# facebookresearch/dmc-net

Hardware: AMD Instinct MI355X
Metric: clips/sec (3-seg 224x224) DMC-gen+ResNet-18 train step (higher is better)
Workload: dtype f32

## Files before the change

### dmc-net_amd/_lib.py

```python
import ctypes
import os

PKG = os.path.dirname(os.path.abspath(__file__))
LIB_PATH = os.environ.get("DMC_HIP_LIB", os.path.join(PKG, "libdmcnet_hip.so"))

_P = ctypes.c_void_p
_I = ctypes.c_int
_F = ctypes.c_float
_Z = ctypes.c_size_t
_L = ctypes.c_long

SIGNATURES = {
    "dmc_version": (_I, []),
    "dmc_last_error": (ctypes.c_char_p, []),
    "dmc_profile_mark": (_I, [_P]),
    "dmc_set_option": (_I, [ctypes.c_char_p, _I]),
    "dmc_get_option": (_I, [ctypes.c_char_p]),
    "dmc_gen_tiny_workspace_bytes": (_Z, []),
    "dmc_gen_tiny_saved_bytes": (_Z, [_I, _I, _I]),
    "dmc_gen_tiny_gbuf_bytes": (_Z, [_I, _I, _I]),
    "dmc_gen_tiny_partials_bytes": (_Z, [_I, _I, _I]),
    "dmc_gen_tiny_fwd": (_I, [_P, _P, _P, _P, _P, _P, _P, _I, _I, _I, _I, _P]),
    "dmc_gen_tiny_mse_partials_bytes": (_Z, []),
    "dmc_gen_tiny_fwd_mse": (_I, [_P] * 10 + [_I, _I, _I, _I, _P]),
    "dmc_gen_tiny_fwd_loss": (_I, [_I] + [_P] * 10 + [_I, _I, _I, _I, _P]),
    "dmc_gen_tiny_bwd": (_I, [_P, _P, _P, _P, _P, _P, _P, _P, _P, _P, _I, _I, _I, _P]),
    "dmc_flow_mse_partials_bytes": (_Z, []),
    "dmc_flow_mse_fwd": (_I, [_P, _P, _P, _P, _Z, _P]),
    "dmc_flow_mse_bwd": (_I, [_P, _P, _P, _P, _Z, _P]),
    "dmc_flow_loss_partials_bytes": (_Z, []),
    "dmc_flow_loss_fwd": (_I, [_I, _P, _P, _P, _P, _P, _Z, _P]),
    "dmc_flow_loss_bwd": (_I, [_I, _P, _P, _P, _P, _P, _P, _Z, _P]),
    "dmc_consensus_ce_fwd_bwd": (_I, [_P, _P, _P, _P, _P, _I, _I, _I, _P]),
    "dmc_disc_tail_stats_bytes": (_Z, [_I]),
    "dmc_disc_tail_fwd": (_I, [_P, _P, _P, _P, _P, _P, _P, _P, _I, _I, _I, _I, _I, _I, _F, _F, _P]),
    "dmc_disc_tail_bwd": (_I, [_P, _P, _P, _P, _P, _P, _P, _P, _I, _I, _I, _I, _I, _P]),
    "dmc_prepare_inputs_workspace_bytes": (_Z, [_I, _I, _I, _I]),
    "dmc_prepare_inputs": (_I, [_P, _P, _P, _P, _P, _P, _I, _I, _I, _I, _P, _P]),
    "dmc_prepare_crop_workspace_bytes": (_Z, [_I, _I, _I, _I]),
    "dmc_prepare_inputs_crop": (_I, [_P, _P, _P, _P, _P, _P, _P, _I, _I, _I, _I, _I, _I, _P, _P]),
    "dmc_prepare_views_workspace_bytes": (_Z, [_I, _I, _I, _I, _I]),
    "dmc_prepare_inputs_views": (_I, [_P, _P, _P, _P, _P, _P, _P, _P, _I, _I, _I, _I, _I, _I, _I, _I, _P, _P]),
    "dmc_prepare_interp_taps": (_I, [_I, _I, _P, _P, _P]),
    "dmc_prepare_clip_workspace_bytes": (_Z, [_I, _I, _I, _I, _I]),
    "dmc_prepare_clip": (_I, [_P, _P, _P, _P] + [_I] * 8 + [_P, _P, _P]),
    "dmc_bn_act_supported": (_I, [_I, _I]),
    "dmc_bn_act_stats_bytes": (_Z, [_I]),
    "dmc_bn_act_scratch_bytes": (_Z, [_I]),
    "dmc_bn_act_fwd": (_I, [_P, _P, _P, _P, _P, _P, _P, _P, _P, _P, _I, _I, _I, _I, _F, _F, _P]),
    "dmc_bn_act_bwd": (_I, [_P, _P, _P, _P, _P, _P, _P, _P, _P, _P, _P, _P, _I, _I, _I, _P]),
    "dmc_bn_apply_nhwc": (_I, [_P, _P, _P, _P, _P, _I, _I, _P]),
    "dmc_bn_apply_act_nhwc": (_I, [_P, _P, _P, _P, _P, _P, _P, _I, _I, _I, _P]),
    "dmc_bn_bwd_act_nhwc": (_I, [_P] * 10 + [_I, _F, _I, _I, _P]),
    "dmc_channel_sum_nhwc": (_I, [_P, _P, _P, _I, _I, _P]),
    "dmc_bn_relu_pool_supported": (_I, [_I, _I, _I, _I]),
    "dmc_bn_relu_pool_fwd": (_I, [_P, _P, _P, _P, _P, _P, _P, _P, _I, _I, _I, _I, _I, _F, _F, _P]),
    "dmc_bn_relu_pool_codes_bytes": (_Z, [_I, _I, _I, _I]),
    "dmc_bn_relu_pool_bwd": (_I, [_P, _P, _P, _P, _P, _P, _P, _P, _P, _P, _I, _I, _I, _I, _P]),
    "dmc_conv_nhwc_supported": (_I, [_I] * 9),
    "dmc_conv_nhwc_stat_blocks": (_I, [_I] * 8),
    "dmc_conv_nhwc_fwd": (_I, [_P] * 7 + [_I] * 11 + [_P]),
    "dmc_conv_nhwc_stats_final": (_I, [_P, _I, _I, ctypes.c_long, _P, _P, _P, _F, _F, _P]),
    "dmc_conv_nhwc_wt_bytes": (_Z, [_I] * 4),
    "dmc_conv_nhwc_presplit_supported": (_I, [_I, _I]),
    "dmc_conv_nhwc_split": (_I, [_P, _P, _P, _I, _I, _I, _I, _P]),
    "dmc_conv_nhwc_dgrad": (_I, [_P] * 4 + [_I] * 9 + [_P]),
    "dmc_conv_nhwc_dgrad_add": (_I, [_P] * 5 + [_I] * 9 + [_P]),
    "dmc_conv_nhwc_wgrad_bytes": (_Z, [_I] * 9),
    "dmc_conv_nhwc_wgrad": (_I, [_P] * 4 + [_I] * 9 + [_P]),
    "dmc_x3s_slices_bytes": (_Z, [_L, _I]),
    "dmc_x3s_split": (_I, [_P, _P, _L, _I, _P]),
    "dmc_x3s_merge": (_I, [_P, _P, _L, _I, _P]),
    "dmc_x3s_wpack_bytes": (_Z, [_I, _I]),
    "dmc_x3s_pack_weights": (_I, [_P, _P, _P, _I, _I, _P]),
    "dmc_x3s_conv_supported": (_I, [_I] * 5),
    "dmc_x3s_conv_stat_blocks": (_I, [_I] * 4),
    "dmc_x3s_conv_fwd": (_I, [_P] * 4 + [_I] * 6 + [_P]),
    "dmc_x3s_conv_bn_eval": (_I, [_P] * 8 + [_I] * 7 + [_P]),
    "dmc_x3s_conv_dgrad": (_I, [_P] * 4 + [_I] * 5 + [_P]),
    "dmc_x3s_conv_wgrad_supported": (_I, [_I] * 5),
    "dmc_x3s_conv_wgrad_bytes": (_Z, [_I] * 5),
    "dmc_x3s_conv_wgrad": (_I, [_P] * 4 + [_I] * 5 + [_P]),
    "dmc_x3s_conv_dgrad_s2_supported": (_I, [_I] * 5),
    "dmc_x3s_pack_weights_s2": (_I, [_P, _P, _I, _I, _P]),
    "dmc_x3s_conv_dgrad_s2": (_I, [_P] * 3 + [_I] * 5 + [_P]),
    "dmc_x3q_wpack_bytes": (_Z, [_I, _I]),
    "dmc_x3q_supported": (_I, [_I] * 5),
    "dmc_x3q_stat_blocks": (_I, [_I] * 4),
    "dmc_x3q_split": (_I, [_P, _P, _I, _I, _I, _I, _P]),
    "dmc_x3q_merge": (_I, [_P, _P, _I, _I, _I, _I, _P]),
    "dmc_x3q_pack_weights": (_I, [_P, _P, _P, _P, _I, _I, _P]),
    "dmc_x3q_conv_fwd": (_I, [_P] * 6 + [_I] * 6 + [_P]),
    "dmc_x3q_conv_bn_eval": (_I, [_P] * 11 + [_I] * 5 + [_P]),
    "dmc_x3q_conv_dgrad": (_I, [_P] * 4 + [_I] * 5 + [_P]),
    "dmc_bn_apply_act_x3q": (_I, [_P] * 8 + [_I] * 5 + [_P]),
    "dmc_x3q_conv_wgrad_supported": (_I, [_I] * 5),
    "dmc_x3q_conv_wgrad_bytes": (_Z, [_I] * 5),
    "dmc_x3q_conv_wgrad": (_I, [_P] * 6 + [_I] * 5 + [_P]),
    "dmc_bn_apply_act_x3s": (_I, [_P] * 8 + [_I, _I, _I, _P]),
    "dmc_bn_act_bwd_x3s": (_I, [_P] * 13 + [_I, _I, _I, _P]),
    "dmc_x3s_conv_dgrad_bnb": (_I, [_P] * 9 + [_I] + [_P] + [_I] + [_P] * 2 + [_I] * 5 + [_P]),
    "dmc_bn_act_bwd_x3s_apply": (_I, [_P] * 12 + [_I, _I, _I, _P]),
    "dmc_bn_relu_pool_fwd_x3s": (_I, [_P] * 9 + [_I, _I, _I, _I, _I, _F, _F, _P]),
    "dmc_bn_relu_pool_fwd_arg": (_I, [_P] * 11 + [_I, _I, _I, _I, _I, _I, _F, _F, _P]),
    "dmc_bn_relu_pool_bwd_arg": (_I, [_P] * 11 + [_I, _I, _I, _I, _P]),
    "dmc_disc_first_supported": (_I, [_I]),
    "dmc_disc_first_fwd": (_I, [_P] * 5 + [_I] * 5 + [_P]),
    "dmc_disc_first_dgrad": (_I, [_P] * 3 + [_I] * 4 + [_P]),
    "dmc_disc_first_wgrad_bytes": (_Z, [_I]),
    "dmc_disc_first_wgrad": (_I, [_P] * 5 + [_I] * 4 + [_P]),
    "dmc_stem_wgrad_supported": (_I, [_I, _I]),
    "dmc_stem_wgrad_partials_bytes": (_Z, [_I, _I, _I]),
    "dmc_stem_wgrad": (_I, [_P, _P, _P, _P, _I, _I, _I, _P]),
    "dmc_stem_fwd": (_I, [_P, _P, _L, _L, _L, _L, _P, _I, _I, _I, _P]),
    "dmc_stem_fwd_x3_workspace_bytes": (_Z, [_I, _I, _I]),
    "dmc_stem_fwd_x3": (_I, [_P, _P, _L, _L, _L, _L, _P, _P, _I, _I, _I, _P]),
    "dmc_stem_fwd_x3_stat_blocks": (_I, [_I, _I, _I]),
    "dmc_stem_dgrad_workspace_bytes": (_Z, []),
    "dmc_stem_dgrad_supported": (_I, [_I, _I]),
    "dmc_stem_dgrad": (_I, [_P, _P, _L, _L, _L, _L, _P, _P, _I, _I, _I, _P]),
    "dmc_stem_fwd_x3_stats": (_I, [_P, _P, _L, _L, _L, _L, _P, _P, _P, _I, _I, _I, _P]),
    "dmc_conv3d_bf16_supported": (_I, [_I] * 9),
    "dmc_conv3d_bf16_wpack_bytes": (_Z, [_I] * 5),
    "dmc_conv3d_bf16_pack": (_I, [_P, _L, _L, _L, _P, _P] + [_I] * 5 + [_P]),
    "dmc_conv3d_bf16_stat_blocks": (_I, [_I] * 5),
    "dmc_conv3d_bf16_stat_blocks_k": (_I, [_I] * 9),
    "dmc_conv3d_bf16_fwd": (_I, [_P, _P, _L, _L, _L, _P, _P, _P] + [_I] * 9 + [_P]),
    "dmc_conv3d_bf16_dgrad": (_I, [_P, _P, _L, _L, _L, _P, _P] + [_I] * 9 + [_P]),
    "dmc_conv3d_bf16_wgrad_bytes": (_Z, [_I] * 9),
    "dmc_conv3d_bf16_wgrad": (_I, [_P] * 4 + [_I] * 9 + [_P]),
    "dmc_stem3d_bf16_workspace_bytes": (_Z, [_I] * 4),
    "dmc_stem3d_bf16_stat_blocks": (_I, [_I] * 4),
    "dmc_stem3d_bf16_fwd": (_I, [_P] * 5 + [_I] * 4 + [_P]),
    "dmc_stem3d_bf16_wgrad_workspace_bytes": (_Z, [_I] * 4),
    "dmc_stem3d_bf16_wgrad": (_I, [_P] * 4 + [_I] * 4 + [_P]),
    "dmc_stem3d_bf16_dgrad_workspace_bytes": (_Z, []),
    "dmc_stem3d_bf16_dgrad": (_I, [_P] * 4 + [_I] * 4 + [_P]),
    "dmc_bn3d_bf16_supported": (_I, [_L, _I]),
    "dmc_bn3d_bf16_scratch_bytes": (_Z, [_I]),
    "dmc_bn3d_bf16_fwd": (_I, [_P, _P, _I, _P, _P, _P, _P, _P, _P, _L, _I, _I, _F, _F, _P]),
    "dmc_add4_bf16": (_I, [_P] * 5 + [_L, _P]),
    "dmc_bn3d_bf16_fwd_ld": (_I, [_P, _P, _I, _P, _P, _P, _P, _P, _P, _L, _L, _I, _I, _F, _F, _P]),
    "dmc_bn3d_bf16_bwd": (_I, [_P, _L] + [_P] * 8 + [_L, _I, _I, _P]),
    "dmc_unit3d_bf16_fwd_workspace_bytes": (_Z, [_I] * 9),
    "dmc_unit3d_bf16_bwd_workspace_bytes": (_Z, [_I] * 9),
    "dmc_unit3d_bf16_fwd": (_I, [_P] * 9 + [_I] * 10 + [_F, _F, _P]),
    "dmc_unit3d_bf16_fwd_into": (_I, [_P] * 9 + [_L] + [_I] * 10 + [_F, _F, _P]),
    "dmc_unit3d_bf16_bwd": (_I, [_P, _L] + [_P] * 11 + [_I] * 10 + [_P]),
    "dmc_unit3d_bf16_eval_workspace_bytes": (_Z, [_I] * 9),
    "dmc_unit3d_bf16_fwd_eval": (_I, [_P] * 6 + [_F, _P, _P, _L] + [_I] * 10 + [_P]),
    "dmc_stem3d_bf16_eval_workspace_bytes": (_Z, [_I] * 4),
    "dmc_stem3d_bf16_fwd_eval": (_I, [_P] * 6 + [_F, _P, _P] + [_I] * 5 + [_P]),
    "dmc_maxpool3d_tf_out_shape": (_I, [_I] * 10 + [_P] * 3),
    "dmc_maxpool3d_tf_bf16_fwd": (_I, [_P] * 3 + [_I] * 11 + [_P]),
    "dmc_maxpool3d_tf_bf16_bwd": (_I, [_P] * 3 + [_I] * 11 + [_P]),
    "dmc_mv_owner_bytes": (_Z, [_I, _I, _I]),
    "dmc_mv_accu_init": (_I, [_P, _I, _I, _P]),
    "dmc_mv_rasterise": (_I, [_P, _I, _I, _P, _P, _P, _I, _I, _P]),
    "dmc_mv_accumulate": (_I, [_P, _I, _I, _P, _P, _P, _P, _I, _I, _P]),
    "dmc_mv_from_accu": (_I, [_P, _P, _I, _I, _P]),
    "dmc_residual": (_I, [_P, _P, _P, _P, _P, _I, _I, _P]),
    "dmc_mv_gop_batch": (_I, [_P, _I, _I, _P, _I, _P, _I, _P, _P, _P, _P, _P, _P, _P, _P, _I, _I, _P]),
}

_lib = None


class DmcHipError(RuntimeError):
    pass


def load():
    global _lib
    if _lib is None:
        if not os.path.exists(LIB_PATH):
            raise DmcHipError(
                "%s is missing: the DMC-Net hot path has no CPU fallback. Build it with "
                "`python -c 'import __graft_entry__ as g; g.build()'`." % LIB_PATH)
        lib = ctypes.CDLL(LIB_PATH)
        for name, (res, args) in SIGNATURES.items():
            fn = getattr(lib, name)
            fn.restype, fn.argtypes = res, args
        _lib = lib
    return _lib


def check(rc, what):
    if rc != 0:
        raise DmcHipError("%s failed (%d): %s" % (what, rc, load().dmc_last_error().decode()))


def ptr(t):
    return _P(t.data_ptr()) if t is not None else _P(0)


def ptr_array(tensors):
    return (_P * len(tensors))(*[t.data_ptr() for t in tensors])
```

### dmc-net_amd/csrc/conv_x3q.hip

```cpp
#include "dmc_common.h"
#include "x3s_common.h"
#include <type_traits>
#include <utility>

using namespace dmc;
using namespace dmc::x3;

namespace {

constexpr int QBM = 256, QBN = 64;
constexpr int QWSLOT = 3 * QBN * 32;
constexpr int QWB = 3 * QWSLOT;
constexpr int QEP = 272, QETILE = 32 * QEP;

template <int NW_, int NPB_, int NT_>
struct QG {
    static constexpr int NW = NW_, NPB = NPB_, NT = NT_;
    static constexpr int NA = NW / 2;
    static constexpr int KP = (NT + NA - 1) / NA;
    static constexpr int PT = 3 * KP;
    static constexpr int KW = (18 + NA - 1) / NA;
    static constexpr int ZROW = 32 * NT;
    static constexpr int PSL = (ZROW + 1) * 32;
    static constexpr int PB = 3 * PSL;
    static constexpr int WOFF = NPB * PB;
    static constexpr int LDS_OP = WOFF + 2 * QWB;
    static constexpr int LDS_EP = NW * QETILE + 8192;
    static constexpr int LDS = LDS_OP > LDS_EP ? LDS_OP : LDS_EP;
    static constexpr bool COUNTED = NPB == 3;
    static_assert(!COUNTED || NT % NA == 0, "counted waits need the same number of transfers from every patch wave");
};
using QGBig = QG<8, 3, 12>;
using QGTwo = QG<4, 2, 7>;

struct QSlot { int sh, acc; };
struct QStep { int unit, nslot; QSlot s[3]; };

struct ProgFwd {
    static constexpr int NUNIT = 4, NSTEP = 5, NACC = 2, NSH = 4, HALO_UP = 1, HALO_DN = 0, NSLOTS = 10;
    static constexpr int SHY[4] = {-1, -1, 0, 0}, SHX[4] = {-1, 0, -1, 0};
    static constexpr int UNIT_T[4] = {0, 0, 0, 0};
    static constexpr int UNIT_G[4] = {3, 1, 2, 0};
    static constexpr QStep STEP[5] = {{0, 2, {{0, 0}, {1, 0}, {0, 0}}}, {0, 2, {{2, 0}, {3, 0}, {0, 0}}}, {1, 2, {{2, 0}, {3, 0}, {0, 0}}},
                                      {2, 2, {{1, 0}, {3, 0}, {0, 0}}}, {3, 2, {{3, 0}, {3, 1}, {0, 0}}}};
};
struct ProgDgrad {
    static constexpr int NUNIT = 2, NSTEP = 4, NACC = 4, NSH = 4, HALO_UP = 0, HALO_DN = 1, NSLOTS = 10;
    static constexpr int SHY[4] = {0, 0, 1, 1}, SHX[4] = {0, 1, 0, 1};
    static constexpr int UNIT_T[2] = {0, 1};
    static constexpr int UNIT_G[2] = {0, 0};
    static constexpr QStep STEP[4] = {{0, 3, {{3, 3}, {2, 2}, {2, 3}}}, {0, 3, {{1, 1}, {0, 0}, {0, 1}}}, {0, 3, {{1, 3}, {0, 2}, {0, 3}}},
                                      {1, 1, {{0, 0}, {0, 0}, {0, 0}}}};
};

template <class P> constexpr int slots_before(int j) { int n = 0; for (int i = 0; i < j; ++i) n += P::STEP[i].nslot; return n; }

struct X3qArgs {
    const void* t0;
    const void* t1;
    const void* wp;
    float* y0;
    float* y1;
    double* part0;
    double* part1;
    int N, H, W;
    int K, R, M;
    unsigned plane_bytes;
    int pps0, pps1;
};

struct X3qEvalArgs : X3qArgs {
    const float *stats0, *gamma0, *beta0;
    const float *stats1, *gamma1, *beta1;
    unsigned short* ys0;
};

template <int N, class F, int... I>
__device__ __forceinline__ void static_for_impl(F&& f, std::integer_sequence<int, I...>) { (f(std::integral_constant<int, I>{}), ...); }
template <int N, class F>
__device__ __forceinline__ void static_for(F&& f) { static_for_impl<N>(f, std::make_integer_sequence<int, N>{}); }

template <class P, int TN, class GEO, bool EVAL = false>
__global__ __launch_bounds__(GEO::NW * 64) void x3q_conv_kernel(std::conditional_t<EVAL, X3qEvalArgs, X3qArgs> a) {
    static_assert(!EVAL || P::NACC == 2, "the eval epilogue belongs to the forward pair");
    constexpr int NSH = P::NSH, NACC = P::NACC, NSTEP = P::NSTEP, NUNIT = P::NUNIT;
    constexpr int QNW = GEO::NW, QNPB = GEO::NPB, QZROW = GEO::ZROW, QPSL = GEO::PSL, QPB = GEO::PB, QWOFF = GEO::WOFF, QPT = GEO::PT;
    constexpr int NA = GEO::NA, KP = GEO::KP, KW = GEO::KW;
    constexpr int WN = 2 / TN, WM = QNW / WN, BM = 32 * WM;
    static_assert(TN == 1 || TN == 2, "a wave owns 32 or 64 of the workgroup's 64 rows");
    constexpr int CHB = P::NSLOTS * QWSLOT;
    static_assert(P::NSLOTS % 2 == 0, "the fragment registers alternate per slot: an even number per chunk keeps the roles fixed");
    extern __shared__ __attribute__((aligned(1024))) char lds_q[];

    const int tid = threadIdx.x, lane = tid & 63;
    const int wave = __builtin_amdgcn_readfirstlane(tid >> 6);
    const int wm = wave % WM, wn = wave / WM;
    const int l31 = lane & 31, khalf = lane >> 5;
    const unsigned lds0 = lds_addr_of(lds_q);

    const int HW = a.H * a.W, PW = a.W;
    const int m0 = blockIdx.x * BM;
    const int mlast = (m0 + BM < a.M ? m0 + BM : a.M) - 1;
    const int r_first = m0 / PW, r_last = mlast / PW;
    const int f0 = (r_first - P::HALO_UP > 0 ? r_first - P::HALO_UP : 0) * PW;
    const int f1 = (r_last + 1 + P::HALO_DN) * PW < a.M ? (r_last + 1 + P::HALO_DN) * PW : a.M;
    const int PP = f1 - f0;

    const bool grp_a = wave < NA;
    const int wq = wave % NA;
    unsigned pvoff[KP];
#pragma unroll
    for (int k = 0; k < KP; ++k) {
        const int pr = 32 * (wq + NA * k) + (lane >> 1), h = lane & 1;
        pvoff[k] = pr < PP ? (unsigned)(f0 + pr) * 32u + (unsigned)((h ^ ((pr >> 3) & 1)) << 4) : OOB;
    }
    const int nchunk = a.K >> 4;
    const int total_units = nchunk * NUNIT, total_steps = nchunk * NSTEP;
    const u32x4 srd0 = make_srd(a.t0), srd1 = make_srd(a.t1 ? a.t1 : a.t0);
    const u32x4 srd_w = make_srd(reinterpret_cast<const char*>(a.wp) + (size_t)blockIdx.y * nchunk * CHB);
    const unsigned lane16 = (unsigned)lane * 16u;

    auto dma_patch = [&](int c, auto uc, int pbuf, int i) {
        constexpr int u = decltype(uc)::value;
        constexpr int ut = P::UNIT_T[u], ug = P::UNIT_G[u];
        const int s = i / KP, k = i - KP * s;
        const unsigned soff = (unsigned)(s * (ut ? a.pps1 : a.pps0) + ug * nchunk + c) * a.plane_bytes;
        if (GEO::COUNTED || wq + NA * k < GEO::NT)
            dma_buf16(ut ? srd1 : srd0, pvoff[k], soff, lds0 + pbuf * QPB + s * QPSL + (wq + NA * k) * 1024);
    };
    auto dma_weight = [&](int c, auto jc, int wbuf, int e) {
        constexpr int j = decltype(jc)::value;
        constexpr int n = P::STEP[j].nslot * 6, off = slots_before<P>(j) * QWSLOT;
        if (e < n) dma_buf16(srd_w, lane16, (unsigned)(c * CHB + off + e * 1024), lds0 + QWOFF + wbuf * QWB + e * 1024);
    };

    int xaddr[NSH];
    {
        int m = m0 + wm * 32 + l31;
        if (m > mlast) m = mlast;
        const int n = m / HW, rem = m - n * HW, yy = rem / a.W, xx = rem - yy * a.W;
        const int pp = m - f0;
        static_for<NSH>([&](auto sc) {
            constexpr int sh = decltype(sc)::value;
            constexpr int dy = P::SHY[sh], dx = P::SHX[sh];
            const int row = (xx + dx >= 0 && xx + dx < a.W && yy + dy >= 0 && yy + dy < a.H) ? pp + dy * PW + dx : QZROW;
            xaddr[sh] = row * 32 + ((khalf ^ ((row >> 3) & 1)) << 4);
        });
    }
    const int waddr = QWOFF + (wn * TN * 32 + l31) * 32 + ((khalf ^ ((l31 >> 3) & 1)) << 4);

    f32x16 acc[NACC][TN];
#pragma unroll
    for (int s = 0; s < NACC; ++s)
#pragma unroll
        for (int j = 0; j < TN; ++j)
#pragma unroll
            for (int e = 0; e < 16; ++e) acc[s][j][e] = 0.f;

    lds_cptr const L = (lds_cptr)lds_q;
    struct Frag { u32x4 X[3], W[TN][3]; };
    auto load_frags = [&](Frag& f, int xa, int wa, auto kc) {
        constexpr int k = decltype(kc)::value;
#pragma unroll
        for (int s = 0; s < 3; ++s) {
#pragma unroll
            for (int j = 0; j < TN; ++j)
                f.W[j][s] = *reinterpret_cast<const __attribute__((address_space(3))) u32x4*>(L + wa + ((k * 3 + s) * QBN + 32 * j) * 32);
            f.X[s] = *reinterpret_cast<const __attribute__((address_space(3))) u32x4*>(L + xa + s * QPSL);
        }
    };
    auto mfma_slot = [&](const Frag& f, auto ac, auto&& between) {
        constexpr int A = decltype(ac)::value;
#pragma unroll
        for (int p = 0; p < 6; ++p) {
            constexpr int WS[6] = {0, 0, 0, 1, 1, 2}, XS[6] = {2, 1, 0, 1, 0, 0};
#pragma unroll
            for (int j = 0; j < TN; ++j) acc[A][j] = mfma_bf16(f.W[j][WS[p]], f.X[XS[p]], acc[A][j]);
            between(p);
        }
    };
    auto nothing = [](int) {};
    constexpr int NRD = 3 + 3 * TN, NMF = 6 * TN;
    auto interleave = [&]() {
#pragma unroll
        for (int k = 0; k < (NRD < NMF ? NRD : NMF); ++k) {
            __builtin_amdgcn_sched_group_barrier(0x008, 1, 0);
            __builtin_amdgcn_sched_group_barrier(0x100, 1, 0);
        }
        if constexpr (NMF > NRD) __builtin_amdgcn_sched_group_barrier(0x008, NMF - NRD, 0);
    };

    if (tid < 2 * 3 * QNPB)
        *reinterpret_cast<float4*>(lds_q + (tid >> 1) / 3 * QPB + ((tid >> 1) % 3) * QPSL + QZROW * 32 + (tid & 1) * 16) = make_float4(0.f, 0.f, 0.f, 0.f);
    if (grp_a) {
        static_for<QNPB>([&](auto uc) {
            constexpr int U = decltype(uc)::value;
            if (U < total_units) {
#pragma unroll
                for (int i = 0; i < QPT; ++i) dma_patch(U / NUNIT, std::integral_constant<int, U % NUNIT>{}, U, i);
            }
        });
    } else {
        static_for<2>([&](auto gc) {
            constexpr int g = decltype(gc)::value;
            if (g < total_steps) {
#pragma unroll
                for (int i = 0; i < KW; ++i) dma_weight(g / NSTEP, std::integral_constant<int, g % NSTEP>{}, g, wq + NA * i);
            }
        });
    }
    asm volatile("s_waitcnt vmcnt(0)" ::: "memory");
    __builtin_amdgcn_s_barrier();

    Frag F0, F1;
    int pb = 0, wb = 0;
    int xcur[NSH];
#pragma unroll
    for (int sh = 0; sh < NSH; ++sh) xcur[sh] = xaddr[sh];
    int wcur = waddr;
    {
        constexpr int sh0 = P::STEP[0].s[0].sh;
        load_frags(F0, xcur[sh0], wcur, std::integral_constant<int, 0>{});
    }

    auto frag_of = [&](auto ic) -> Frag& {
        if constexpr (decltype(ic)::value == 0) return F0; else return F1;
    };
#pragma unroll 1
    for (int c = 0; c < nchunk; ++c) {
        static_for<NSTEP>([&](auto jc) {
            constexpr int J = decltype(jc)::value;
            constexpr int JN = (J + 1) % NSTEP;
            constexpr int unit = P::STEP[J].unit, nslot = P::STEP[J].nslot;
            constexpr bool unit_last = (P::STEP[JN].unit != unit) || (NUNIT == 1 && J == NSTEP - 1);
            constexpr int par = slots_before<P>(J) & 1;
            const int g = c * NSTEP + J, U = c * NUNIT + unit;
            static_for<nslot - 1>([&](auto kc) {
                constexpr int k = decltype(kc)::value;
                constexpr int sh_next = P::STEP[J].s[k + 1].sh, acc_k = P::STEP[J].s[k].acc;
                load_frags(frag_of(std::integral_constant<int, (par + k + 1) & 1>{}), xcur[sh_next], wcur, std::integral_constant<int, k + 1>{});
                mfma_slot(frag_of(std::integral_constant<int, (par + k) & 1>{}), std::integral_constant<int, acc_k>{}, nothing);
                interleave();
            });
            if (GEO::COUNTED && grp_a && U + 2 < total_units) asm volatile("s_waitcnt vmcnt(%0) lgkmcnt(0)" :: "n"(QPT) : "memory");
            else asm volatile("s_waitcnt vmcnt(0) lgkmcnt(0)" ::: "memory");
            __builtin_amdgcn_s_barrier();
            const int pb_old = pb, wb_old = wb;
            if constexpr (unit_last) {
                pb = pb == QNPB - 1 ? 0 : pb + 1;
#pragma unroll
                for (int sh = 0; sh < NSH; ++sh) xcur[sh] = xaddr[sh] + pb * QPB;
            }
            wb ^= 1;
            wcur = waddr + wb * QWB;
            constexpr int kl = nslot - 1;
            constexpr int sh_first = P::STEP[JN].s[0].sh, acc_last = P::STEP[J].s[kl].acc;
            if (g + 1 < total_steps)
                load_frags(frag_of(std::integral_constant<int, (par + kl + 1) & 1>{}), xcur[sh_first], wcur, std::integral_constant<int, 0>{});
            constexpr int J2 = (J + 2) % NSTEP, C2 = (J + 2) / NSTEP;
            constexpr int U3 = (unit + QNPB) % NUNIT, CU3 = (unit + QNPB) / NUNIT;
            const bool wgo = !grp_a && g + 2 < total_steps;
            const bool pgo = grp_a && unit_last && U + QNPB < total_units;
            mfma_slot(frag_of(std::integral_constant<int, (par + kl) & 1>{}), std::integral_constant<int, acc_last>{}, [&](int p) {
                if (wgo) {
#pragma unroll
                    for (int i = p; i < KW; i += 6) dma_weight(c + C2, std::integral_constant<int, J2>{}, wb_old, wq + NA * i);
                }
                if constexpr (unit_last) {
                    if (pgo) {
#pragma unroll
                        for (int i = p; i < QPT; i += 6) dma_patch(c + CU3, std::integral_constant<int, U3>{}, pb_old, i);
                    }
                }
            });
        });
    }

    __syncthreads();
    constexpr int CW = 32 * TN, LPR = CW / 4, RPI = 64 / LPR;
    char* etile = lds_q + wave * QETILE;
    const int mw0 = m0 + wm * 32;
    const int rbase = blockIdx.y * QBN + wn * CW;
    const bool ok = mw0 + l31 <= mlast;
#pragma unroll
    for (int A = 0; A < NACC; ++A) {
#pragma unroll
        for (int j = 0; j < TN; ++j)
#pragma unroll
            for (int g4 = 0; g4 < 4; ++g4) {
                float4 v = make_float4(acc[A][j][4 * g4], acc[A][j][4 * g4 + 1], acc[A][j][4 * g4 + 2], acc[A][j][4 * g4 + 3]);
                if (!ok) v = make_float4(0.f, 0.f, 0.f, 0.f);
                *reinterpret_cast<float4*>(etile + l31 * QEP + (32 * j + 8 * g4 + 4 * khalf) * 4) = v;
            }
        float* const yout = (NACC == 2 && A == 1) ? a.y1 : a.y0;
        if constexpr (EVAL) {
            const int c4 = rbase + (lane % LPR) * 4;
            const float* const st = A == 1 ? a.stats1 : a.stats0;
            const float4 mean = *reinterpret_cast<const float4*>(st + c4), istd = *reinterpret_cast<const float4*>(st + a.R + c4);
            const float4 gm = *reinterpret_cast<const float4*>((A == 1 ? a.gamma1 : a.gamma0) + c4);
            const float4 bt = *reinterpret_cast<const float4*>((A == 1 ? a.beta1 : a.beta0) + c4);
            unsigned short* const ys = A == 1 ? nullptr : a.ys0;
#pragma unroll
            for (int it = 0; it < 32 / RPI; ++it) {
                const int prow = RPI * it + lane / LPR;
                const int m = mw0 + prow;
                const float4 v = *reinterpret_cast<const float4*>(etile + prow * QEP + (lane % LPR) * 16);
                if (m <= mlast) {
                    const float w[4] = {bn_apply_act1(v.x, mean.x, istd.x, gm.x, bt.x, false, 0.f, A == 0),
                                        bn_apply_act1(v.y, mean.y, istd.y, gm.y, bt.y, false, 0.f, A == 0),
                                        bn_apply_act1(v.z, mean.z, istd.z, gm.z, bt.z, false, 0.f, A == 0),
                                        bn_apply_act1(v.w, mean.w, istd.w, gm.w, bt.w, false, 0.f, A == 0)};
                    if (yout) *reinterpret_cast<float4*>(yout + (size_t)m * a.R + c4) = make_float4(w[0], w[1], w[2], w[3]);
                    if (ys) x3s_store4(ys, w, (size_t)a.M, a.R >> 4, (size_t)m, c4 >> 2);
                }
            }
        } else {
#pragma unroll
        for (int it = 0; it < 32 / RPI; ++it) {
            const int prow = RPI * it + lane / LPR;
            const int m = mw0 + prow;
            const float4 v = *reinterpret_cast<const float4*>(etile + prow * QEP + (lane % LPR) * 16);
            if (m <= mlast) {
                size_t opix = (size_t)m;
                if (NACC == 4) {
                    const int n = m / HW, rem = m - n * HW, ya = rem / a.W, xb = rem - ya * a.W;
                    opix = ((size_t)n * (2 * a.H) + 2 * ya + (A >> 1)) * (2 * a.W) + 2 * xb + (A & 1);
                }
                *reinterpret_cast<float4*>(yout + opix * a.R + rbase + (lane % LPR) * 4) = v;
            }
        }
        }
        if (NACC == 2 && !EVAL) {
            double* const part = A == 1 ? a.part1 : a.part0;
            if (part) {
                double* red = reinterpret_cast<double*>(lds_q + QNW * QETILE);
                if (lane < CW) {
                    double d1 = 0.0, d2 = 0.0;
#pragma unroll 8
                    for (int p = 0; p < 32; ++p) {
                        const double v = (double)*reinterpret_cast<const float*>(etile + p * QEP + lane * 4);
                        d1 += v;
                        d2 += v * v;
                    }
                    red[(wm * 64 + wn * CW + lane) * 2 + 0] = d1;
                    red[(wm * 64 + wn * CW + lane) * 2 + 1] = d2;
                }
                __syncthreads();
                for (int cc = tid; cc < QBN; cc += QNW * 64) {
                    double e1 = 0.0, e2 = 0.0;
#pragma unroll
                    for (int w = 0; w < WM; ++w) { e1 += red[(w * 64 + cc) * 2 + 0]; e2 += red[(w * 64 + cc) * 2 + 1]; }
                    double* dst = part + ((size_t)blockIdx.x * a.R + blockIdx.y * QBN + cc) * 2;
                    dst[0] = e1; dst[1] = e2;
                }
                __syncthreads();
            }
        }
    }
}

__global__ __launch_bounds__(256) void x3q_pack_w_kernel(const float* __restrict__ w3, const float* __restrict__ w1,
                                                         unsigned short* __restrict__ wf, unsigned short* __restrict__ wt, int Cout, int Cin) {
    const bool transposed = blockIdx.y == 1;
    unsigned short* dst = transposed ? wt : wf;
    if (!dst) return;
    const int R = transposed ? Cin : Cout, K = transposed ? Cout : Cin;
    const int nchunk = K >> 4;
    const long total = (long)R * 10 * K;
    for (long i = (long)blockIdx.x * 256 + threadIdx.x; i < total; i += (long)gridDim.x * 256) {
        long t = i;
        const int kk = (int)(t & 15); t >>= 4;
        const int rl = (int)(t & 63); t >>= 6;
        const int slot = (int)(t % 10); t /= 10;
        const int ch = (int)(t % nchunk);
        const int rt = (int)(t / nchunk);
        const int r = rt * 64 + rl, k = ch * 16 + kk;
        constexpr int FWD_TAP[10] = {0, 2, 6, 8, 3, 5, 1, 7, 4, 9};
        const int tap = transposed ? slot : FWD_TAP[slot];
        const int co = transposed ? k : r, ci = transposed ? r : k;
        const float v = tap < 9 ? w3[((long)co * 9 + tap) * Cin + ci] : w1[(long)co * Cin + ci];
        unsigned u0, u1, u2;
        split3(v, u0, u1, u2);
        const size_t base = ((((size_t)(rt * nchunk + ch) * 10 + slot) * 3) * 64 + rl) * 16 + (kk ^ (((rl >> 3) & 1) << 3));
        dst[base] = (unsigned short)(u0 >> 16);
        dst[base + 64 * 16] = (unsigned short)(u1 >> 16);
        dst[base + 2 * 64 * 16] = (unsigned short)(u2 >> 16);
    }
}

__global__ __launch_bounds__(256) void x3q_split_kernel(const float* __restrict__ x, unsigned short* __restrict__ xq, int N, int H, int W, int C) {
    const int c8 = C >> 3, nchunk = C >> 4, H2 = H >> 1, W2 = W >> 1;
    const long total = (long)N * H * W * c8;
    const size_t Mq = (size_t)N * H2 * W2;
    for (long o = (long)blockIdx.x * 256 + threadIdx.x; o < total; o += (long)gridDim.x * 256) {
        const long m = o / c8;
        const int g = (int)(o - m * c8);
        const int xx = (int)(m % W), yy = (int)((m / W) % H), n = (int)(m / ((long)W * H));
        const float4 a = reinterpret_cast<const float4*>(x)[2 * o], b = reinterpret_cast<const float4*>(x)[2 * o + 1];
        const float v[8] = {a.x, a.y, a.z, a.w, b.x, b.y, b.z, b.w};
        const int cls = (yy & 1) * 2 + (xx & 1);
        x3s_store8(xq, v, Mq, 4 * nchunk, ((size_t)n * H2 + (yy >> 1)) * W2 + (xx >> 1), g + cls * 2 * nchunk);
    }
}

__global__ __launch_bounds__(256) void x3q_merge_kernel(const unsigned short* __restrict__ xq, float* __restrict__ x, int N, int H, int W, int C) {
    const int nchunk = C >> 4, H2 = H >> 1, W2 = W >> 1;
    const long total = (long)N * H * W * C;
    const size_t Mq = (size_t)N * H2 * W2, plane = Mq * 16;
    for (long o = (long)blockIdx.x * 256 + threadIdx.x; o < total; o += (long)gridDim.x * 256) {
        const long m = o / C;
        const int c = (int)(o - m * C);
        const int xx = (int)(m % W), yy = (int)((m / W) % H), n = (int)(m / ((long)W * H));
        const int cls = (yy & 1) * 2 + (xx & 1);
        const size_t mq = ((size_t)n * H2 + (yy >> 1)) * W2 + (xx >> 1);
        const size_t w = ((size_t)(cls * nchunk + (c >> 4)) * Mq + mq) * 16 + (c & 15);
        const float s0 = __uint_as_float((unsigned)xq[w] << 16);
        const float s1 = __uint_as_float((unsigned)xq[(size_t)4 * nchunk * plane + w] << 16);
        const float s2 = __uint_as_float((unsigned)xq[(size_t)8 * nchunk * plane + w] << 16);
        x[o] = (s0 + s1) + s2;
    }
}

int stream_blocks_q(long total) {
    long b = (total + 255) / 256;
    return (int)(b < 1 ? 1 : (b > 8192 ? 8192 : b));
}

int q_patch_pixels_max(long M, int W) {
    int worst = 0;
    long tiles = (M + QBM - 1) / QBM;
    if (tiles > W) tiles = W;
    for (long t = 0; t < tiles; ++t) {
        const long m0 = t * QBM, ml = (m0 + QBM < M ? m0 + QBM : M) - 1;
        const int pp = (int)((ml / W - m0 / W + 2) * W);
        if (pp > worst) worst = pp;
    }
    return worst;
}

int q_patch_pixels_max128(long M, int W) {
    int worst = 0;
    long tiles = (M + 127) / 128;
    if (tiles > W) tiles = W;
    for (long t = 0; t < tiles; ++t) {
        const long m0 = t * 128, ml = (m0 + 128 < M ? m0 + 128 : M) - 1;
        const int pp = (int)((ml / W - m0 / W + 2) * W);
        if (pp > worst) worst = pp;
    }
    return worst;
}

bool q_shape_ok(int N, int OH, int OW, int Cin, int Cout) {
    if (N <= 0 || OH <= 0 || OW <= 0 || Cin <= 0 || Cout <= 0 || Cin % 64 != 0 || Cout % 64 != 0) return false;
    const long M = (long)N * OH * OW;
    if (M * 4 * Cin * 6 >= (1L << 31) || M * Cout * 6 >= (1L << 31)) return false;
    return q_patch_pixels_max(M, OW) <= QGBig::ZROW;
}

int q_choose_tn(long M, int R) {
    const int forced = option(OPT_CONV_CFG);
    if (forced == 201) return 2;
    if (forced == 202) return 1;
    const long n2 = ((M + 255) / 256) * (R / QBN), n1 = ((M + 127) / 128) * (R / QBN);
    const double t2 = (double)((n2 + 255) / 256), t1 = 0.75 * (double)((n1 + 255) / 256);
    return t1 < t2 ? 1 : 2;
}

template <class P, int TN, class GEO>
int launch_q(const X3qArgs& a, hipStream_t s) {
    static LdsLimit lim;
    const hipError_t attr = lim.raise(reinterpret_cast<const void*>(&x3q_conv_kernel<P, TN, GEO>), GEO::LDS);
    if (attr != hipSuccess) return fail(DMC_E_LAUNCH, "x3q_conv: cannot raise the dynamic LDS limit: %s", hipGetErrorString(attr));
    constexpr int BM = 32 * GEO::NW / (2 / TN);
    dim3 grid((a.M + BM - 1) / BM, a.R / QBN);
    x3q_conv_kernel<P, TN, GEO><<<grid, GEO::NW * 64, GEO::LDS, s>>>(a);
    return check_launch("x3q_conv");
}

template <int TN, class GEO>
int launch_q_eval(const X3qEvalArgs& a, hipStream_t s) {
    static LdsLimit lim;
    const hipError_t attr = lim.raise(reinterpret_cast<const void*>(&x3q_conv_kernel<ProgFwd, TN, GEO, true>), GEO::LDS);
    if (attr != hipSuccess) return fail(DMC_E_LAUNCH, "x3q_conv_bn_eval: cannot raise the dynamic LDS limit: %s", hipGetErrorString(attr));
    constexpr int BM = 32 * GEO::NW / (2 / TN);
    dim3 grid((a.M + BM - 1) / BM, a.R / QBN);
    x3q_conv_kernel<ProgFwd, TN, GEO, true><<<grid, GEO::NW * 64, GEO::LDS, s>>>(a);
    return check_launch("x3q_conv_bn_eval");
}

int q_patch_pixels_max128(long M, int W);
int q_variant(long M, int W, int R) {
    const int forced = option(OPT_CONV_CFG);
    const bool two_ok = q_patch_pixels_max128(M, W) <= QGTwo::ZROW;
    if (forced == 201) return 0;
    if (forced == 202) return 1;
    if (forced == 203 && two_ok) return 2;
    if (forced != 204 && two_ok && ((M + 127) / 128) * (R / QBN) >= 512) return 2;
    return q_choose_tn(M, R) == 2 ? 0 : 1;
}
int q_block_pixels(int variant) { return variant == 0 ? 256 : 128; }


struct X3qWgArgs {
    const void* xq;
    const void* dys;
    float* part;
    int N, OH, Cin, Cout;
    unsigned plane_bytes;
    int steps, per_group, tiles_ci;
};

template <int OW_, int R, int HP_>
struct QWgGeom {
    static constexpr int PW = OW_ + 1;
    static constexpr int D1 = 3, D0 = 2;
    static constexpr int XPL1 = ((D1 * R * PW + 3) / 8) * 8 + 4;
    static constexpr int XPL0 = ((D0 * R * PW + 3) / 8) * 8 + 4;
    static constexpr int NPX = R * OW_;
    static constexpr int NKB = (NPX + 15) / 16;
    static constexpr int DYT = ((NKB * 16 + 31) / 32) * 32;
    static constexpr int DYPL = ((DYT + 3) / 8) * 8 + 4;
    static constexpr int XI = (R * PW + 31) / 32;
    static constexpr int DI = DYT / 32;
    static constexpr int CLS_OFF[4] = {0, 4 * XPL0 * 32, 8 * XPL0 * 32, 8 * XPL0 * 32 + 4 * XPL1 * 32};
    static constexpr int SLB = 8 * XPL0 * 32 + 8 * XPL1 * 32;
    static constexpr int XBYTES = 3 * SLB, DYBYTES = 12 * DYPL * 32;
    static constexpr int LDS = XBYTES + 2 * DYBYTES;
    static_assert(HP_ % R == 0, "steps are whole groups of padded rows");
};

template <int OW_, int R, int HP_>
__global__ __launch_bounds__(768) void x3q_wgrad_kernel(X3qWgArgs a) {
    using G = QWgGeom<OW_, R, HP_>;
    constexpr int PW = G::PW, DYPL = G::DYPL, NKB = G::NKB;
    extern __shared__ __attribute__((aligned(1024))) char lds_qw[];
    const int tid = threadIdx.x, lane = tid & 63;
    const int wave = __builtin_amdgcn_readfirstlane(tid >> 6);
    const int l31 = lane & 31, khalf = lane >> 5, L = lane & 15, grp = (lane >> 4) & 1;
    const int quarter = wave & 3, trow = wave >> 2;
    const int wi = quarter & 1, wj = quarter >> 1;
    const int tci = blockIdx.x % a.tiles_ci, tco = blockIdx.x / a.tiles_ci;
    const unsigned lds0 = lds_addr_of(lds_qw);
    const int s_begin = blockIdx.y * a.per_group;
    const int s_end = s_begin + a.per_group < a.steps ? s_begin + a.per_group : a.steps;
    const u32x4 srd_x = make_srd(a.xq), srd_d = make_srd(a.dys);
    const int nch_in = a.Cin >> 4;
    const int tsl = wave >> 2, tch = wave & 3;
    const unsigned soff_d = (unsigned)(tsl * (a.Cout >> 4) + tco * 4 + tch) * a.plane_bytes;
    const unsigned dplane = lds0 + G::XBYTES + (unsigned)wave * DYPL * 32;
    const int lpx = lane >> 1;
    const unsigned lhalf = (unsigned)(lane & 1) << 4;

    const unsigned img_bytes = (unsigned)(a.OH * OW_) * 32u;
    unsigned xpre[G::XI], dpre[G::DI];
#pragma unroll
    for (int i = 0; i < G::XI; ++i) {
        const int px = 32 * i + lpx;
        const int r = px / PW, col = px - r * PW - 1;
        xpre[i] = (col >= 0 && col < OW_) ? (unsigned)(r * OW_ + col) * 32u + lhalf : NOPIX;
    }
#pragma unroll
    for (int i = 0; i < G::DI; ++i) {
        const int p = 32 * i + lpx;
        dpre[i] = p < G::NPX ? (unsigned)p * 32u + lhalf : NOPIX;
    }
    auto issue_x = [&](int q, const WgGroupPos& g) {
        unsigned tbase, img_off;
        wg_group_base(g, a.N, OW_, img_bytes, tbase, img_off);
        unsigned voff[G::XI];
#pragma unroll
        for (int i = 0; i < G::XI; ++i) voff[i] = wg_lane_off(tbase, xpre[i], img_bytes);
#pragma unroll
        for (int cls = 0; cls < 4; ++cls) {
            const int D = (cls >> 1) ? G::D1 : G::D0, xpl = (cls >> 1) ? G::XPL1 : G::XPL0;
            const int slot0 = (((q % D) + D) % D) * R;
            const unsigned soff_x = (unsigned)(tsl * 4 * nch_in + cls * nch_in + tci * 4 + tch) * a.plane_bytes + img_off;
            const unsigned xplane = lds0 + (unsigned)(tsl * G::SLB + G::CLS_OFF[cls] + tch * xpl * 32);
#pragma unroll
            for (int i = 0; i < G::XI; ++i)
                if (32 * i + lpx < R * PW) dma_buf16(srd_x, voff[i], soff_x, xplane + (unsigned)(slot0 * PW + 32 * i) * 32u);
        }
    };
    auto issue_dy = [&](const WgGroupPos& g, int buf) {
        unsigned tbase, img_off;
        wg_group_base(g, a.N, OW_, img_bytes, tbase, img_off);
#pragma unroll
        for (int i = 0; i < G::DI; ++i)
            dma_buf16(srd_d, wg_lane_off(tbase, dpre[i], img_bytes), soff_d + img_off, dplane + (unsigned)buf * G::DYBYTES + (unsigned)(32 * i) * 32u);
    };

    f32x16 acc[3];
#pragma unroll
    for (int t = 0; t < 3; ++t)
#pragma unroll
        for (int e = 0; e < 16; ++e) acc[t][e] = 0.f;

    WgGroupPos g1 = wg_group_at(s_begin, R, HP_);
    if (s_begin < s_end) {
        issue_x(s_begin - 1, wg_group_prev(g1, R, HP_));
        issue_x(s_begin, g1);
        issue_dy(g1, 0);
    }
    g1 = wg_group_next(g1, R, HP_);
    asm volatile("s_waitcnt vmcnt(0)" ::: "memory");
    __builtin_amdgcn_s_barrier();
    const int py = trow != 1, da = trow == 0 ? -1 : 0;
    const int DR = (py ? G::D1 : G::D0) * R, xpl = py ? G::XPL1 : G::XPL0;
    const int cls_a = py ? G::CLS_OFF[3] : G::CLS_OFF[1];
    const int cls_b = py ? G::CLS_OFF[2] : G::CLS_OFF[0];
    lds_cptr const LB = (lds_cptr)lds_qw;
    int rr[NKB][2], xcol[NKB][2], dyoff[NKB][2];
#pragma unroll
    for (int kb = 0; kb < NKB; ++kb)
#pragma unroll
        for (int u = 0; u < 2; ++u) {
            int P = 16 * kb + 8 * khalf + 4 * u + (L >> 2);
            dyoff[kb][u] = (2 * wi + grp) * DYPL * 32 + G::XBYTES + (L & 3) * 8 + P * 32;
            if (P >= G::NPX) P = G::NPX - 1;
            rr[kb][u] = P / OW_;
            xcol[kb][u] = (2 * wj + grp) * xpl * 32 + (L & 3) * 8 + (P - rr[kb][u] * OW_) * 32;
        }
#pragma unroll 1
    for (int s = s_begin; s < s_end; ++s) {
        const int buf = (s - s_begin) & 1;
        issue_x(s + 1, g1);
        if (s + 1 < s_end) issue_dy(g1, buf ^ 1);
        g1 = wg_group_next(g1, R, HP_);
        const int sb = (((R * s + da) % DR) + DR) % DR;
#pragma unroll
        for (int kb = 0; kb < NKB; ++kb) {
            int dyo[2], xa[2], xb[2];
#pragma unroll
            for (int u = 0; u < 2; ++u) {
                dyo[u] = dyoff[kb][u] + buf * G::DYBYTES;
                int slot = sb + rr[kb][u];
                slot = slot >= DR ? slot - DR : slot;
                const int xo = xcol[kb][u] + slot * PW * 32;
                xa[u] = xo + cls_a;
                xb[u] = xo + cls_b;
            }
            u32x4 A[3], B[3][3];
#pragma unroll
            for (int sl = 0; sl < 3; ++sl) {
                tr_read2(LB + dyo[0] + sl * 4 * DYPL * 32, LB + dyo[1] + sl * 4 * DYPL * 32, A[sl]);
                tr_read2(LB + xa[0] + sl * G::SLB, LB + xa[1] + sl * G::SLB, B[0][sl]);
                tr_read2(LB + xb[0] + sl * G::SLB + 32, LB + xb[1] + sl * G::SLB + 32, B[1][sl]);
                tr_read2(LB + xa[0] + sl * G::SLB + 32, LB + xa[1] + sl * G::SLB + 32, B[2][sl]);
            }
#pragma unroll
            for (int t = 0; t < 3; ++t) {
                acc[t] = mfma_bf16(A[0], B[t][2], acc[t]);
                acc[t] = mfma_bf16(A[2], B[t][0], acc[t]);
                acc[t] = mfma_bf16(A[1], B[t][1], acc[t]);
                acc[t] = mfma_bf16(A[0], B[t][1], acc[t]);
                acc[t] = mfma_bf16(A[1], B[t][0], acc[t]);
                acc[t] = mfma_bf16(A[0], B[t][0], acc[t]);
            }
        }
        asm volatile("s_waitcnt vmcnt(0) lgkmcnt(0)" ::: "memory");
        __builtin_amdgcn_s_barrier();
    }
    float* out = a.part + (size_t)blockIdx.y * a.Cout * 9 * a.Cin;
    const int ci = tci * 64 + 32 * wj + l31;
#pragma unroll
    for (int t = 0; t < 3; ++t)
#pragma unroll
        for (int e = 0; e < 16; ++e) {
            const int co = tco * 64 + 32 * wi + 8 * (e >> 2) + 4 * khalf + (e & 3);
            out[((size_t)co * 9 + 3 * trow + t) * a.Cin + ci] = acc[t][e];
        }
}

struct X3qWg1Args {
    const void* xq; const void* dys; float* part;
    int Cin, Cout; long Mq; unsigned plane_bytes; int steps, per_group, tiles_ci;
};
constexpr int W1PX = 64, W1PL = 68;
constexpr int W1TILE = 12 * W1PL * 32, W1LDS = 4 * W1TILE;

__global__ __launch_bounds__(256) void x3q_wgrad1_kernel(X3qWg1Args a) {
    extern __shared__ __attribute__((aligned(1024))) char lds_w1[];
    const int tid = threadIdx.x, lane = tid & 63;
    const int wave = __builtin_amdgcn_readfirstlane(tid >> 6);
    const int l31 = lane & 31, khalf = lane >> 5, L = lane & 15, grp = (lane >> 4) & 1;
    const int wi = wave & 1, wj = wave >> 1;
    const int tci = blockIdx.x % a.tiles_ci, tco = blockIdx.x / a.tiles_ci;
    const unsigned lds0 = lds_addr_of(lds_w1);
    const int s_begin = blockIdx.y * a.per_group;
    const int s_end = s_begin + a.per_group < a.steps ? s_begin + a.per_group : a.steps;
    const u32x4 srd_x = make_srd(a.xq), srd_d = make_srd(a.dys);
    const int nch_in = a.Cin >> 4, nch_out = a.Cout >> 4;
    const int lpx = lane >> 1;
    const unsigned lhalf = (unsigned)(lane & 1) << 4;
    auto issue = [&](int s, int buf) {
#pragma unroll
        for (int k = 0; k < 3; ++k) {
            const int pl = 3 * wave + k, sl = pl >> 2, ch = pl & 3;
#pragma unroll
            for (int i = 0; i < 2; ++i) {
                const long p = (long)s * W1PX + 32 * i + lpx;
                const unsigned voff = p < a.Mq ? (unsigned)p * 32u + lhalf : OOB;
                dma_buf16(srd_x, voff, (unsigned)(sl * 4 * nch_in + tci * 4 + ch) * a.plane_bytes,
                          lds0 + (unsigned)(buf * 2 * W1TILE + pl * W1PL * 32 + 32 * i * 32));
                dma_buf16(srd_d, voff, (unsigned)(sl * nch_out + tco * 4 + ch) * a.plane_bytes,
                          lds0 + (unsigned)(buf * 2 * W1TILE + W1TILE + pl * W1PL * 32 + 32 * i * 32));
            }
        }
    };
    f32x16 acc;
#pragma unroll
    for (int e = 0; e < 16; ++e) acc[e] = 0.f;
    if (s_begin < s_end) issue(s_begin, 0);
    asm volatile("s_waitcnt vmcnt(0)" ::: "memory");
    __builtin_amdgcn_s_barrier();
    lds_cptr const LB = (lds_cptr)lds_w1;
#pragma unroll 1
    for (int s = s_begin; s < s_end; ++s) {
        const int buf = (s - s_begin) & 1;
        if (s + 1 < s_end) issue(s + 1, buf ^ 1);
        const int xb = buf * 2 * W1TILE + (2 * wj + grp) * W1PL * 32 + (L & 3) * 8;
        const int db = buf * 2 * W1TILE + W1TILE + (2 * wi + grp) * W1PL * 32 + (L & 3) * 8;
#pragma unroll
        for (int kb = 0; kb < W1PX / 16; ++kb) {
            u32x4 A[3], B[3];
            const int P0 = 16 * kb + 8 * khalf + (L >> 2), P1 = P0 + 4;
#pragma unroll
            for (int sl = 0; sl < 3; ++sl) {
                tr_read2(LB + db + sl * 4 * W1PL * 32 + P0 * 32, LB + db + sl * 4 * W1PL * 32 + P1 * 32, A[sl]);
                tr_read2(LB + xb + sl * 4 * W1PL * 32 + P0 * 32, LB + xb + sl * 4 * W1PL * 32 + P1 * 32, B[sl]);
            }
            acc = mfma_bf16(A[0], B[2], acc);
            acc = mfma_bf16(A[2], B[0], acc);
            acc = mfma_bf16(A[1], B[1], acc);
            acc = mfma_bf16(A[0], B[1], acc);
            acc = mfma_bf16(A[1], B[0], acc);
            acc = mfma_bf16(A[0], B[0], acc);
        }
        asm volatile("s_waitcnt vmcnt(0) lgkmcnt(0)" ::: "memory");
        __builtin_amdgcn_s_barrier();
    }
    float* out = a.part + (size_t)blockIdx.y * a.Cout * a.Cin;
    const int ci = tci * 64 + 32 * wj + l31;
#pragma unroll
    for (int e = 0; e < 16; ++e) {
        const int co = tco * 64 + 32 * wi + 8 * (e >> 2) + 4 * khalf + (e & 3);
        out[(size_t)co * a.Cin + ci] = acc[e];
    }
}

__global__ __launch_bounds__(256) void x3q_wgrad_reduce_kernel(const float* __restrict__ part, float* __restrict__ dw, int ngroup, long numel) {
    __shared__ float4 red[16][17];
    const int o = threadIdx.x & 15, sl = threadIdx.x >> 4;
    for (long i0 = (long)blockIdx.x * 64; i0 < numel; i0 += (long)gridDim.x * 64) {
        const long i = i0 + 4 * o;
        float4 s = make_float4(0.f, 0.f, 0.f, 0.f);
        if (i < numel)
            for (int k = sl; k < ngroup; k += 16) {
                const float4 v = *reinterpret_cast<const float4*>(part + (size_t)k * numel + i);
                s.x += v.x; s.y += v.y; s.z += v.z; s.w += v.w;
            }
        red[sl][o] = s;
        __syncthreads();
        if (sl == 0 && i < numel) {
            float4 t = red[0][o];
#pragma unroll
            for (int k = 1; k < 16; ++k) { const float4 v = red[k][o]; t.x += v.x; t.y += v.y; t.z += v.z; t.w += v.w; }
            *reinterpret_cast<float4*>(dw + i) = t;
        }
        __syncthreads();
    }
}

struct QWgPlan { int R, HP, steps, tiles, groups, per_group, steps1, groups1, per_group1; };
bool q_wgrad_plan(int N, int OH, int OW, int Cin, int Cout, QWgPlan& p) {
    if (Cin % 64 != 0 || Cout % 64 != 0 || N <= 0) return false;
    if (OW == 28 && OH == 28) { p.R = 1; p.HP = 29; }
    else if (OW == 14 && OH == 14) { p.R = 2; p.HP = 16; }
    else if (OW == 7 && OH == 7) { p.R = 4; p.HP = 8; }
    else return false;
    p.steps = N * p.HP / p.R;
    p.tiles = (Cout / 64) * (Cin / 64);
    int groups = 256 / p.tiles;
    if (groups < 1) groups = 1;
    if (groups > p.steps) groups = p.steps;
    p.per_group = (p.steps + groups - 1) / groups;
    p.groups = (p.steps + p.per_group - 1) / p.per_group;
    const long Mq = (long)N * OH * OW;
    p.steps1 = (int)((Mq + W1PX - 1) / W1PX);
    int g1 = 512 / p.tiles;
    if (g1 < 1) g1 = 1;
    if (g1 > p.steps1) g1 = p.steps1;
    p.per_group1 = (p.steps1 + g1 - 1) / g1;
    p.groups1 = (p.steps1 + p.per_group1 - 1) / p.per_group1;
    return true;
}

template <int OW_, int R, int HP_>
int launch_q_wgrad(const QWgPlan& p, const X3qWgArgs& a, hipStream_t s) {
    using G = QWgGeom<OW_, R, HP_>;
    static_assert(G::LDS <= 160 * 1024, "weight-gradient tiles exceed the LDS");
    static LdsLimit lim;
    const hipError_t attr = lim.raise(reinterpret_cast<const void*>(&x3q_wgrad_kernel<OW_, R, HP_>), G::LDS);
    if (attr != hipSuccess) return fail(DMC_E_LAUNCH, "x3q_wgrad: cannot raise the dynamic LDS limit: %s", hipGetErrorString(attr));
    x3q_wgrad_kernel<OW_, R, HP_><<<dim3(p.tiles, p.groups), 768, G::LDS, s>>>(a);
    return check_launch("x3q_wgrad");
}

}

extern "C" {

size_t dmc_x3q_wpack_bytes(int Cin, int Cout) { return (size_t)Cin * (size_t)Cout * 10 * 6; }

int dmc_x3q_supported(int N, int OH, int OW, int Cin, int Cout) { return q_shape_ok(N, OH, OW, Cin, Cout) ? 1 : 0; }

int dmc_x3q_stat_blocks(int N, int OH, int OW, int Cout) {
    const long M = (long)N * OH * OW;
    const int bm = q_block_pixels(q_variant(M, OW, Cout));
    return (int)((M + bm - 1) / bm);
}

int dmc_x3q_split(const float* x, void* xq, int N, int H, int W, int C, dmc_stream_t stream) {
    if (!x || !xq || N <= 0 || H <= 0 || W <= 0 || (H & 1) || (W & 1) || C <= 0 || C % 16 != 0)
        return fail(DMC_E_INVALID, "dmc_x3q_split: bad argument");
    x3q_split_kernel<<<stream_blocks_q((long)N * H * W * (C / 8)), 256, 0, (hipStream_t)stream>>>(x, static_cast<unsigned short*>(xq), N, H, W, C);
    return check_launch("x3q_split");
}

int dmc_x3q_merge(const void* xq, float* x, int N, int H, int W, int C, dmc_stream_t stream) {
    if (!x || !xq || N <= 0 || H <= 0 || W <= 0 || (H & 1) || (W & 1) || C <= 0 || C % 16 != 0)
        return fail(DMC_E_INVALID, "dmc_x3q_merge: bad argument");
    x3q_merge_kernel<<<stream_blocks_q((long)N * H * W * C), 256, 0, (hipStream_t)stream>>>(static_cast<const unsigned short*>(xq), x, N, H, W, C);
    return check_launch("x3q_merge");
}

int dmc_x3q_pack_weights(const float* w3, const float* w1, void* wpack_f, void* wpack_t, int Cin, int Cout, dmc_stream_t stream) {
    if (!w3 || !w1 || (!wpack_f && !wpack_t) || Cin % 64 != 0 || Cout % 64 != 0 || Cin <= 0 || Cout <= 0)
        return fail(DMC_E_INVALID, "dmc_x3q_pack_weights: bad argument");
    const long total = (long)Cin * Cout * 10;
    const int blocks = stream_blocks_q(total) > 1024 ? 1024 : stream_blocks_q(total);
    x3q_pack_w_kernel<<<dim3(blocks, 2), 256, 0, (hipStream_t)stream>>>(w3, w1, static_cast<unsigned short*>(wpack_f),
                                                                           static_cast<unsigned short*>(wpack_t), Cout, Cin);
    return check_launch("x3q_pack_w");
}

int dmc_x3q_conv_fwd(const void* xq, const void* wpack_f, float* y3, float* y1, double* stat_partials3, double* stat_partials1,
                     int stat_blocks, int N, int OH, int OW, int Cin, int Cout, dmc_stream_t stream) {
    if (!xq || !wpack_f || !y3 || !y1) return fail(DMC_E_INVALID, "dmc_x3q_conv_fwd: null pointer");
    if (!q_shape_ok(N, OH, OW, Cin, Cout))
        return fail(DMC_E_INVALID, "dmc_x3q_conv_fwd: unsupported shape N=%d OH=%d OW=%d Cin=%d Cout=%d", N, OH, OW, Cin, Cout);
    const int var = q_variant((long)N * OH * OW, OW, Cout);
    const int rows = (int)(((long)N * OH * OW + q_block_pixels(var) - 1) / q_block_pixels(var));
    if ((stat_partials3 || stat_partials1) && stat_blocks != rows)
        return fail(DMC_E_INVALID, "dmc_x3q_conv_fwd: statistics partials have %d rows but this launch writes %d (dmc_x3q_stat_blocks "
                                   "was called under another conv_cfg option?)", stat_blocks, rows);
    X3qArgs a;
    a.t0 = xq; a.t1 = nullptr; a.wp = wpack_f; a.y0 = y3; a.y1 = y1; a.part0 = stat_partials3; a.part1 = stat_partials1;
    a.N = N; a.H = OH; a.W = OW; a.K = Cin; a.R = Cout; a.M = N * OH * OW;
    a.plane_bytes = (unsigned)a.M * 32u;
    a.pps0 = 4 * (Cin / 16); a.pps1 = 0;
    return var == 0 ? launch_q<ProgFwd, 2, QGBig>(a, (hipStream_t)stream) : var == 1 ? launch_q<ProgFwd, 1, QGBig>(a, (hipStream_t)stream)
                                                                                      : launch_q<ProgFwd, 2, QGTwo>(a, (hipStream_t)stream);
}

int dmc_x3q_conv_bn_eval(const void* xq, const void* wpack_f, const float* stats3, const float* gamma3, const float* beta3,
                         const float* stats1, const float* gamma1, const float* beta1, float* y3, void* ys3, float* y1, int N, int OH,
                         int OW, int Cin, int Cout, dmc_stream_t stream) {
    if (!xq || !wpack_f || !stats3 || !gamma3 || !beta3 || !stats1 || !gamma1 || !beta1 || !y1)
        return fail(DMC_E_INVALID, "dmc_x3q_conv_bn_eval: null pointer");
    if (!y3 && !ys3) return fail(DMC_E_INVALID, "dmc_x3q_conv_bn_eval: no main-branch output (y3 and ys3 are both null)");
    if (!q_shape_ok(N, OH, OW, Cin, Cout))
        return fail(DMC_E_INVALID, "dmc_x3q_conv_bn_eval: unsupported shape N=%d OH=%d OW=%d Cin=%d Cout=%d", N, OH, OW, Cin, Cout);
    const int var = q_variant((long)N * OH * OW, OW, Cout);
    X3qEvalArgs a;
    a.t0 = xq; a.t1 = nullptr; a.wp = wpack_f; a.y0 = y3; a.y1 = y1; a.part0 = a.part1 = nullptr;
    a.N = N; a.H = OH; a.W = OW; a.K = Cin; a.R = Cout; a.M = N * OH * OW;
    a.plane_bytes = (unsigned)a.M * 32u;
    a.pps0 = 4 * (Cin / 16); a.pps1 = 0;
    a.stats0 = stats3; a.gamma0 = gamma3; a.beta0 = beta3; a.stats1 = stats1; a.gamma1 = gamma1; a.beta1 = beta1;
    a.ys0 = static_cast<unsigned short*>(ys3);
    return var == 0 ? launch_q_eval<2, QGBig>(a, (hipStream_t)stream) : var == 1 ? launch_q_eval<1, QGBig>(a, (hipStream_t)stream)
                                                                                  : launch_q_eval<2, QGTwo>(a, (hipStream_t)stream);
}

int dmc_x3q_conv_dgrad(const void* dys3, const void* dys1, const void* wpack_t, float* dx, int N, int OH, int OW, int Cin, int Cout,
                       dmc_stream_t stream) {
    if (!dys3 || !dys1 || !wpack_t || !dx) return fail(DMC_E_INVALID, "dmc_x3q_conv_dgrad: null pointer");
    if (!q_shape_ok(N, OH, OW, Cin, Cout))
        return fail(DMC_E_INVALID, "dmc_x3q_conv_dgrad: unsupported shape N=%d OH=%d OW=%d Cin=%d Cout=%d", N, OH, OW, Cin, Cout);
    X3qArgs a;
    a.t0 = dys3; a.t1 = dys1; a.wp = wpack_t; a.y0 = dx; a.y1 = nullptr; a.part0 = a.part1 = nullptr;
    a.N = N; a.H = OH; a.W = OW; a.K = Cout; a.R = Cin; a.M = N * OH * OW;
    a.plane_bytes = (unsigned)a.M * 32u;
    a.pps0 = a.pps1 = Cout / 16;
    const int var = q_variant(a.M, OW, Cin);
    return var == 0 ? launch_q<ProgDgrad, 2, QGBig>(a, (hipStream_t)stream) : var == 1 ? launch_q<ProgDgrad, 1, QGBig>(a, (hipStream_t)stream)
                                                                                        : launch_q<ProgDgrad, 2, QGTwo>(a, (hipStream_t)stream);
}

int dmc_x3q_conv_wgrad_supported(int N, int OH, int OW, int Cin, int Cout) {
    QWgPlan p;
    return q_shape_ok(N, OH, OW, Cin, Cout) && q_wgrad_plan(N, OH, OW, Cin, Cout, p) ? 1 : 0;
}

size_t dmc_x3q_conv_wgrad_bytes(int N, int OH, int OW, int Cin, int Cout) {
    QWgPlan p;
    if (!q_wgrad_plan(N, OH, OW, Cin, Cout, p)) return 0;
    return ((size_t)p.groups * 9 + (size_t)p.groups1) * Cout * Cin * sizeof(float);
}

int dmc_x3q_conv_wgrad(const void* xq, const void* dys3, const void* dys1, float* dw3, float* dw1, float* workspace, int N, int OH,
                       int OW, int Cin, int Cout, dmc_stream_t stream) {
    QWgPlan p;
    if (!xq || !dys3 || !dys1 || !dw3 || !dw1 || !workspace) return fail(DMC_E_INVALID, "dmc_x3q_conv_wgrad: null pointer");
    if (!dmc_x3q_conv_wgrad_supported(N, OH, OW, Cin, Cout) || !q_wgrad_plan(N, OH, OW, Cin, Cout, p))
        return fail(DMC_E_INVALID, "dmc_x3q_conv_wgrad: unsupported shape N=%d OH=%d OW=%d Cin=%d Cout=%d", N, OH, OW, Cin, Cout);
    hipStream_t s = (hipStream_t)stream;
    const long Mq = (long)N * OH * OW;
    X3qWgArgs a;
    a.xq = xq; a.dys = dys3; a.part = workspace;
    a.N = N; a.OH = OH; a.Cin = Cin; a.Cout = Cout;
    a.plane_bytes = (unsigned)Mq * 32u;
    a.steps = p.steps; a.per_group = p.per_group; a.tiles_ci = Cin / 64;
    int rc = OW == 28 ? launch_q_wgrad<28, 1, 29>(p, a, s) : OW == 14 ? launch_q_wgrad<14, 2, 16>(p, a, s) : launch_q_wgrad<7, 4, 8>(p, a, s);
    if (rc) return rc;
    const long numel3 = (long)Cout * 9 * Cin, numel1 = (long)Cout * Cin;
    long blocks = (numel3 + 63) / 64;
    x3q_wgrad_reduce_kernel<<<(int)(blocks > 4096 ? 4096 : blocks), 256, 0, s>>>(workspace, dw3, p.groups, numel3);
    rc = check_launch("x3q_wgrad_reduce");
    if (rc) return rc;
    float* part1 = workspace + (size_t)p.groups * numel3;
    X3qWg1Args b;
    b.xq = xq; b.dys = dys1; b.part = part1; b.Cin = Cin; b.Cout = Cout; b.Mq = Mq; b.plane_bytes = (unsigned)Mq * 32u;
    b.steps = p.steps1; b.per_group = p.per_group1; b.tiles_ci = Cin / 64;
    static LdsLimit lim1;
    const hipError_t attr = lim1.raise(reinterpret_cast<const void*>(&x3q_wgrad1_kernel), W1LDS);
    if (attr != hipSuccess) return fail(DMC_E_LAUNCH, "x3q_wgrad1: cannot raise the dynamic LDS limit: %s", hipGetErrorString(attr));
    x3q_wgrad1_kernel<<<dim3(p.tiles, p.groups1), 256, W1LDS, s>>>(b);
    rc = check_launch("x3q_wgrad1");
    if (rc) return rc;
    blocks = (numel1 + 63) / 64;
    x3q_wgrad_reduce_kernel<<<(int)(blocks > 4096 ? 4096 : blocks), 256, 0, s>>>(part1, dw1, p.groups1, numel1);
    return check_launch("x3q_wgrad_reduce1");
}

}
```

### dmc-net_amd/csrc/conv_x3s.hip

```cpp
#include "dmc_common.h"
#include "x3s_common.h"
#include <type_traits>

using namespace dmc;
using namespace dmc::x3;

namespace {

__global__ __launch_bounds__(256) void x3s_split_kernel(const float* __restrict__ x, unsigned short* __restrict__ xs, long M, int C) {
    const int c8 = C >> 3;
    const long total = M * c8;
    const int nchunk = C >> 4;
    for (long o = (long)blockIdx.x * 256 + threadIdx.x; o < total; o += (long)gridDim.x * 256) {
        const long m = o / c8;
        const int g = (int)(o - m * c8);
        const float4 a = reinterpret_cast<const float4*>(x)[2 * o], b = reinterpret_cast<const float4*>(x)[2 * o + 1];
        const float v[8] = {a.x, a.y, a.z, a.w, b.x, b.y, b.z, b.w};
        x3s_store8(xs, v, (size_t)M, nchunk, (size_t)m, g);
    }
}

__global__ __launch_bounds__(256) void x3s_merge_kernel(const unsigned short* __restrict__ xs, float* __restrict__ x, long M, int C) {
    const long total = M * C;
    const size_t plane = (size_t)M * 16;
    const int nchunk = C >> 4;
    for (long o = (long)blockIdx.x * 256 + threadIdx.x; o < total; o += (long)gridDim.x * 256) {
        const long m = o / C;
        const int c = (int)(o - m * C);
        const size_t w = ((size_t)(c >> 4) * M + m) * 16 + (c & 15);
        const float a = __uint_as_float((unsigned)xs[w] << 16);
        const float b = __uint_as_float((unsigned)xs[(size_t)nchunk * plane + w] << 16);
        const float d = __uint_as_float((unsigned)xs[(size_t)2 * nchunk * plane + w] << 16);
        x[o] = (a + b) + d;
    }
}

__global__ __launch_bounds__(256) void x3s_pack_w_kernel(const float* __restrict__ w, unsigned short* __restrict__ wf,
                                                         unsigned short* __restrict__ wt, int Cout, int Cin, int mirror) {
    const bool transposed = blockIdx.y == 1;
    unsigned short* dst = transposed ? wt : wf;
    if (!dst) return;
    const int R = transposed ? Cin : Cout, K = transposed ? Cout : Cin;
    const int nchunk = K >> 4;
    const long total = (long)R * 9 * K;
    for (long i = (long)blockIdx.x * 256 + threadIdx.x; i < total; i += (long)gridDim.x * 256) {
        long t = i;
        const int kk = (int)(t & 15); t >>= 4;
        const int rl = (int)(t & 63); t >>= 6;
        const int tap = (int)(t % 9); t /= 9;
        const int ch = (int)(t % nchunk);
        const int rt = (int)(t / nchunk);
        const int r = rt * 64 + rl, k = ch * 16 + kk;
        const float v = transposed ? w[((long)k * 9 + (mirror ? 8 - tap : tap)) * Cin + r] : w[((long)r * 9 + tap) * Cin + k];
        unsigned u0, u1, u2;
        split3(v, u0, u1, u2);
        const size_t base = ((((size_t)(rt * nchunk + ch) * 9 + tap) * 3) * 64 + rl) * 16 + (kk ^ (((rl >> 3) & 1) << 3));
        dst[base] = (unsigned short)(u0 >> 16);
        dst[base + 64 * 16] = (unsigned short)(u1 >> 16);
        dst[base + 2 * 64 * 16] = (unsigned short)(u2 >> 16);
    }
}

struct X3Args {
    const void* xs;
    const void* wp;
    float* y;
    const float* addend;
    double* stat_part;
    int N, H, W, K, R;
    int M;
    unsigned plane_bytes;
    const float* bnb_y = nullptr;
    const float* bnb_stats = nullptr;
    const float* bnb_gamma = nullptr;
    const float* bnb_beta = nullptr;
    const unsigned char* bnb_mask = nullptr;
    int bnb_relu = 0;
    double* bnb_part = nullptr;
    int part_blocks = -1;
    int ablate;
};
struct X3EvalArgs : X3Args {
    const float* stats;
    const float* gamma;
    const float* beta;
    const float* res;
    unsigned short* ys;
    int s2d, relu;
};

template <int WM, int WN, int TM, int TN, int PPMAX, bool STAG = false, int CLS = 1, bool EVAL = false>
__global__ __launch_bounds__(WM * WN * 64) void x3s_conv_kernel(std::conditional_t<EVAL, X3EvalArgs, X3Args> a) {
    static_assert(!EVAL || CLS == 1, "the eval epilogue belongs to the forward convolution");
    constexpr int NW = WM * WN, BM = 32 * TM * WM, BN = 32 * TN * WN;
    static_assert(BN == 64, "packed weight image is 64 rows wide");
    static_assert(PPMAX % 32 == 0 || PPMAX % 32 == 1, "patch transfers move 32 pixel rows");
    constexpr int PSL = PPMAX * 32;
    constexpr int PB = 3 * PSL;
    constexpr int WB = 3 * 3 * BN * 32;
    constexpr int WOFF = 2 * PB;
    static_assert(!STAG || NW >= 4, "two transfer groups need four waves");
    constexpr int NA = STAG ? NW / 2 : NW, NB = NW - (STAG ? NA : 0);
    constexpr int NDW = (PPMAX / 32 + NA - 1) / NA;
    constexpr int NEW = WB / 1024;
    constexpr int NEWW = (NEW + NB - 1) / NB;
    extern __shared__ __attribute__((aligned(1024))) char lds_x3[];

    const int tid = threadIdx.x, lane = tid & 63;
    const int wave = __builtin_amdgcn_readfirstlane(tid >> 6);
    const int wm = wave % WM, wn = wave / WM;
    const int l31 = lane & 31, khalf = lane >> 5;
    const unsigned lds0 = lds_addr_of(lds_x3);

    const int HW = a.H * a.W, PW = a.W;
    constexpr int ZROW = PPMAX - 1;
    const int m0 = blockIdx.x * BM;
    const int mlast = (m0 + BM < a.M ? m0 + BM : a.M) - 1;
    const int r_first = m0 / PW, r_last = mlast / PW;
    const int f0 = (r_first > 0 ? r_first - 1 : 0) * PW;
    const int f1 = (r_last + 2) * PW < a.M ? (r_last + 2) * PW : a.M;
    const int PP = f1 - f0;
    const int ND = (PP + 31) >> 5;

    unsigned pvoff[NDW];
#pragma unroll
    for (int k = 0; k < NDW; ++k) {
        const int pr = 32 * (wave + NA * k) + (lane >> 1), h = lane & 1;
        pvoff[k] = pr < PP ? (unsigned)(f0 + pr) * 32u + (unsigned)((h ^ ((pr >> 3) & 1)) << 4) : OOB;
    }
    int xaddr[TM][9];
#pragma unroll
    for (int i = 0; i < TM; ++i) {
        int m = m0 + (wm * TM + i) * 32 + l31;
        if (m > mlast) m = mlast;
        const int n = m / HW, rem = m - n * HW, yy = rem / a.W, xx = rem - yy * a.W;
        const int pp = m - f0;
#pragma unroll
        for (int t = 0; t < 9; ++t) {
            const int dx = CLS == 4 ? (t % 3 == 0 ? 1 : 0) : t % 3 - 1, dy = CLS == 4 ? (t / 3 == 0 ? 1 : 0) : t / 3 - 1;
            const int row = (xx + dx >= 0 && xx + dx < a.W && yy + dy >= 0 && yy + dy < a.H) ? pp + dy * PW + dx : ZROW;
            xaddr[i][t] = row * 32 + ((khalf ^ ((row >> 3) & 1)) << 4);
        }
    }
    const int waddr = (wn * TN * 32 + l31) * 32 + ((khalf ^ ((l31 >> 3) & 1)) << 4);

    const u32x4 srd_x = make_srd(a.xs);
    const int nchunk = a.K >> 4, S = 3 * nchunk;
    const u32x4 srd_w = make_srd(reinterpret_cast<const char*>(a.wp) + (size_t)blockIdx.y * S * WB);
    const unsigned lane16 = (unsigned)lane * 16u;

    const bool grp_a = wave < NA, grp_b = !STAG || wave >= NA;
    const int wb = STAG ? wave - NA : wave;
    auto dma_weight = [&](int step, int wbuf, int k) {
        const int e = wb + NB * k;
        if (e < NEW) dma_buf16(srd_w, lane16, (unsigned)(step * WB + e * 1024), lds0 + WOFF + wbuf * WB + e * 1024);
    };
    auto dma_patch = [&](int chunk, int slice, int pbuf, int k) {
        const int d = wave + NA * k;
        if (d < ND) dma_buf16(srd_x, pvoff[k], (unsigned)(slice * nchunk + chunk) * a.plane_bytes, lds0 + pbuf * PB + slice * PSL + d * 1024);
    };
    auto issue_weights = [&](int step, int wbuf) {
        if (grp_b) {
#pragma unroll
            for (int k = 0; k < NEWW; ++k) dma_weight(step, wbuf, k);
        }
    };
    auto issue_patch = [&](int chunk, int slice, int pbuf) {
        if (grp_a) {
#pragma unroll
            for (int k = 0; k < NDW; ++k) dma_patch(chunk, slice, pbuf, k);
        }
    };

    f32x16 acc[CLS][TM][TN];
#pragma unroll
    for (int cl = 0; cl < CLS; ++cl)
#pragma unroll
        for (int i = 0; i < TM; ++i)
#pragma unroll
            for (int j = 0; j < TN; ++j)
#pragma unroll
                for (int e = 0; e < 16; ++e) acc[cl][i][j][e] = 0.f;

    lds_cptr const L = (lds_cptr)lds_x3;
    struct Frag { u32x4 X[TM][3], W[TN][3]; };
    auto load_frags = [&](auto pbufc, auto wbufc, auto tc, Frag& f) {
        constexpr int pbuf = decltype(pbufc)::value, wbuf = decltype(wbufc)::value, t = decltype(tc)::value;
#pragma unroll
        for (int s = 0; s < 3; ++s) {
#pragma unroll
            for (int j = 0; j < TN; ++j)
                f.W[j][s] = *reinterpret_cast<const __attribute__((address_space(3))) u32x4*>(
                    L + waddr + (WOFF + wbuf * WB + (((t % 3) * 3 + s) * BN + 32 * j) * 32));
#pragma unroll
            for (int i = 0; i < TM; ++i)
                f.X[i][s] = *reinterpret_cast<const __attribute__((address_space(3))) u32x4*>(L + xaddr[i][t] + (pbuf * PB + s * PSL));
        }
    };
    auto mfma_frags = [&](const Frag& f, auto tc, auto&& between) {
        constexpr int t = decltype(tc)::value;
        constexpr int cl = CLS == 4 ? (t / 3 != 1) * 2 + (t % 3 != 1) : 0;
#pragma unroll
        for (int p = 0; p < 6; ++p) {
            constexpr int WS[6] = {0, 0, 0, 1, 1, 2}, XS[6] = {2, 1, 0, 1, 0, 0};
#pragma unroll
            for (int i = 0; i < TM; ++i)
#pragma unroll
                for (int j = 0; j < TN; ++j) acc[cl][i][j] = mfma_bf16(f.W[j][WS[p]], f.X[i][XS[p]], acc[cl][i][j]);
            between(p);
        }
    };
    auto nothing = [](int) {};
    constexpr int NRD = 3 * (TM + TN), NMF = 6 * TM * TN;
    auto interleave = [&]() {
#pragma unroll
        for (int k = 0; k < NRD; ++k) {
            __builtin_amdgcn_sched_group_barrier(0x008, 1, 0);
            __builtin_amdgcn_sched_group_barrier(0x100, 1, 0);
        }
        __builtin_amdgcn_sched_group_barrier(0x008, NMF - NRD, 0);
    };
    const bool dma_on = !(DMC_ABL(a.ablate) & 64);
    auto step = [&](auto pbufc, auto wbufc, auto qc, Frag& FA, Frag& FB, int c) {
        constexpr int pbuf = decltype(pbufc)::value, wbuf = decltype(wbufc)::value, q = decltype(qc)::value;
        using NP = std::integral_constant<int, q == 2 ? (pbuf ^ 1) : pbuf>;
        using NWB = std::integral_constant<int, wbuf ^ 1>;
        using NT = std::integral_constant<int, q == 2 ? 0 : 3 * (q + 1)>;
        using T0 = std::integral_constant<int, 3 * q>;
        using T1 = std::integral_constant<int, 3 * q + 1>;
        using T2 = std::integral_constant<int, 3 * q + 2>;
        const int s = 3 * c + q;
        load_frags(pbufc, wbufc, std::integral_constant<int, 3 * q + 1>{}, FB);
        if constexpr (STAG) {
            const bool go = grp_b && dma_on && s + 1 < S;
            mfma_frags(FA, T0{}, [&](int p) {
                if (go) {
#pragma unroll
                    for (int k = p; k < NEWW; k += 6) dma_weight(s + 1, wbuf ^ 1, k);
                }
            });
        } else {
            mfma_frags(FA, T0{}, nothing);
            interleave();
        }
        load_frags(pbufc, wbufc, std::integral_constant<int, 3 * q + 2>{}, FA);
        mfma_frags(FB, T1{}, nothing);
        interleave();
        if (DMC_ABL(a.ablate) & 16) asm volatile("s_waitcnt lgkmcnt(0)" ::: "memory");
        else asm volatile("s_waitcnt vmcnt(0) lgkmcnt(0)" ::: "memory");
        __builtin_amdgcn_s_barrier();
        const int vc = q == 2 ? c + 2 : c + 1;
        if constexpr (STAG) {
            if (s + 1 < S) load_frags(NP{}, NWB{}, NT{}, FB);
            const bool go = grp_a && dma_on && vc < nchunk;
            mfma_frags(FA, T2{}, [&](int p) {
                if (go) {
#pragma unroll
                    for (int k = p; k < NDW; k += 6) dma_patch(vc, q == 2 ? 0 : q + 1, q == 2 ? pbuf : (pbuf ^ 1), k);
                }
            });
        } else {
            if (dma_on) {
                if (s + 2 < S) issue_weights(s + 2, wbuf);
                if (vc < nchunk) issue_patch(vc, q == 2 ? 0 : q + 1, q == 2 ? pbuf : (pbuf ^ 1));
            }
            if (s + 1 < S) load_frags(NP{}, NWB{}, NT{}, FB);
            mfma_frags(FA, T2{}, nothing);
        }
    };
    using I0 = std::integral_constant<int, 0>;
    using I1 = std::integral_constant<int, 1>;
    using Q0 = std::integral_constant<int, 0>;
    using Q1 = std::integral_constant<int, 1>;
    using Q2 = std::integral_constant<int, 2>;

    if (tid < 12)
        *reinterpret_cast<float4*>(lds_x3 + (tid >> 1) * PSL + ZROW * 32 + (tid & 1) * 16) = make_float4(0.f, 0.f, 0.f, 0.f);
    issue_weights(0, 0);
    issue_patch(0, 0, 0); issue_patch(0, 1, 0); issue_patch(0, 2, 0);
    asm volatile("s_waitcnt vmcnt(0)" ::: "memory");
    __builtin_amdgcn_s_barrier();
    if (dma_on) {
        if (!STAG && S > 1) issue_weights(1, 1);
        if (nchunk > 1) issue_patch(1, 0, 1);
    }
    Frag F0, F1;
    load_frags(I0{}, I0{}, Q0{}, F0);
#pragma unroll 1
    for (int c = 0; c < ((DMC_ABL(a.ablate) & 256) ? 0 : nchunk); c += 2) {
        step(I0{}, I0{}, Q0{}, F0, F1, c);
        step(I0{}, I1{}, Q1{}, F1, F0, c);
        step(I0{}, I0{}, Q2{}, F0, F1, c);
        step(I1{}, I1{}, Q0{}, F1, F0, c + 1);
        step(I1{}, I0{}, Q1{}, F0, F1, c + 1);
        step(I1{}, I1{}, Q2{}, F1, F0, c + 1);
    }

    static_assert(WN == 1 && TN == 2, "epilogue: a wave owns all 64 channels of its pixels");
    constexpr int EP = 272, ETILE = 32 * TM * EP;
    char* etile = lds_x3 + wave * ETILE;
    const int mw0 = m0 + wm * TM * 32;
    const int rbase = blockIdx.y * BN;
#pragma unroll
    for (int cl = 0; cl < CLS; ++cl) {
#pragma unroll
        for (int i = 0; i < TM; ++i) {
            const bool ok = mw0 + 32 * i + l31 <= mlast;
#pragma unroll
            for (int j = 0; j < TN; ++j)
#pragma unroll
                for (int g = 0; g < 4; ++g) {
                    float4 v = make_float4(acc[cl][i][j][4 * g], acc[cl][i][j][4 * g + 1], acc[cl][i][j][4 * g + 2], acc[cl][i][j][4 * g + 3]);
                    if (!ok) v = make_float4(0.f, 0.f, 0.f, 0.f);
                    *reinterpret_cast<float4*>(etile + (32 * i + l31) * EP + (32 * j + 8 * g + 4 * khalf) * 4) = v;
                }
        }
        if constexpr (EVAL) {
            const int c4 = rbase + (lane & 15) * 4;
            const float4 mean = *reinterpret_cast<const float4*>(a.stats + c4), istd = *reinterpret_cast<const float4*>(a.stats + a.R + c4);
            const float4 gm = *reinterpret_cast<const float4*>(a.gamma + c4), bt = *reinterpret_cast<const float4*>(a.beta + c4);
            const bool has_res = a.res != nullptr, relu = a.relu != 0;
            const int ochunk = a.R >> 4;
#pragma unroll
            for (int it = 0; it < 8 * TM; ++it) {
                const int prow = 4 * it + (lane >> 4);
                const int m = mw0 + prow;
                const float4 v = *reinterpret_cast<const float4*>(etile + prow * EP + (lane & 15) * 16);
                if (m <= mlast) {
                    const size_t o = (size_t)m * a.R + c4;
                    float4 rv = make_float4(0.f, 0.f, 0.f, 0.f);
                    if (has_res) rv = *reinterpret_cast<const float4*>(a.res + o);
                    const float w[4] = {bn_apply_act1(v.x, mean.x, istd.x, gm.x, bt.x, has_res, rv.x, relu),
                                        bn_apply_act1(v.y, mean.y, istd.y, gm.y, bt.y, has_res, rv.y, relu),
                                        bn_apply_act1(v.z, mean.z, istd.z, gm.z, bt.z, has_res, rv.z, relu),
                                        bn_apply_act1(v.w, mean.w, istd.w, gm.w, bt.w, has_res, rv.w, relu)};
                    if (a.y) *reinterpret_cast<float4*>(a.y + o) = make_float4(w[0], w[1], w[2], w[3]);
                    if (a.ys) {
                        if (a.s2d) {
                            const int n = m / HW, rem = m - n * HW, yy = rem / a.W, xx = rem - yy * a.W;
                            const int cls = (yy & 1) * 2 + (xx & 1);
                            const size_t mq = ((size_t)n * (a.H >> 1) + (yy >> 1)) * (a.W >> 1) + (xx >> 1);
                            x3s_store4(a.ys, w, (size_t)a.M >> 2, 4 * ochunk, mq, (c4 >> 2) + cls * 4 * ochunk);
                        } else {
                            x3s_store4(a.ys, w, (size_t)a.M, ochunk, (size_t)m, c4 >> 2);
                        }
                    }
                }
            }
        } else
        if (!(DMC_ABL(a.ablate) & 128)) {
#pragma unroll
            for (int it = 0; it < 8 * TM; ++it) {
                const int prow = 4 * it + (lane >> 4);
                const int m = mw0 + prow;
                float4 v = *reinterpret_cast<const float4*>(etile + prow * EP + (lane & 15) * 16);
                if (m <= mlast) {
                    size_t opix = (size_t)m;
                    if (CLS == 4) {
                        const int n = m / HW, rem = m - n * HW, ya = rem / a.W, xb = rem - ya * a.W;
                        opix = ((size_t)n * (2 * a.H) + 2 * ya + (cl >> 1)) * (2 * a.W) + 2 * xb + (cl & 1);
                    }
                    const size_t o = opix * a.R + rbase + (lane & 15) * 4;
                    if (a.addend) {
                        const float4 av = *reinterpret_cast<const float4*>(a.addend + o);
                        v.x += av.x; v.y += av.y; v.z += av.z; v.w += av.w;
                    }
                    *reinterpret_cast<float4*>(a.y + o) = v;
                    if (CLS == 1 && a.bnb_part) {
                        const int c4 = rbase + (lane & 15) * 4;
                        const float4 yv = *reinterpret_cast<const float4*>(a.bnb_y + o);
                        const float4 mean = *reinterpret_cast<const float4*>(a.bnb_stats + c4);
                        const float4 istd = *reinterpret_cast<const float4*>(a.bnb_stats + a.R + c4);
                        const float4 xh = make_float4((yv.x - mean.x) * istd.x, (yv.y - mean.y) * istd.y, (yv.z - mean.z) * istd.z, (yv.w - mean.w) * istd.w);
                        if (a.bnb_relu) {
                            unsigned mb;
                            if (a.bnb_mask) {
                                mb = a.bnb_mask[o >> 2];
                            } else {
                                const float4 g = *reinterpret_cast<const float4*>(a.bnb_gamma + c4), b = *reinterpret_cast<const float4*>(a.bnb_beta + c4);
                                mb = (fmaf(xh.x, g.x, b.x) > 0.f ? 1u : 0u) | (fmaf(xh.y, g.y, b.y) > 0.f ? 2u : 0u) |
                                     (fmaf(xh.z, g.z, b.z) > 0.f ? 4u : 0u) | (fmaf(xh.w, g.w, b.w) > 0.f ? 8u : 0u);
                            }
                            v.x = (mb & 1) ? v.x : 0.f; v.y = (mb & 2) ? v.y : 0.f; v.z = (mb & 4) ? v.z : 0.f; v.w = (mb & 8) ? v.w : 0.f;
                        }
                        *reinterpret_cast<float4*>(etile + prow * EP + (lane & 15) * 16) = v;
                        *reinterpret_cast<float4*>(etile + NW * ETILE + 8192 + prow * EP + (lane & 15) * 16) = xh;
                    }
                } else if (CLS == 1 && a.bnb_part) {
                    *reinterpret_cast<float4*>(etile + prow * EP + (lane & 15) * 16) = make_float4(0.f, 0.f, 0.f, 0.f);
                    *reinterpret_cast<float4*>(etile + NW * ETILE + 8192 + prow * EP + (lane & 15) * 16) = make_float4(0.f, 0.f, 0.f, 0.f);
                }
            }
        }
    }
    if constexpr (EVAL) return;
    if (CLS == 1 && a.bnb_part) {
        double* red = reinterpret_cast<double*>(lds_x3 + NW * ETILE);
        const char* xtile = etile + NW * ETILE + 8192;
        double d1 = 0.0, d2 = 0.0;
#pragma unroll 8
        for (int p = 0; p < 32 * TM; ++p) {
            const double d = (double)*reinterpret_cast<const float*>(etile + p * EP + lane * 4);
            const double xh = (double)*reinterpret_cast<const float*>(xtile + p * EP + lane * 4);
            d1 += d;
            d2 += d * xh;
        }
        red[(wm * 64 + lane) * 2 + 0] = d1;
        red[(wm * 64 + lane) * 2 + 1] = d2;
        __syncthreads();
        for (int cc = tid; cc < BN; cc += NW * 64) {
            double e1 = 0.0, e2 = 0.0;
#pragma unroll
            for (int w = 0; w < WM; ++w) { e1 += red[(w * 64 + cc) * 2 + 0]; e2 += red[(w * 64 + cc) * 2 + 1]; }
            double* dst = a.bnb_part + ((size_t)blockIdx.x * a.R + rbase + cc) * 2;
            dst[0] = e1; dst[1] = e2;
        }
    }
    if (CLS == 1 && a.stat_part) {
        double* red = reinterpret_cast<double*>(lds_x3 + NW * ETILE);
        double d1 = 0.0, d2 = 0.0;
#pragma unroll 8
        for (int p = 0; p < 32 * TM; ++p) {
            const double v = (double)*reinterpret_cast<const float*>(etile + p * EP + lane * 4);
            d1 += v;
            d2 += v * v;
        }
        red[(wm * 64 + lane) * 2 + 0] = d1;
        red[(wm * 64 + lane) * 2 + 1] = d2;
        __syncthreads();
        for (int c = tid; c < BN; c += NW * 64) {
            double e1 = 0.0, e2 = 0.0;
#pragma unroll
            for (int w = 0; w < WM; ++w) { e1 += red[(w * 64 + c) * 2 + 0]; e2 += red[(w * 64 + c) * 2 + 1]; }
            double* dst = a.stat_part + ((size_t)blockIdx.x * a.R + rbase + c) * 2;
            dst[0] = e1; dst[1] = e2;
        }
    }
}

int patch_pixels_max(int N, int H, int W, int BM) {
    const long M = (long)N * H * W;
    int worst = 0;
    long tiles = (M + BM - 1) / BM;
    if (tiles > W) tiles = W;
    for (long t = 0; t < tiles; ++t) {
        const long m0 = t * BM, ml = (m0 + BM < M ? m0 + BM : M) - 1;
        const long r0 = m0 / W, r1 = ml / W;
        const long f0 = (r0 > 0 ? r0 - 1 : 0) * W, f1 = (r1 + 2) * W;
        if ((int)(f1 - f0) + 1 > worst) worst = (int)(f1 - f0) + 1;
    }
    return worst;
}

struct X3Cfg { int id, BM, PPMAX, threads; };
constexpr X3Cfg X3CFGS[] = {{0, 256, 608, 512}, {1, 128, 320, 256}, {2, 64, 192, 128}, {3, 256, 608, 256}, {4, 128, 225, 256}};

bool x3s_shape_ok(int N, int H, int W, int K, int R) {
    if (N <= 0 || H <= 0 || W <= 0 || K % 32 != 0 || R % 64 != 0 || K <= 0 || R <= 0) return false;
    const long M = (long)N * H * W;
    return M * (K > R ? K : R) * 6 < (1L << 31);
}

int x3s_choose(int N, int H, int W, int R) {
    const long M = (long)N * H * W;
    const int forced = option(OPT_CONV_CFG);
    if (forced >= 101 && forced <= 105 && patch_pixels_max(N, H, W, X3CFGS[forced - 101].BM) <= X3CFGS[forced - 101].PPMAX) return forced - 101;
    if (forced != 106 && patch_pixels_max(N, H, W, X3CFGS[4].BM) <= X3CFGS[4].PPMAX && ((M + X3CFGS[4].BM - 1) / X3CFGS[4].BM) * (R / 64) >= 512)
        return 4;
    int fallback = -1;
    for (const X3Cfg& c : X3CFGS) {
        if (c.id > 2 || patch_pixels_max(N, H, W, c.BM) > c.PPMAX) continue;
        const long wgs = ((M + c.BM - 1) / c.BM) * (R / 64);
        if (wgs >= 160) return c.id;
        fallback = c.id;
    }
    return fallback;
}

template <int WM, int TM, int PPMAX>
int launch_x3s(const X3Args& a, hipStream_t s) {
    constexpr int BM = 32 * TM * WM;
    constexpr size_t op_bytes = 2 * 3 * PPMAX * 32 + 2 * 3 * 3 * 64 * 32, ep_bytes = 2 * (size_t)BM * 272 + 8192;
    constexpr size_t lds_bytes = op_bytes > ep_bytes ? op_bytes : ep_bytes;
    dim3 grid((a.M + BM - 1) / BM, a.R / 64);
    if ((a.stat_part || a.bnb_part) && a.part_blocks >= 0 && (unsigned)a.part_blocks != grid.x)
        return fail(DMC_E_INVALID, "x3s_conv: statistics partials have %d rows but this launch writes %u (dmc_x3s_conv_stat_blocks was "
                                   "called under another conv_cfg option?)", a.part_blocks, grid.x);
    if constexpr (WM >= 4) {
        if (!(option(OPT_CONV_ABLATE) & 512)) {
            static LdsLimit lim_attr2;
    const hipError_t attr2 = lim_attr2.raise(reinterpret_cast<const void*>(&x3s_conv_kernel<WM, 1, TM, 2, PPMAX, true>), (int)lds_bytes);
            if (attr2 != hipSuccess) return fail(DMC_E_LAUNCH, "x3s_conv: cannot raise the dynamic LDS limit: %s", hipGetErrorString(attr2));
            x3s_conv_kernel<WM, 1, TM, 2, PPMAX, true><<<grid, WM * 64, lds_bytes, s>>>(a);
            return check_launch("x3s_conv");
        }
    }
    static LdsLimit lim_attr;
    const hipError_t attr = lim_attr.raise(reinterpret_cast<const void*>(&x3s_conv_kernel<WM, 1, TM, 2, PPMAX>), (int)lds_bytes);
    if (attr != hipSuccess) return fail(DMC_E_LAUNCH, "x3s_conv: cannot raise the dynamic LDS limit: %s", hipGetErrorString(attr));
    x3s_conv_kernel<WM, 1, TM, 2, PPMAX><<<grid, WM * 64, lds_bytes, s>>>(a);
    return check_launch("x3s_conv");
}

struct X3Bnb { const float *y, *stats, *gamma, *beta; const unsigned char* mask; int relu; double* part; };

int run_x3s(const void* xs, const void* wp, const float* addend, float* y, double* stat_part, int part_blocks, int N, int H, int W,
            int K, int R, hipStream_t s, const X3Bnb* bnb = nullptr) {
    if (!xs || !wp || !y) return fail(DMC_E_INVALID, "x3s_conv: null pointer");
    if (!x3s_shape_ok(N, H, W, K, R)) return fail(DMC_E_INVALID, "x3s_conv: unsupported shape N=%d H=%d W=%d K=%d R=%d", N, H, W, K, R);
    const int cfg = x3s_choose(N, H, W, R);
    X3Args a;
    a.xs = xs; a.wp = wp; a.y = y; a.addend = addend; a.stat_part = stat_part;
    a.N = N; a.H = H; a.W = W; a.K = K; a.R = R; a.M = N * H * W;
    a.plane_bytes = (unsigned)a.M * 32u;
    a.part_blocks = part_blocks;
    if ((stat_part || bnb) && part_blocks <= 0) return fail(DMC_E_INVALID, "x3s_conv: stat_blocks must be the row count of the partials");
    if (bnb) {
        a.bnb_y = bnb->y; a.bnb_stats = bnb->stats; a.bnb_gamma = bnb->gamma; a.bnb_beta = bnb->beta; a.bnb_mask = bnb->mask;
        a.bnb_relu = bnb->relu; a.bnb_part = bnb->part;
    }
    a.ablate = option(OPT_CONV_ABLATE);
    if (DMC_ABL(a.ablate) & 32) a.stat_part = nullptr;
    switch (cfg) {
        case 0: return launch_x3s<8, 1, 608>(a, s);
        case 1: return launch_x3s<4, 1, 320>(a, s);
        case 2: return launch_x3s<2, 1, 192>(a, s);
        case 3: return launch_x3s<4, 2, 608>(a, s);
        case 4: return launch_x3s<4, 1, 225>(a, s);
        default: return fail(DMC_E_INVALID, "x3s_conv: the patch of a %d x %d image does not fit the LDS", H, W);
    }
}

template <int WM, int TM, int PPMAX>
int launch_x3s_eval(const X3EvalArgs& a, hipStream_t s) {
    constexpr int BM = 32 * TM * WM;
    constexpr size_t lds_bytes = 2 * 3 * PPMAX * 32 + 2 * 3 * 3 * 64 * 32;
    static_assert((size_t)BM * 272 <= lds_bytes, "the epilogue tiles live in the operand LDS");
    dim3 grid((a.M + BM - 1) / BM, a.R / 64);
    static LdsLimit lim_attr;
    const hipError_t attr = lim_attr.raise(reinterpret_cast<const void*>(&x3s_conv_kernel<WM, 1, TM, 2, PPMAX, (WM >= 4), 1, true>), (int)lds_bytes);
    if (attr != hipSuccess) return fail(DMC_E_LAUNCH, "x3s_conv_bn_eval: cannot raise the dynamic LDS limit: %s", hipGetErrorString(attr));
    x3s_conv_kernel<WM, 1, TM, 2, PPMAX, (WM >= 4), 1, true><<<grid, WM * 64, lds_bytes, s>>>(a);
    return check_launch("x3s_conv_bn_eval");
}

struct X3WgArgs {
    const void* xs;
    const void* dys;
    float* part;
    int N, H, Cin, Cout;
    unsigned plane_bytes;
    int steps, per_group, tiles_ci;
};

template <int W_, int R>
struct WgGeom {
    static constexpr int PW = W_ + 2;
    static constexpr int NGRP = R >= W_ + 2 ? 2 : 4, LA = NGRP / 2;
    static constexpr int NRING = NGRP * R;
    static constexpr int XPX = NRING * PW;
    static constexpr int XPL = ((XPX + 3) / 8) * 8 + 4;
    static constexpr int NPX = R * W_;
    static constexpr int NKB = (NPX + 15) / 16;
    static constexpr int DYP = NKB * 16;
    static constexpr int DYT = ((DYP + 31) / 32) * 32;
    static constexpr int DYPL = ((DYT + 3) / 8) * 8 + 4;
    static constexpr int XI = (R * PW + 31) / 32;
    static constexpr int DI = DYT / 32;
    static constexpr int XBYTES = 12 * XPL * 32, DYBYTES = 12 * DYPL * 32;
    static constexpr int LDS = XBYTES + 2 * DYBYTES;
};

template <int W_, int R>
__global__ __launch_bounds__(768) void x3s_wgrad_kernel(X3WgArgs a) {
    using G = WgGeom<W_, R>;
    constexpr int PW = G::PW, NRING = G::NRING, XPL = G::XPL, DYPL = G::DYPL, NKB = G::NKB;
    extern __shared__ __attribute__((aligned(1024))) char lds_wg[];
    const int tid = threadIdx.x, lane = tid & 63;
    const int wave = __builtin_amdgcn_readfirstlane(tid >> 6);
    const int l31 = lane & 31, khalf = lane >> 5, L = lane & 15, grp = (lane >> 4) & 1;
    const int quarter = wave & 3, trow = wave >> 2;
    const int wi = quarter & 1, wj = quarter >> 1;
    const int tci = blockIdx.x % a.tiles_ci, tco = blockIdx.x / a.tiles_ci;
    const unsigned lds0 = lds_addr_of(lds_wg);
    const int HP = a.H + 2;
    const int s_begin = blockIdx.y * a.per_group;
    const int s_end = s_begin + a.per_group < a.steps ? s_begin + a.per_group : a.steps;
    const u32x4 srd_x = make_srd(a.xs), srd_d = make_srd(a.dys);
    const unsigned soff_x = (unsigned)((wave >> 2) * (a.Cin >> 4) + tci * 4 + (wave & 3)) * a.plane_bytes;
    const unsigned soff_d = (unsigned)((wave >> 2) * (a.Cout >> 4) + tco * 4 + (wave & 3)) * a.plane_bytes;
    const unsigned xplane = lds0 + (unsigned)wave * XPL * 32, dplane = lds0 + G::XBYTES + (unsigned)wave * DYPL * 32;
    const int lpx = lane >> 1;
    const unsigned lhalf = (unsigned)(lane & 1) << 4;

    const unsigned img_bytes = (unsigned)(a.H * W_) * 32u;
    unsigned xpre[G::XI], dpre[G::DI];
#pragma unroll
    for (int i = 0; i < G::XI; ++i) {
        const int px = 32 * i + lpx;
        const int r = px / PW, col = px - r * PW - 1;
        xpre[i] = (col >= 0 && col < W_) ? (unsigned)(r * W_ + col) * 32u + lhalf : NOPIX;
    }
#pragma unroll
    for (int i = 0; i < G::DI; ++i) {
        const int p = 32 * i + lpx;
        dpre[i] = p < G::NPX ? (unsigned)p * 32u + lhalf : NOPIX;
    }
    auto issue_x = [&](int q, const WgGroupPos& g) {
        const int slot0 = (((q % G::NGRP) + G::NGRP) % G::NGRP) * R;
        unsigned tbase, img_off;
        wg_group_base(g, a.N, W_, img_bytes, tbase, img_off);
#pragma unroll
        for (int i = 0; i < G::XI; ++i)
            if (32 * i + lpx < R * PW)
                dma_buf16(srd_x, wg_lane_off(tbase, xpre[i], img_bytes), soff_x + img_off, xplane + (unsigned)(slot0 * PW + 32 * i) * 32u);
    };
    auto issue_dy = [&](const WgGroupPos& g, int buf) {
        unsigned tbase, img_off;
        wg_group_base(g, a.N, W_, img_bytes, tbase, img_off);
#pragma unroll
        for (int i = 0; i < G::DI; ++i)
            dma_buf16(srd_d, wg_lane_off(tbase, dpre[i], img_bytes), soff_d + img_off, dplane + (unsigned)buf * G::DYBYTES + (unsigned)(32 * i) * 32u);
    };

    f32x16 acc[3];
#pragma unroll
    for (int t = 0; t < 3; ++t)
#pragma unroll
        for (int e = 0; e < 16; ++e) acc[t][e] = 0.f;

    WgGroupPos g1 = wg_group_at(s_begin, R, HP);
    if (s_begin < s_end) {
        WgGroupPos g = wg_group_prev(g1, R, HP);
#pragma unroll
        for (int q = -1; q < G::LA; ++q, g = wg_group_next(g, R, HP)) issue_x(s_begin + q, g);
        issue_dy(g1, 0);
    }
    g1 = wg_group_next(g1, R, HP);
    asm volatile("s_waitcnt vmcnt(0)" ::: "memory");
    __builtin_amdgcn_s_barrier();
    lds_cptr const LB = (lds_cptr)lds_wg;
    int rr[NKB][2], xcol[NKB][2], dyoff[NKB][2];
#pragma unroll
    for (int kb = 0; kb < NKB; ++kb)
#pragma unroll
        for (int u = 0; u < 2; ++u) {
            int P = 16 * kb + 8 * khalf + 4 * u + (L >> 2);
            dyoff[kb][u] = (2 * wi + grp) * DYPL * 32 + G::XBYTES + (L & 3) * 8 + P * 32;
            if (P >= G::NPX) P = G::NPX - 1;
            rr[kb][u] = P / W_;
            xcol[kb][u] = (2 * wj + grp) * XPL * 32 + (L & 3) * 8 + (P - rr[kb][u] * W_) * 32;
        }
#pragma unroll 1
    for (int s = s_begin; s < s_end; ++s) {
        const int buf = (s - s_begin) & 1;
        issue_x(s + G::LA, G::LA == 1 ? g1 : wg_group_next(g1, R, HP));
        if (s + 1 < s_end) issue_dy(g1, buf ^ 1);
        g1 = wg_group_next(g1, R, HP);
        const int sb = (((R * s + trow - 1) % NRING) + NRING) % NRING;
#pragma unroll
        for (int kb = 0; kb < NKB; ++kb) {
            int dyo[2], xo[2];
#pragma unroll
            for (int u = 0; u < 2; ++u) {
                dyo[u] = dyoff[kb][u] + buf * G::DYBYTES;
                int slot = sb + rr[kb][u];
                slot = slot >= NRING ? slot - NRING : slot;
                xo[u] = xcol[kb][u] + slot * PW * 32;
            }
            u32x4 A[3], B[3][3];
#pragma unroll
            for (int sl = 0; sl < 3; ++sl) {
                tr_read2(LB + dyo[0] + sl * 4 * DYPL * 32, LB + dyo[1] + sl * 4 * DYPL * 32, A[sl]);
#pragma unroll
                for (int t = 0; t < 3; ++t)
                    tr_read2(LB + xo[0] + (sl * 4 * XPL + t) * 32, LB + xo[1] + (sl * 4 * XPL + t) * 32, B[t][sl]);
            }
#pragma unroll
            for (int t = 0; t < 3; ++t) {
                acc[t] = mfma_bf16(A[0], B[t][2], acc[t]);
                acc[t] = mfma_bf16(A[2], B[t][0], acc[t]);
                acc[t] = mfma_bf16(A[1], B[t][1], acc[t]);
                acc[t] = mfma_bf16(A[0], B[t][1], acc[t]);
                acc[t] = mfma_bf16(A[1], B[t][0], acc[t]);
                acc[t] = mfma_bf16(A[0], B[t][0], acc[t]);
            }
        }
        asm volatile("s_waitcnt vmcnt(0) lgkmcnt(0)" ::: "memory");
        __builtin_amdgcn_s_barrier();
    }
    float* out = a.part + (size_t)blockIdx.y * a.Cout * 9 * a.Cin;
    const int ci = tci * 64 + 32 * wj + l31;
#pragma unroll
    for (int t = 0; t < 3; ++t)
#pragma unroll
        for (int e = 0; e < 16; ++e) {
            const int co = tco * 64 + 32 * wi + 8 * (e >> 2) + 4 * khalf + (e & 3);
            out[((size_t)co * 9 + 3 * trow + t) * a.Cin + ci] = acc[t][e];
        }
}

__global__ __launch_bounds__(256) void x3s_wgrad_reduce_kernel(const float* __restrict__ part, float* __restrict__ dw, int ngroup, long numel) {
    __shared__ float4 red[16][17];
    const int o = threadIdx.x & 15, sl = threadIdx.x >> 4;
    for (long i0 = (long)blockIdx.x * 64; i0 < numel; i0 += (long)gridDim.x * 64) {
        const long i = i0 + 4 * o;
        float4 s = make_float4(0.f, 0.f, 0.f, 0.f);
        if (i < numel)
            for (int k = sl; k < ngroup; k += 16) {
                const float4 v = *reinterpret_cast<const float4*>(part + (size_t)k * numel + i);
                s.x += v.x; s.y += v.y; s.z += v.z; s.w += v.w;
            }
        red[sl][o] = s;
        __syncthreads();
        if (sl == 0 && i < numel) {
            float4 t = red[0][o];
#pragma unroll
            for (int k = 1; k < 16; ++k) { const float4 v = red[k][o]; t.x += v.x; t.y += v.y; t.z += v.z; t.w += v.w; }
            *reinterpret_cast<float4*>(dw + i) = t;
        }
        __syncthreads();
    }
}

struct X3WgPlan { int R, steps, tiles, groups, per_group; };
bool x3s_wgrad_plan(int N, int H, int W, int Cin, int Cout, X3WgPlan& p) {
    p.R = W == 56 ? 1 : W == 28 ? 2 : W == 14 ? 4 : W == 7 ? 9 : 0;
    if (!p.R || (H + 2) % p.R != 0 || (W == 7 && H != 7) || Cin % 64 != 0 || Cout % 64 != 0) return false;
    p.steps = N * (H + 2) / p.R;
    p.tiles = (Cout / 64) * (Cin / 64);
    int groups = 256 / p.tiles;
    if (groups < 1) groups = 1;
    if (groups > p.steps) groups = p.steps;
    p.per_group = (p.steps + groups - 1) / groups;
    p.groups = (p.steps + p.per_group - 1) / p.per_group;
    return true;
}

template <int W_, int R>
int launch_x3s_wgrad(const X3WgPlan& p, X3WgArgs a, float* dw, hipStream_t s) {
    using G = WgGeom<W_, R>;
    static_assert(G::LDS <= 160 * 1024, "weight-gradient tiles exceed the LDS");
    static LdsLimit lim_attr;
    const hipError_t attr = lim_attr.raise(reinterpret_cast<const void*>(&x3s_wgrad_kernel<W_, R>), G::LDS);
    if (attr != hipSuccess) return fail(DMC_E_LAUNCH, "x3s_wgrad: cannot raise the dynamic LDS limit: %s", hipGetErrorString(attr));
    x3s_wgrad_kernel<W_, R><<<dim3(p.tiles, p.groups), 768, G::LDS, s>>>(a);
    int rc = check_launch("x3s_wgrad");
    if (rc || p.groups == 1) return rc;
    const long numel = (long)a.Cout * 9 * a.Cin;
    const long blocks = (numel + 63) / 64;
    x3s_wgrad_reduce_kernel<<<(int)(blocks > 4096 ? 4096 : blocks), 256, 0, s>>>(a.part, dw, p.groups, numel);
    return check_launch("x3s_wgrad_reduce");
}

__global__ __launch_bounds__(256) void x3s_bnb_final_kernel(const double* __restrict__ part, int nblk, int C,
                                                            float* __restrict__ dgamma, float* __restrict__ dbeta) {
    __shared__ double red[2][4];
    const int c = blockIdx.x, lane = threadIdx.x & 63, wave = threadIdx.x >> 6;
    double s = 0.0, ss = 0.0;
    for (int b = threadIdx.x; b < nblk; b += 256) {
        const double2 v = *reinterpret_cast<const double2*>(part + ((size_t)b * C + c) * 2);
        s += v.x;
        ss += v.y;
    }
#pragma unroll
    for (int o = 32; o > 0; o >>= 1) { s += __shfl_down(s, o, 64); ss += __shfl_down(ss, o, 64); }
    if (lane == 0) { red[0][wave] = s; red[1][wave] = ss; }
    __syncthreads();
    if (threadIdx.x != 0) return;
    dbeta[c] = (float)(red[0][0] + red[0][1] + red[0][2] + red[0][3]);
    dgamma[c] = (float)(red[1][0] + red[1][1] + red[1][2] + red[1][3]);
}

int stream_blocks(long total) {
    long b = (total + 255) / 256;
    return (int)(b < 1 ? 1 : (b > 8192 ? 8192 : b));
}

}

extern "C" {

size_t dmc_x3s_slices_bytes(long M, int C) { return (size_t)M * (size_t)C * 6; }

int dmc_x3s_split(const float* x, void* xs, long M, int C, dmc_stream_t stream) {
    if (!x || !xs || M <= 0 || C <= 0 || C % 16 != 0) return fail(DMC_E_INVALID, "dmc_x3s_split: bad argument");
    x3s_split_kernel<<<stream_blocks(M * (C / 8)), 256, 0, (hipStream_t)stream>>>(x, static_cast<unsigned short*>(xs), M, C);
    return check_launch("x3s_split");
}

int dmc_x3s_merge(const void* xs, float* x, long M, int C, dmc_stream_t stream) {
    if (!x || !xs || M <= 0 || C <= 0 || C % 16 != 0) return fail(DMC_E_INVALID, "dmc_x3s_merge: bad argument");
    x3s_merge_kernel<<<stream_blocks(M * C), 256, 0, (hipStream_t)stream>>>(static_cast<const unsigned short*>(xs), x, M, C);
    return check_launch("x3s_merge");
}

size_t dmc_x3s_wpack_bytes(int Cin, int Cout) { return (size_t)Cin * (size_t)Cout * 9 * 6; }

int dmc_x3s_pack_weights(const float* w, void* wpack_f, void* wpack_t, int Cin, int Cout, dmc_stream_t stream) {
    if (!w || (!wpack_f && !wpack_t) || Cin % 64 != 0 || Cout % 64 != 0 || Cin <= 0 || Cout <= 0)
        return fail(DMC_E_INVALID, "dmc_x3s_pack_weights: bad argument");
    const long total = (long)Cin * Cout * 9;
    x3s_pack_w_kernel<<<dim3(stream_blocks(total) > 1024 ? 1024 : stream_blocks(total), 2), 256, 0, (hipStream_t)stream>>>(
        w, static_cast<unsigned short*>(wpack_f), static_cast<unsigned short*>(wpack_t), Cout, Cin, 1);
    return check_launch("x3s_pack_w");
}

int dmc_x3s_conv_supported(int N, int H, int W, int Cin, int Cout) {
    return Cin % 64 == 0 && Cout % 64 == 0 && x3s_shape_ok(N, H, W, Cin, Cout) && x3s_shape_ok(N, H, W, Cout, Cin) &&
           x3s_choose(N, H, W, Cout) >= 0 && x3s_choose(N, H, W, Cin) >= 0 ? 1 : 0;
}

int dmc_x3s_conv_stat_blocks(int N, int H, int W, int Cout) {
    const int cfg = x3s_choose(N, H, W, Cout);
    if (cfg < 0) return 0;
    const long M = (long)N * H * W;
    return (int)((M + X3CFGS[cfg].BM - 1) / X3CFGS[cfg].BM);
}

int dmc_x3s_conv_fwd(const void* xs, const void* wpack_f, float* y, double* stat_partials, int stat_blocks, int N, int H, int W,
                     int Cin, int Cout, dmc_stream_t stream) {
    return run_x3s(xs, wpack_f, nullptr, y, stat_partials, stat_blocks, N, H, W, Cin, Cout, (hipStream_t)stream);
}

int dmc_x3s_conv_bn_eval(const void* xs, const void* wpack_f, const float* stats, const float* gamma, const float* beta,
                         const float* residual, float* y, void* ys, int s2d, int relu, int N, int H, int W, int Cin, int Cout,
                         dmc_stream_t stream) {
    if (!xs || !wpack_f || !stats || !gamma || !beta) return fail(DMC_E_INVALID, "dmc_x3s_conv_bn_eval: null pointer");
    if (!y && !ys) return fail(DMC_E_INVALID, "dmc_x3s_conv_bn_eval: no output (y and ys are both null)");
    if (s2d && !ys) return fail(DMC_E_INVALID, "dmc_x3s_conv_bn_eval: s2d describes the slice output, which is null");
    if (s2d && ((H & 1) || (W & 1))) return fail(DMC_E_INVALID, "dmc_x3s_conv_bn_eval: a space-to-depth result needs even H and W (H=%d W=%d)", H, W);
    if (Cin % 64 != 0 || Cout % 64 != 0 || !x3s_shape_ok(N, H, W, Cin, Cout) || !x3s_shape_ok(N, H, W, Cout, Cin))
        return fail(DMC_E_INVALID, "dmc_x3s_conv_bn_eval: unsupported shape N=%d H=%d W=%d Cin=%d Cout=%d", N, H, W, Cin, Cout);
    X3EvalArgs a;
    a.xs = xs; a.wp = wpack_f; a.y = y; a.addend = nullptr; a.stat_part = nullptr;
    a.N = N; a.H = H; a.W = W; a.K = Cin; a.R = Cout; a.M = N * H * W;
    a.plane_bytes = (unsigned)a.M * 32u;
    a.ablate = 0;
    a.stats = stats; a.gamma = gamma; a.beta = beta; a.res = residual; a.ys = static_cast<unsigned short*>(ys);
    a.s2d = s2d ? 1 : 0; a.relu = relu ? 1 : 0;
    hipStream_t s = (hipStream_t)stream;
    switch (x3s_choose(N, H, W, Cout)) {
        case 0: return launch_x3s_eval<8, 1, 608>(a, s);
        case 1: return launch_x3s_eval<4, 1, 320>(a, s);
        case 2: return launch_x3s_eval<2, 1, 192>(a, s);
        case 3: return launch_x3s_eval<4, 2, 608>(a, s);
        case 4: return launch_x3s_eval<4, 1, 225>(a, s);
        default: return fail(DMC_E_INVALID, "dmc_x3s_conv_bn_eval: the patch of a %d x %d image does not fit the LDS", H, W);
    }
}

int dmc_x3s_conv_dgrad(const void* dys, const void* wpack_t, const float* addend, float* dx, int N, int H, int W, int Cin, int Cout,
                       dmc_stream_t stream) {
    return run_x3s(dys, wpack_t, addend, dx, nullptr, -1, N, H, W, Cout, Cin, (hipStream_t)stream);
}

int dmc_x3s_conv_wgrad_supported(int N, int H, int W, int Cin, int Cout) {
    X3WgPlan p;
    return x3s_wgrad_plan(N, H, W, Cin, Cout, p) && x3s_shape_ok(N, H, W, Cin, Cout) && x3s_shape_ok(N, H, W, Cout, Cin) ? 1 : 0;
}

size_t dmc_x3s_conv_wgrad_bytes(int N, int H, int W, int Cin, int Cout) {
    X3WgPlan p;
    if (!x3s_wgrad_plan(N, H, W, Cin, Cout, p) || p.groups <= 1) return 0;
    return (size_t)p.groups * Cout * 9 * Cin * sizeof(float);
}

int dmc_x3s_conv_wgrad(const void* xs, const void* dys, float* dw, float* workspace, int N, int H, int W, int Cin, int Cout,
                       dmc_stream_t stream) {
    X3WgPlan p;
    if (!xs || !dys || !dw) return fail(DMC_E_INVALID, "dmc_x3s_conv_wgrad: null pointer");
    if (!dmc_x3s_conv_wgrad_supported(N, H, W, Cin, Cout) || !x3s_wgrad_plan(N, H, W, Cin, Cout, p))
        return fail(DMC_E_INVALID, "dmc_x3s_conv_wgrad: unsupported shape N=%d H=%d W=%d Cin=%d Cout=%d", N, H, W, Cin, Cout);
    if (p.groups > 1 && !workspace) return fail(DMC_E_INVALID, "dmc_x3s_conv_wgrad: workspace required");
    X3WgArgs a;
    a.xs = xs; a.dys = dys; a.part = p.groups > 1 ? workspace : dw;
    a.N = N; a.H = H; a.Cin = Cin; a.Cout = Cout;
    a.plane_bytes = (unsigned)((long)N * H * W) * 32u;
    a.steps = p.steps; a.per_group = p.per_group; a.tiles_ci = Cin / 64;
    hipStream_t s = (hipStream_t)stream;
    switch (W) {
        case 56: return launch_x3s_wgrad<56, 1>(p, a, dw, s);
        case 28: return launch_x3s_wgrad<28, 2>(p, a, dw, s);
        case 14: return launch_x3s_wgrad<14, 4>(p, a, dw, s);
        default: return launch_x3s_wgrad<7, 9>(p, a, dw, s);
    }
}

int dmc_x3s_conv_dgrad_s2_supported(int N, int OH, int OW, int Cin, int Cout) {
    return Cin % 64 == 0 && Cout % 64 == 0 && x3s_shape_ok(N, OH, OW, Cout, Cin) && (long)N * OH * OW * 4 * Cin * 4 < (1L << 40) &&
           patch_pixels_max(N, OH, OW, 128) <= 320 ? 1 : 0;
}

int dmc_x3s_pack_weights_s2(const float* w, void* wpack_t2, int Cin, int Cout, dmc_stream_t stream) {
    if (!w || !wpack_t2 || Cin % 64 != 0 || Cout % 64 != 0 || Cin <= 0 || Cout <= 0)
        return fail(DMC_E_INVALID, "dmc_x3s_pack_weights_s2: bad argument");
    const long total = (long)Cin * Cout * 9;
    x3s_pack_w_kernel<<<dim3(stream_blocks(total) > 1024 ? 1024 : stream_blocks(total), 2), 256, 0, (hipStream_t)stream>>>(
        w, nullptr, static_cast<unsigned short*>(wpack_t2), Cout, Cin, 0);
    return check_launch("x3s_pack_w_s2");
}

int dmc_x3s_conv_dgrad_s2(const void* dys, const void* wpack_t2, float* dx, int N, int OH, int OW, int Cin, int Cout,
                          dmc_stream_t stream) {
    if (!dys || !wpack_t2 || !dx) return fail(DMC_E_INVALID, "dmc_x3s_conv_dgrad_s2: null pointer");
    if (!dmc_x3s_conv_dgrad_s2_supported(N, OH, OW, Cin, Cout))
        return fail(DMC_E_INVALID, "dmc_x3s_conv_dgrad_s2: unsupported shape N=%d OH=%d OW=%d Cin=%d Cout=%d", N, OH, OW, Cin, Cout);
    X3Args a;
    a.xs = dys; a.wp = wpack_t2; a.y = dx; a.addend = nullptr; a.stat_part = nullptr;
    a.N = N; a.H = OH; a.W = OW; a.K = Cout; a.R = Cin; a.M = N * OH * OW;
    a.plane_bytes = (unsigned)a.M * 32u;
    a.ablate = option(OPT_CONV_ABLATE);
    constexpr size_t lds_bytes = 2 * 3 * 320 * 32 + 2 * 3 * 3 * 64 * 32;
    static LdsLimit lim_attr;
    const hipError_t attr = lim_attr.raise(reinterpret_cast<const void*>(&x3s_conv_kernel<4, 1, 1, 2, 320, true, 4>), (int)lds_bytes);
    if (attr != hipSuccess) return fail(DMC_E_LAUNCH, "x3s_conv_dgrad_s2: cannot raise the dynamic LDS limit: %s", hipGetErrorString(attr));
    dim3 grid((a.M + 127) / 128, Cin / 64);
    x3s_conv_kernel<4, 1, 1, 2, 320, true, 4><<<grid, 256, lds_bytes, (hipStream_t)stream>>>(a);
    return check_launch("x3s_conv_dgrad_s2");
}

int dmc_x3s_conv_dgrad_bnb(const void* dys, const void* wpack_t, const float* addend, float* dx, const float* bn_y,
                           const float* bn_stats, const float* bn_gamma, const float* bn_beta, const unsigned char* bn_relu_mask,
                           int bn_relu, double* partials, int stat_blocks, float* dgamma, float* dbeta, int N, int H, int W, int Cin,
                           int Cout, dmc_stream_t stream) {
    if (!bn_y || !bn_stats || !bn_gamma || !bn_beta || !partials || !dgamma || !dbeta)
        return fail(DMC_E_INVALID, "dmc_x3s_conv_dgrad_bnb: null pointer");
    X3Bnb b = {bn_y, bn_stats, bn_gamma, bn_beta, bn_relu_mask, bn_relu, partials};
    int rc = run_x3s(dys, wpack_t, addend, dx, nullptr, stat_blocks, N, H, W, Cout, Cin, (hipStream_t)stream, &b);
    if (rc) return rc;
    x3s_bnb_final_kernel<<<Cin, 256, 0, (hipStream_t)stream>>>(partials, stat_blocks, Cin, dgamma, dbeta);
    return check_launch("x3s_bnb_final");
}

}
```

### dmc-net_amd/csrc/dmc_common.h

```cpp
#pragma once
#include <hip/hip_runtime.h>
#include <stdarg.h>
#include <stdio.h>

#include <atomic>

#include "dmcnet_hip.h"

namespace dmc {

inline char* err_buf() {
    static thread_local char buf[512] = {0};
    return buf;
}
inline int fail(int code, const char* fmt, ...) {
    va_list ap;
    va_start(ap, fmt);
    vsnprintf(err_buf(), 512, fmt, ap);
    va_end(ap);
    return code;
}
inline int check_launch(const char* what) {
    hipError_t e = hipGetLastError();
    if (e != hipSuccess) return fail(DMC_E_LAUNCH, "%s: %s", what, hipGetErrorString(e));
    return DMC_OK;
}

struct LdsLimit {
    std::atomic<unsigned long long> raised{0};
    hipError_t raise(const void* kernel, int bytes) {
        int dev = 0;
        hipError_t e = hipGetDevice(&dev);
        if (e != hipSuccess) return e;
        if (dev >= 0 && dev < 64 && ((raised.load(std::memory_order_relaxed) >> dev) & 1ull)) return hipSuccess;
        e = hipFuncSetAttribute(kernel, hipFuncAttributeMaxDynamicSharedMemorySize, bytes);
        if (e == hipSuccess && dev >= 0 && dev < 64) raised.fetch_or(1ull << dev, std::memory_order_relaxed);
        return e;
    }
};

enum Option { OPT_GEN_LAYER_PATH = 0, OPT_GEN_GATHER, OPT_GEN_FUSE45, OPT_GEN_WGRAD_PATH, OPT_GEN_FUSE_FWD,
              OPT_GEN_FUSE_BWD, OPT_GEN_FRAMES, OPT_CONV_PATH, OPT_CONV_CFG, OPT_CONV_ABLATE, OPT_GEN_ABLATE, OPT_CONV_ARITH, OPT_CONV3D_WGRAD, OPT_GEN_X3, OPT_GEN_WINO, OPT_GEN_STAGGER, OPT_GEN_FUSED, OPT_GRID_RESERVE_CUS, OPT_COUNT };
int option(Option o);
inline int persistent_cus(int hw) {
    const int r = option(OPT_GRID_RESERVE_CUS);
    int n = hw - (r > 0 ? r : 0);
    n -= n % 8;
    return n < 8 ? (hw < 8 ? hw : 8) : n;
}
#ifdef DMC_MEASURE
#define DMC_ABL(x) (x)
constexpr bool MEASURE_BUILD = true;
#else
#define DMC_ABL(x) 0
constexpr bool MEASURE_BUILD = false;
#endif
constexpr bool measure_only(int o) { return o == OPT_GEN_ABLATE || o == OPT_CONV_ABLATE || o == OPT_GEN_STAGGER; }
constexpr bool product_value(int o, int v) {
    return o == OPT_GEN_FUSED ? (v == 0 || v == 1) : o == OPT_GEN_LAYER_PATH ? (v == 0 || v == 1)
         : o == OPT_GEN_WGRAD_PATH ? (v == 4 || v == 5) : true;
}

constexpr int NL = 6;
__host__ __device__ constexpr int cin_of(int k) {
    return k == 0 ? 5 : k == 1 ? 13 : k == 2 ? 21 : k == 3 ? 27 : k == 4 ? 31 : 33;
}
__host__ __device__ constexpr int cout_of(int k) {
    return k == 0 ? 8 : k == 1 ? 8 : k == 2 ? 6 : k == 3 ? 4 : 2;
}
__host__ __device__ constexpr int yoff(int k) { return cin_of(k); }
constexpr int NFEAT = 28;
constexpr int NIN = 5;

__host__ __device__ constexpr int wf_off(int k) {
    int o = 0;
    for (int i = 0; i < k; ++i) o += cin_of(i) * 9 * cout_of(i);
    return o;
}
constexpr int WF_TOTAL = wf_off(6);
__host__ __device__ constexpr int bf_off(int k) {
    int o = WF_TOTAL;
    for (int i = 0; i < k; ++i) o += cout_of(i);
    return o;
}
constexpr int NPARAM = bf_off(6);
__host__ __device__ constexpr int gin_of(int j) { return 35 - yoff(j + 1); }
__host__ __device__ constexpr int wb_off(int j) {
    int o = NPARAM;
    for (int i = 0; i < j; ++i) o += gin_of(i) * 9 * cout_of(i);
    return o;
}
constexpr int PACKED_TOTAL = wb_off(5);
constexpr int ZERO_PAD = 256;
constexpr int BN_MAX_SPLIT = 1024;

__host__ __device__ inline int logical_of(int k, int p) {
    if (p < NIN) return (cin_of(k) - NIN) + p;
    int j = 0;
    while (p >= yoff(j) + cout_of(j)) ++j;
    int l = 0;
    for (int i = j + 1; i < k; ++i) l += cout_of(i);
    return l + (p - yoff(j));
}

struct ParamPtrs {
    const float* w[NL];
    const float* b[NL];
};
struct GradPtrs {
    float* w[NL];
    float* b[NL];
};

}

namespace dmc {
typedef __attribute__((address_space(3))) void* lds_ptr_t;
typedef float mfma_f32x4 __attribute__((ext_vector_type(4)));
__device__ __forceinline__ unsigned lds_addr_of(const void* p) { return (unsigned)(size_t)(lds_ptr_t)p; }
__device__ __forceinline__ void lds_dma16(unsigned long long sbase, unsigned voff, unsigned lds_byte_addr) {
    asm volatile("s_mov_b32 m0, %2\n\ts_nop 0\n\tglobal_load_lds_dwordx4 %0, %1"
                 :: "v"(voff), "s"(sbase), "s"(__builtin_amdgcn_readfirstlane(lds_byte_addr)) : "memory");
}
}

namespace dmc {
template <int CTRL, int ROW_MASK>
__device__ __forceinline__ double dpp_f64(double v) {
    const int lo = __builtin_amdgcn_update_dpp(0, __double2loint(v), CTRL, ROW_MASK, 0xf, false);
    const int hi = __builtin_amdgcn_update_dpp(0, __double2hiint(v), CTRL, ROW_MASK, 0xf, false);
    return __hiloint2double(hi, lo);
}
__device__ __forceinline__ double row16_sum(double v) {
    v += dpp_f64<0x128, 0xf>(v);
    v += dpp_f64<0x124, 0xf>(v);
    v += dpp_f64<0x122, 0xf>(v);
    v += dpp_f64<0x121, 0xf>(v);
    return v;
}
__device__ __forceinline__ double half32_sum_hi(double v) {
    v = row16_sum(v);
    v += dpp_f64<0x142, 0xa>(v);
    return v;
}
}

namespace dmc {
struct BnEval { const float* gamma; const float* beta; const float* mean; const float* var; float eps; };
__device__ __forceinline__ void bn_eval_affine(const BnEval& b, int C, int c, float* scale, float* shift) {
    float sc = 0.f, sh = 0.f;
    if (c < C) {
        sc = b.gamma[c] / sqrtf(b.var[c] + b.eps);
        const float ms = b.mean[c] * sc;
        sh = b.beta[c] - ms;
    }
    scale[c] = sc;
    shift[c] = sh;
}
}

namespace dmc {
typedef unsigned x3s_u32x4 __attribute__((ext_vector_type(4)));
__device__ __forceinline__ void x3s_split3(float v, unsigned& u0, unsigned& u1, unsigned& u2) {
    u0 = __float_as_uint(v);
    const float r1 = v - __uint_as_float(u0 & 0xffff0000u);
    u1 = __float_as_uint(r1);
    u2 = __float_as_uint(r1 - __uint_as_float(u1 & 0xffff0000u));
}
__device__ __forceinline__ void x3s_store8(unsigned short* __restrict__ xs, const float (&v)[8], size_t M, int nchunk, size_t m, int g) {
    unsigned u0[8], u1[8], u2[8];
#pragma unroll
    for (int e = 0; e < 8; ++e) x3s_split3(v[e], u0[e], u1[e], u2[e]);
    x3s_u32x4 s0, s1, s2;
#pragma unroll
    for (int e = 0; e < 4; ++e) {
        s0[e] = __builtin_amdgcn_perm(u0[2 * e + 1], u0[2 * e], 0x07060302u);
        s1[e] = __builtin_amdgcn_perm(u1[2 * e + 1], u1[2 * e], 0x07060302u);
        s2[e] = __builtin_amdgcn_perm(u2[2 * e + 1], u2[2 * e], 0x07060302u);
    }
    const size_t plane = M * 16;
    const size_t w = ((size_t)(g >> 1) * M + m) * 16 + (size_t)(g & 1) * 8;
    *reinterpret_cast<x3s_u32x4*>(xs + w) = s0;
    *reinterpret_cast<x3s_u32x4*>(xs + (size_t)nchunk * plane + w) = s1;
    *reinterpret_cast<x3s_u32x4*>(xs + (size_t)2 * nchunk * plane + w) = s2;
}
typedef unsigned x3s_u32x2 __attribute__((ext_vector_type(2)));
__device__ __forceinline__ void x3s_store4(unsigned short* __restrict__ xs, const float (&v)[4], size_t M, int nchunk, size_t m, int q) {
    unsigned u0[4], u1[4], u2[4];
#pragma unroll
    for (int e = 0; e < 4; ++e) x3s_split3(v[e], u0[e], u1[e], u2[e]);
    x3s_u32x2 s0, s1, s2;
#pragma unroll
    for (int e = 0; e < 2; ++e) {
        s0[e] = __builtin_amdgcn_perm(u0[2 * e + 1], u0[2 * e], 0x07060302u);
        s1[e] = __builtin_amdgcn_perm(u1[2 * e + 1], u1[2 * e], 0x07060302u);
        s2[e] = __builtin_amdgcn_perm(u2[2 * e + 1], u2[2 * e], 0x07060302u);
    }
    const size_t plane = M * 16;
    const size_t w = ((size_t)(q >> 2) * M + m) * 16 + (size_t)(q & 3) * 4;
    *reinterpret_cast<x3s_u32x2*>(xs + w) = s0;
    *reinterpret_cast<x3s_u32x2*>(xs + (size_t)nchunk * plane + w) = s1;
    *reinterpret_cast<x3s_u32x2*>(xs + (size_t)2 * nchunk * plane + w) = s2;
}

__device__ __forceinline__ float bn_apply_act1(float x, float mean, float istd, float gamma, float beta, bool has_res, float res, bool relu) {
    float v = fmaf((x - mean) * istd, gamma, beta);
    if (has_res) v += res;
    if (relu) v = fmaxf(v, 0.f);
    return v;
}
}
```

### dmc-net_amd/csrc/losses.hip

```cpp
#include <atomic>
#include <string.h>

#include "dmc_common.h"

using namespace dmc;

namespace {

constexpr int MSE_BLOCKS = 2048;

__device__ __forceinline__ double wave_sum(double v) {
#pragma unroll
    for (int o = 32; o > 0; o >>= 1) v += __shfl_down(v, o, 64);
    return v;
}
__device__ __forceinline__ float wave_sum(float v) {
#pragma unroll
    for (int o = 32; o > 0; o >>= 1) v += __shfl_down(v, o, 64);
    return v;
}
__device__ __forceinline__ float wave_max(float v) {
#pragma unroll
    for (int o = 32; o > 0; o >>= 1) v = fmaxf(v, __shfl_down(v, o, 64));
    return v;
}

__global__ __launch_bounds__(256) void flow_mse_partial_kernel(const float* __restrict__ a,
                                                               const float* __restrict__ b,
                                                               double* __restrict__ partials,
                                                               size_t numel) {
    __shared__ double sm[4];
    const size_t n4 = numel / 4;
    const float4* a4 = reinterpret_cast<const float4*>(a);
    const float4* b4 = reinterpret_cast<const float4*>(b);
    float s0 = 0.f, s1 = 0.f, s2 = 0.f, s3 = 0.f;
    for (size_t i = (size_t)blockIdx.x * 256 + threadIdx.x; i < n4; i += (size_t)gridDim.x * 256) {
        const float4 x = a4[i], y = b4[i];
        const float d0 = x.x - y.x, d1 = x.y - y.y, d2 = x.z - y.z, d3 = x.w - y.w;
        s0 = fmaf(d0, d0, s0); s1 = fmaf(d1, d1, s1); s2 = fmaf(d2, d2, s2); s3 = fmaf(d3, d3, s3);
    }
    double s = (double)s0 + (double)s1 + (double)s2 + (double)s3;
    if (blockIdx.x == 0 && threadIdx.x == 0)
        for (size_t i = n4 * 4; i < numel; ++i) { const double d = (double)a[i] - (double)b[i]; s += d * d; }
    s = wave_sum(s);
    if ((threadIdx.x & 63) == 0) sm[threadIdx.x >> 6] = s;
    __syncthreads();
    if (threadIdx.x == 0) partials[blockIdx.x] = sm[0] + sm[1] + sm[2] + sm[3];
}

__global__ void flow_mse_final_kernel(const double* __restrict__ partials, int nblocks,
                                      float* __restrict__ loss_out, size_t numel) {
    __shared__ double sm[4];
    double s = 0.0;
    for (int i = threadIdx.x; i < nblocks; i += 256) s += partials[i];
    s = wave_sum(s);
    if ((threadIdx.x & 63) == 0) sm[threadIdx.x >> 6] = s;
    __syncthreads();
    if (threadIdx.x == 0) *loss_out = (float)((sm[0] + sm[1] + sm[2] + sm[3]) / (double)numel);
}

__global__ __launch_bounds__(256) void flow_mse_bwd_kernel(const float* __restrict__ a,
                                                           const float* __restrict__ b,
                                                           const float* __restrict__ grad_loss,
                                                           float* __restrict__ ga, size_t numel) {
    const float scale = 2.f * (*grad_loss) / (float)numel;
    const size_t n4 = numel / 4;
    const float4* a4 = reinterpret_cast<const float4*>(a);
    const float4* b4 = reinterpret_cast<const float4*>(b);
    float4* g4 = reinterpret_cast<float4*>(ga);
    for (size_t i = (size_t)blockIdx.x * 256 + threadIdx.x; i < n4; i += (size_t)gridDim.x * 256) {
        const float4 x = a4[i], y = b4[i];
        g4[i] = make_float4((x.x - y.x) * scale, (x.y - y.y) * scale, (x.z - y.z) * scale,
                            (x.w - y.w) * scale);
    }
    if (blockIdx.x == 0 && threadIdx.x == 0)
        for (size_t i = n4 * 4; i < numel; ++i) ga[i] = (a[i] - b[i]) * scale;
}

template <bool ATT>
__device__ __forceinline__ float loss_diff(float g, float f, float t) {
    return ATT ? __fsub_rn(__fmul_rn(t, g), __fmul_rn(t, f)) : g - f;
}
template <int KIND>
__device__ __forceinline__ float loss_term(float d) {
    if constexpr (KIND == 0) return d * d;
    const float ad = fabsf(d);
    if constexpr (KIND == 1) return ad < 1.f ? 0.5f * d * d : ad - 0.5f;
    return ad;
}
template <int KIND>
__device__ __forceinline__ float loss_deriv(float d) {
    const float sg = (float)(d > 0.f) - (float)(d < 0.f);
    if constexpr (KIND == 0) return 2.f * d;
    if constexpr (KIND == 1) return fabsf(d) < 1.f ? d : sg;
    return sg;
}

template <int KIND, bool ATT>
__global__ __launch_bounds__(256) void flow_loss_partial_kernel(const float* __restrict__ a, const float* __restrict__ b,
                                                                const float* __restrict__ t, double* __restrict__ partials,
                                                                size_t numel) {
    __shared__ double sm[4];
    const size_t n4 = numel / 4;
    const float4* a4 = reinterpret_cast<const float4*>(a);
    const float4* b4 = reinterpret_cast<const float4*>(b);
    const float4* t4 = reinterpret_cast<const float4*>(t);
    float s0 = 0.f, s1 = 0.f, s2 = 0.f, s3 = 0.f;
    for (size_t i = (size_t)blockIdx.x * 256 + threadIdx.x; i < n4; i += (size_t)gridDim.x * 256) {
        const float4 x = a4[i], y = b4[i];
        float4 w = make_float4(1.f, 1.f, 1.f, 1.f);
        if constexpr (ATT) w = t4[i];
        s0 += loss_term<KIND>(loss_diff<ATT>(x.x, y.x, w.x));
        s1 += loss_term<KIND>(loss_diff<ATT>(x.y, y.y, w.y));
        s2 += loss_term<KIND>(loss_diff<ATT>(x.z, y.z, w.z));
        s3 += loss_term<KIND>(loss_diff<ATT>(x.w, y.w, w.w));
    }
    double s = (double)s0 + (double)s1 + (double)s2 + (double)s3;
    if (blockIdx.x == 0 && threadIdx.x == 0)
        for (size_t i = n4 * 4; i < numel; ++i) s += (double)loss_term<KIND>(loss_diff<ATT>(a[i], b[i], ATT ? t[i] : 1.f));
    s = wave_sum(s);
    if ((threadIdx.x & 63) == 0) sm[threadIdx.x >> 6] = s;
    __syncthreads();
    if (threadIdx.x == 0) partials[blockIdx.x] = sm[0] + sm[1] + sm[2] + sm[3];
}

template <int KIND, bool ATT, bool GATT>
__global__ __launch_bounds__(256) void flow_loss_bwd_kernel(const float* __restrict__ a, const float* __restrict__ b,
                                                            const float* __restrict__ t, const float* __restrict__ grad_loss,
                                                            float* __restrict__ ga, float* __restrict__ gt, size_t numel) {
    const float scale = (*grad_loss) / (float)numel;
    const size_t n4 = numel / 4;
    const float4* a4 = reinterpret_cast<const float4*>(a);
    const float4* b4 = reinterpret_cast<const float4*>(b);
    const float4* t4 = reinterpret_cast<const float4*>(t);
    float4* ga4 = reinterpret_cast<float4*>(ga);
    float4* gt4 = reinterpret_cast<float4*>(gt);
    auto one = [&](float x, float y, float w, float& gx, float& gw) {
        const float g = loss_deriv<KIND>(loss_diff<ATT>(x, y, w)) * scale;
        gx = ATT ? __fmul_rn(g, w) : g;
        if constexpr (GATT) gw = __fsub_rn(__fmul_rn(x, g), __fmul_rn(y, g));
    };
    for (size_t i = (size_t)blockIdx.x * 256 + threadIdx.x; i < n4; i += (size_t)gridDim.x * 256) {
        const float4 x = a4[i], y = b4[i];
        float4 w = make_float4(1.f, 1.f, 1.f, 1.f), gx, gw;
        if constexpr (ATT) w = t4[i];
        one(x.x, y.x, w.x, gx.x, gw.x);
        one(x.y, y.y, w.y, gx.y, gw.y);
        one(x.z, y.z, w.z, gx.z, gw.z);
        one(x.w, y.w, w.w, gx.w, gw.w);
        ga4[i] = gx;
        if constexpr (GATT) gt4[i] = gw;
    }
    if (blockIdx.x == 0 && threadIdx.x == 0)
        for (size_t i = n4 * 4; i < numel; ++i) {
            float gx, gw;
            one(a[i], b[i], ATT ? t[i] : 1.f, gx, gw);
            ga[i] = gx;
            if constexpr (GATT) gt[i] = gw;
        }
}

template <int KIND>
int launch_flow_loss_partial(const float* a, const float* b, const float* t, double* part, size_t numel, int blocks, hipStream_t s) {
    if (t) flow_loss_partial_kernel<KIND, true><<<blocks, 256, 0, s>>>(a, b, t, part, numel);
    else flow_loss_partial_kernel<KIND, false><<<blocks, 256, 0, s>>>(a, b, t, part, numel);
    return check_launch("flow_loss_partial");
}
template <int KIND>
int launch_flow_loss_bwd(const float* a, const float* b, const float* t, const float* gl, float* ga, float* gt, size_t numel,
                         int blocks, hipStream_t s) {
    if (t && gt) flow_loss_bwd_kernel<KIND, true, true><<<blocks, 256, 0, s>>>(a, b, t, gl, ga, gt, numel);
    else if (t) flow_loss_bwd_kernel<KIND, true, false><<<blocks, 256, 0, s>>>(a, b, t, gl, ga, gt, numel);
    else flow_loss_bwd_kernel<KIND, false, false><<<blocks, 256, 0, s>>>(a, b, t, gl, ga, gt, numel);
    return check_launch("flow_loss_bwd");
}

__global__ __launch_bounds__(1024) void consensus_ce_kernel(const float* __restrict__ logits,
                                                            const int64_t* __restrict__ target,
                                                            float* __restrict__ consensus,
                                                            float* __restrict__ loss_out,
                                                            float* __restrict__ grad, int B, int S,
                                                            int C) {
    __shared__ float wave_loss[16];
    const int wave = threadIdx.x >> 6, lane = threadIdx.x & 63;
    const float inv_s = 1.f / (float)S, inv_n = 1.f / ((float)B * (float)S);
    float loss = 0.f;
    for (int b = wave; b < B; b += 16) {
        const float* lb = logits + (size_t)b * S * C;
        float mx = -INFINITY;
        for (int c = lane; c < C; c += 64) {
            float a = 0.f;
            for (int s = 0; s < S; ++s) a += lb[(size_t)s * C + c];
            a *= inv_s;
            consensus[(size_t)b * C + c] = a;
            mx = fmaxf(mx, a);
        }
        mx = __shfl(wave_max(mx), 0, 64);
        float se = 0.f;
        for (int c = lane; c < C; c += 64) {
            float a = 0.f;
            for (int s = 0; s < S; ++s) a += lb[(size_t)s * C + c];
            se += expf(a * inv_s - mx);
        }
        se = __shfl(wave_sum(se), 0, 64);
        const float log_se = logf(se), inv_se = 1.f / se;
        const int64_t t64 = target[b];
        const bool t_ok = t64 >= 0 && t64 < (int64_t)C;
        const int t = t_ok ? (int)t64 : 0;
        if (lane == 0) {
            float a = 0.f;
            for (int s = 0; s < S; ++s) a += lb[(size_t)s * C + t];
            loss += t_ok ? log_se + (mx - a * inv_s) : NAN;
        }
        if (grad != nullptr) {
            for (int c = lane; c < C; c += 64) {
                float a = 0.f;
                for (int s = 0; s < S; ++s) a += lb[(size_t)s * C + c];
                const float p = expf(a * inv_s - mx) * inv_se;
                const float g = t_ok ? (p - (c == t ? 1.f : 0.f)) * inv_n : NAN;
                for (int s = 0; s < S; ++s) grad[((size_t)b * S + s) * C + c] = g;
            }
        }
    }
    if (lane == 0) wave_loss[wave] = loss;
    __syncthreads();
    if (threadIdx.x == 0) {
        float s = 0.f;
        for (int w = 0; w < 16; ++w) s += wave_loss[w];
        *loss_out = s / (float)B;
    }
}

const char* const OPTION_NAMES[OPT_COUNT] = {"gen_layer_path", "gen_gather", "gen_fuse45", "gen_wgrad_path",
                                             "gen_fuse_fwd", "gen_fuse_bwd", "gen_frames", "conv_path", "conv_cfg", "conv_ablate", "gen_ablate", "conv_arith", "conv3d_wgrad", "gen_x3", "gen_wino", "gen_stagger", "gen_fused", "grid_reserve_cus"};
std::atomic<int> g_options[OPT_COUNT] = {{1}, {1}, {1}, {5}, {1}, {1}, {0}, {1}, {0}, {0}, {0}, {1}, {2}, {2}, {768}, {0}, {1}, {0}};
int option_index(const char* name) {
    if (!name) return -1;
    for (int i = 0; i < OPT_COUNT; ++i)
        if (strcmp(name, OPTION_NAMES[i]) == 0) return i;
    return -1;
}

}

namespace dmc {
int option(Option o) { return !MEASURE_BUILD && measure_only(o) ? 0 : g_options[o].load(std::memory_order_relaxed); }
}

__global__ void dmc_profile_mark_kernel() {}

extern "C" {

size_t dmc_flow_mse_partials_bytes(void) { return (size_t)MSE_BLOCKS * sizeof(double); }

int dmc_flow_mse_fwd(const float* gen_flow, const float* flow, float* loss_out, float* partials,
                     size_t numel, dmc_stream_t stream) {
    if (!gen_flow || !flow || !loss_out || !partials || numel == 0)
        return fail(DMC_E_INVALID, "dmc_flow_mse_fwd: null pointer or empty tensor");
    hipStream_t s = (hipStream_t)stream;
    size_t want = (numel / 4 + 255) / 256;
    const int blocks = (int)(want < 1 ? 1 : (want > MSE_BLOCKS ? MSE_BLOCKS : want));
    flow_mse_partial_kernel<<<blocks, 256, 0, s>>>(gen_flow, flow, (double*)partials, numel);
    int rc = check_launch("flow_mse_partial");
    if (rc) return rc;
    flow_mse_final_kernel<<<1, 256, 0, s>>>((const double*)partials, blocks, loss_out, numel);
    return check_launch("flow_mse_final");
}

int dmc_flow_mse_bwd(const float* gen_flow, const float* flow, const float* grad_loss,
                     float* grad_gen, size_t numel, dmc_stream_t stream) {
    if (!gen_flow || !flow || !grad_loss || !grad_gen || numel == 0)
        return fail(DMC_E_INVALID, "dmc_flow_mse_bwd: null pointer or empty tensor");
    size_t want = (numel / 4 + 255) / 256;
    const int blocks = (int)(want < 1 ? 1 : (want > 4096 ? 4096 : want));
    flow_mse_bwd_kernel<<<blocks, 256, 0, (hipStream_t)stream>>>(gen_flow, flow, grad_loss, grad_gen, numel);
    return check_launch("flow_mse_bwd");
}

size_t dmc_flow_loss_partials_bytes(void) { return dmc_flow_mse_partials_bytes(); }

int dmc_flow_loss_fwd(int kind, const float* gen_flow, const float* flow, const float* att, float* loss_out, float* partials,
                      size_t numel, dmc_stream_t stream) {
    if (kind < 0 || kind > 2) return fail(DMC_E_INVALID, "dmc_flow_loss_fwd: kind %d (0 = MSE, 1 = SmoothL1, 2 = L1)", kind);
    if (!gen_flow || !flow || !loss_out || !partials || numel == 0)
        return fail(DMC_E_INVALID, "dmc_flow_loss_fwd: null pointer or empty tensor");
    if (kind == 0 && !att) return dmc_flow_mse_fwd(gen_flow, flow, loss_out, partials, numel, stream);
    hipStream_t s = (hipStream_t)stream;
    size_t want = (numel / 4 + 255) / 256;
    const int blocks = (int)(want < 1 ? 1 : (want > MSE_BLOCKS ? MSE_BLOCKS : want));
    double* part = (double*)partials;
    int rc = kind == 0 ? launch_flow_loss_partial<0>(gen_flow, flow, att, part, numel, blocks, s)
           : kind == 1 ? launch_flow_loss_partial<1>(gen_flow, flow, att, part, numel, blocks, s)
                       : launch_flow_loss_partial<2>(gen_flow, flow, att, part, numel, blocks, s);
    if (rc) return rc;
    flow_mse_final_kernel<<<1, 256, 0, s>>>(part, blocks, loss_out, numel);
    return check_launch("flow_loss_final");
}

int dmc_flow_loss_bwd(int kind, const float* gen_flow, const float* flow, const float* att, const float* grad_loss,
                      float* grad_gen, float* grad_att, size_t numel, dmc_stream_t stream) {
    if (kind < 0 || kind > 2) return fail(DMC_E_INVALID, "dmc_flow_loss_bwd: kind %d (0 = MSE, 1 = SmoothL1, 2 = L1)", kind);
    if (!gen_flow || !flow || !grad_loss || !grad_gen || numel == 0)
        return fail(DMC_E_INVALID, "dmc_flow_loss_bwd: null pointer or empty tensor");
    if (grad_att && !att) return fail(DMC_E_INVALID, "dmc_flow_loss_bwd: grad_att given without att");
    if (kind == 0 && !att) return dmc_flow_mse_bwd(gen_flow, flow, grad_loss, grad_gen, numel, stream);
    hipStream_t s = (hipStream_t)stream;
    size_t want = (numel / 4 + 255) / 256;
    const int blocks = (int)(want < 1 ? 1 : (want > 4096 ? 4096 : want));
    return kind == 0 ? launch_flow_loss_bwd<0>(gen_flow, flow, att, grad_loss, grad_gen, grad_att, numel, blocks, s)
         : kind == 1 ? launch_flow_loss_bwd<1>(gen_flow, flow, att, grad_loss, grad_gen, grad_att, numel, blocks, s)
                     : launch_flow_loss_bwd<2>(gen_flow, flow, att, grad_loss, grad_gen, grad_att, numel, blocks, s);
}

int dmc_consensus_ce_fwd_bwd(const float* logits, const int64_t* target, float* consensus,
                             float* loss_out, float* grad_logits, int B, int S, int C,
                             dmc_stream_t stream) {
    if (!logits || !target || !consensus || !loss_out)
        return fail(DMC_E_INVALID, "dmc_consensus_ce_fwd_bwd: null pointer");
    if (B <= 0 || S <= 0 || C <= 0) return fail(DMC_E_INVALID, "dmc_consensus_ce_fwd_bwd: bad shape");
    consensus_ce_kernel<<<1, 1024, 0, (hipStream_t)stream>>>(logits, target, consensus, loss_out,
                                                              grad_logits, B, S, C);
    return check_launch("consensus_ce");
}

int dmc_profile_mark(dmc_stream_t stream) {
    dmc_profile_mark_kernel<<<1, 64, 0, (hipStream_t)stream>>>();
    return check_launch("dmc_profile_mark");
}

int dmc_version(void) { return 200; }

int dmc_set_option(const char* name, int value) {
    const int i = option_index(name);
    if (i < 0) return fail(DMC_E_INVALID, "dmc_set_option: unknown option '%s'", name ? name : "(null)");
    if (!MEASURE_BUILD && measure_only(i))
        return fail(DMC_E_INVALID, "dmc_set_option: '%s' switches parts of a kernel off (results wrong) and exists only in the -DDMC_MEASURE build", name);
    if (i == OPT_GRID_RESERVE_CUS && (value < 0 || value > 128))
        return fail(DMC_E_INVALID, "dmc_set_option: grid_reserve_cus = %d (0 .. 128 CUs may be left to other streams)", value);
    if (!MEASURE_BUILD && !product_value(i, value))
        return fail(DMC_E_INVALID, "dmc_set_option: %s = %d selects a kernel variant that lost its A/B measurement; it is compiled into the "
                    "-DDMC_MEASURE build only", name, value);
    g_options[i].store(value, std::memory_order_relaxed);
    return DMC_OK;
}
int dmc_get_option(const char* name) {
    if (name && !strcmp(name, "measure_build")) return MEASURE_BUILD ? 1 : 0;
    const int i = option_index(name);
    return i < 0 ? -1 : (!MEASURE_BUILD && measure_only(i)) ? 0 : g_options[i].load(std::memory_order_relaxed);
}
const char* dmc_last_error(void) { return err_buf(); }

}
```

### dmc-net_amd/csrc/x3s_common.h

```cpp
#pragma once
#include "dmc_common.h"

namespace dmc {
namespace x3 {

typedef float f32x16 __attribute__((ext_vector_type(16)));
typedef __bf16 bf16x8 __attribute__((ext_vector_type(8)));
typedef unsigned u32x4 __attribute__((ext_vector_type(4)));
typedef const __attribute__((address_space(3))) char* lds_cptr;

__device__ __forceinline__ f32x16 mfma_bf16(const u32x4& a, const u32x4& b, const f32x16& c) {
    return __builtin_amdgcn_mfma_f32_32x32x16_bf16(__builtin_bit_cast(bf16x8, a), __builtin_bit_cast(bf16x8, b), c, 0, 0, 0);
}

__device__ __forceinline__ void split3(float v, unsigned& u0, unsigned& u1, unsigned& u2) {
    u0 = __float_as_uint(v);
    const float r1 = v - __uint_as_float(u0 & 0xffff0000u);
    u1 = __float_as_uint(r1);
    u2 = __float_as_uint(r1 - __uint_as_float(u1 & 0xffff0000u));
}
__device__ __forceinline__ unsigned pack_hi(unsigned hi_of_second, unsigned hi_of_first) {
    return __builtin_amdgcn_perm(hi_of_second, hi_of_first, 0x07060302u);
}

constexpr unsigned OOB = 0x80000000u;

__device__ __forceinline__ void dma_buf16(const u32x4& srd, unsigned voff, unsigned soff, unsigned lds_byte_addr) {
    asm volatile("s_mov_b32 m0, %2\n\ts_nop 3\n\tbuffer_load_dwordx4 %0, %1, %3 offen lds"
                 :: "v"(voff), "s"(srd), "s"(lds_byte_addr), "s"(soff) : "memory");
}
__device__ __forceinline__ u32x4 make_srd(const void* base) {
    const unsigned long long b = (unsigned long long)base;
    u32x4 srd;
    srd[0] = __builtin_amdgcn_readfirstlane((unsigned)b);
    srd[1] = __builtin_amdgcn_readfirstlane((unsigned)(b >> 32) & 0xffffu);
    srd[2] = 0x7fffffffu;
    srd[3] = 0x00020000u;
    return srd;
}

typedef short s16x4 __attribute__((ext_vector_type(4)));
__device__ __forceinline__ void tr_read2(lds_cptr p0, lds_cptr p1, u32x4& f) {
    const s16x4 a = __builtin_amdgcn_ds_read_tr16_b64_v4i16((__attribute__((address_space(3))) s16x4*)p0);
    const s16x4 b = __builtin_amdgcn_ds_read_tr16_b64_v4i16((__attribute__((address_space(3))) s16x4*)p1);
    typedef unsigned u32x2 __attribute__((ext_vector_type(2)));
    const u32x2 ua = __builtin_bit_cast(u32x2, a), ub = __builtin_bit_cast(u32x2, b);
    f[0] = ua[0]; f[1] = ua[1]; f[2] = ub[0]; f[3] = ub[1];
}

constexpr unsigned NOPIX = 0x40000000u;

struct WgGroupPos { int n, y; };
__device__ __forceinline__ WgGroupPos wg_group_at(int q, int R, int HP) {
    const int g = R * q, n = g / HP;
    WgGroupPos p;
    p.n = __builtin_amdgcn_readfirstlane(n);
    p.y = __builtin_amdgcn_readfirstlane(g - n * HP);
    return p;
}
__device__ __forceinline__ WgGroupPos wg_group_next(WgGroupPos p, int R, int HP) {
    p.y += R;
    if (p.y >= HP) { p.y -= HP; ++p.n; }
    return p;
}
__device__ __forceinline__ WgGroupPos wg_group_prev(WgGroupPos p, int R, int HP) {
    p.y -= R;
    if (p.y < 0) { p.y += HP; --p.n; }
    return p;
}
__device__ __forceinline__ void wg_group_base(const WgGroupPos& p, int N, int W, unsigned img_bytes, unsigned& tbase, unsigned& img_off) {
    const bool in = p.n >= 0 && p.n < N;
    tbase = in ? (unsigned)((p.y - 1) * W) * 32u : NOPIX;
    img_off = in ? (unsigned)p.n * img_bytes : 0u;
}
__device__ __forceinline__ unsigned wg_lane_off(unsigned tbase, unsigned pre, unsigned img_bytes) {
    const unsigned t = tbase + pre;
    return t < img_bytes ? t : OOB;
}

typedef float f32x4 __attribute__((ext_vector_type(4)));
__device__ __forceinline__ f32x4 mfma16(const u32x4& a, const u32x4& b, const f32x4& c) {
    return __builtin_amdgcn_mfma_f32_16x16x32_bf16(__builtin_bit_cast(bf16x8, a), __builtin_bit_cast(bf16x8, b), c, 0, 0, 0);
}

__device__ __forceinline__ void split8(const float4& lo, const float4& hi, u32x4& s0, u32x4& s1, u32x4& s2) {
    const float v[8] = {lo.x, lo.y, lo.z, lo.w, hi.x, hi.y, hi.z, hi.w};
    unsigned u0[8], u1[8], u2[8];
#pragma unroll
    for (int e = 0; e < 8; ++e) split3(v[e], u0[e], u1[e], u2[e]);
#pragma unroll
    for (int e = 0; e < 4; ++e) {
        s0[e] = pack_hi(u0[2 * e + 1], u0[2 * e]);
        s1[e] = pack_hi(u1[2 * e + 1], u1[2 * e]);
        s2[e] = pack_hi(u2[2 * e + 1], u2[2 * e]);
    }
}

}
}
```

### include/dmcnet_hip.h

```cpp
#ifndef DMCNET_HIP_H
#define DMCNET_HIP_H

#include <stddef.h>
#include <stdint.h>

#ifdef __cplusplus
extern "C" {
#endif

#define DMC_OK 0
#define DMC_E_INVALID (-1)
#define DMC_E_LAUNCH (-2)

typedef void* dmc_stream_t;

int dmc_version(void);
const char* dmc_last_error(void);
int dmc_set_option(const char* name, int value);
int dmc_get_option(const char* name);
int dmc_profile_mark(dmc_stream_t stream);


size_t dmc_gen_tiny_workspace_bytes(void);
size_t dmc_gen_tiny_saved_bytes(int N, int H, int W);

int dmc_gen_tiny_fwd(const float* mv, const float* res, const float* const* w,
                     const float* const* b, float* out, float* saved, float* workspace, int N,
                     int H, int W, int add_mv_delta, dmc_stream_t stream);

size_t dmc_gen_tiny_mse_partials_bytes(void);
int dmc_gen_tiny_fwd_mse(const float* mv, const float* res, const float* const* w, const float* const* b,
                         const float* flow, float* out, float* saved, float* workspace, float* loss_out,
                         void* mse_partials, int N, int H, int W, int add_mv_delta, dmc_stream_t stream);

int dmc_gen_tiny_fwd_loss(int kind, const float* mv, const float* res, const float* const* w, const float* const* b,
                          const float* flow, float* out, float* saved, float* workspace, float* loss_out,
                          void* mse_partials, int N, int H, int W, int add_mv_delta, dmc_stream_t stream);

size_t dmc_gen_tiny_gbuf_bytes(int N, int H, int W);
size_t dmc_gen_tiny_partials_bytes(int N, int H, int W);

int dmc_gen_tiny_bwd(const float* mv, const float* res, const float* const* w,
                     const float* saved, const float* grad_out, float* const* dw,
                     float* const* db, float* gbuf, float* partials, float* workspace, int N,
                     int H, int W, dmc_stream_t stream);

size_t dmc_flow_mse_partials_bytes(void);
int dmc_flow_mse_fwd(const float* gen_flow, const float* flow, float* loss_out, float* partials,
                     size_t numel, dmc_stream_t stream);
int dmc_flow_mse_bwd(const float* gen_flow, const float* flow, const float* grad_loss,
                     float* grad_gen, size_t numel, dmc_stream_t stream);

size_t dmc_flow_loss_partials_bytes(void);
int dmc_flow_loss_fwd(int kind, const float* gen_flow, const float* flow, const float* att, float* loss_out,
                      float* partials, size_t numel, dmc_stream_t stream);
int dmc_flow_loss_bwd(int kind, const float* gen_flow, const float* flow, const float* att, const float* grad_loss,
                      float* grad_gen, float* grad_att, size_t numel, dmc_stream_t stream);

int dmc_consensus_ce_fwd_bwd(const float* logits, const int64_t* target, float* consensus,
                             float* loss_out, float* grad_logits, int B, int S, int C,
                             dmc_stream_t stream);

size_t dmc_disc_tail_stats_bytes(int C);
int dmc_disc_tail_fwd(const float* x, const float* keep, const float* gamma, const float* beta,
                      float* running_mean, float* running_var, float* y, float* stats, int N,
                      int C, int H, int W, int use_bn, int training, float eps, float momentum,
                      dmc_stream_t stream);
int dmc_disc_tail_bwd(const float* x, const float* keep, const float* gamma, float* stats,
                      const float* dy, float* dx, float* dgamma, float* dbeta, int N, int C, int H,
                      int W, int use_bn, dmc_stream_t stream);

int dmc_bn_act_supported(int M, int C);
size_t dmc_bn_act_stats_bytes(int C);
size_t dmc_bn_act_scratch_bytes(int C);
int dmc_bn_act_fwd(const float* x, const float* residual, const float* gamma, const float* beta,
                   float* running_mean, float* running_var, float* y, float* stats, void* scratch,
                   unsigned char* relu_mask, int M, int C, int relu, int training, float eps,
                   float momentum, dmc_stream_t stream);
int dmc_bn_act_bwd(const float* x, const float* residual, const float* gamma, const float* beta,
                   const float* stats, void* scratch, const float* dy, float* dx, float* dresidual,
                   float* dgamma, float* dbeta, const unsigned char* relu_mask, int M, int C, int relu,
                   dmc_stream_t stream);

int dmc_bn_apply_nhwc(const float* x, const float* gamma, const float* beta, const float* stats, float* y,
                      int M, int C, dmc_stream_t stream);
int dmc_bn_apply_act_nhwc(const float* x, const float* residual, const float* gamma, const float* beta,
                          const float* stats, float* y, unsigned char* relu_mask, int M, int C, int relu,
                          dmc_stream_t stream);
int dmc_bn_bwd_act_nhwc(const float* z, const float* gamma, const float* beta, const float* stats, void* scratch,
                        const float* dy, float* dpre, float* dgamma, float* dbeta, const float* keep, int hw,
                        float slope, int M, int C, dmc_stream_t stream);
int dmc_channel_sum_nhwc(const float* g, void* scratch, float* out, int M, int C, dmc_stream_t stream);

size_t dmc_prepare_inputs_workspace_bytes(int N, int H, int W, int flow_ds_factor);
int dmc_prepare_inputs(const unsigned char* frames_u8, const unsigned char* flip, float* out_flow,
                       float* out_mv, float* out_res, float* workspace, int N, int H, int W,
                       int flow_ds_factor, const float* std4_host, dmc_stream_t stream);

size_t dmc_prepare_crop_workspace_bytes(int N, int OH, int OW, int flow_ds_factor);
int dmc_prepare_inputs_crop(const unsigned char* frames_u8, const int* boxes, const unsigned char* flip,
                            float* out_flow, float* out_mv, float* out_res, float* workspace, int N,
                            int H0, int W0, int OH, int OW, int flow_ds_factor, const float* std4_host,
                            dmc_stream_t stream);

size_t dmc_prepare_views_workspace_bytes(int N_out, int OH, int OW, int flow_ds_factor, int upsample_interp);
int dmc_prepare_inputs_views(const unsigned char* frames_u8, const int* src_index, const int* boxes,
                             const unsigned char* flip, float* out_flow, float* out_mv, float* out_res,
                             void* workspace, int N_src, int N_out, int H0, int W0, int OH, int OW,
                             int flow_ds_factor, int upsample_interp, const float* std4_host, dmc_stream_t stream);
int dmc_prepare_interp_taps(int n_blocks, int factor, int* lo, double* dx, double* t);

size_t dmc_prepare_clip_workspace_bytes(int B, int T, int OH, int OW, int flow_ds_factor);
int dmc_prepare_clip(const unsigned char* clips_u8, const int* plans, float* out, void* workspace,
                     int B, int T, int H0, int W0, int OH, int OW, int flow_ds_factor,
                     int n_norm, const float* mean_host, const float* std_host, dmc_stream_t stream);

int dmc_bn_relu_pool_supported(int N, int H, int W, int C);
int dmc_bn_relu_pool_fwd(const float* x, const float* gamma, const float* beta, float* running_mean,
                         float* running_var, float* y_pool, float* stats, void* scratch, int N, int H,
                         int W, int C, int training, float eps, float momentum, dmc_stream_t stream);
size_t dmc_bn_relu_pool_codes_bytes(int N, int H, int W, int C);
int dmc_bn_relu_pool_bwd(const float* x, const float* gamma, const float* beta, const float* stats,
                         void* scratch, const float* d_pool, float* dx, float* dgamma, float* dbeta,
                         void* codes, int N, int H, int W, int C, dmc_stream_t stream);

int dmc_conv_nhwc_supported(int N, int H, int W, int Cin, int Cout, int KH, int KW, int stride, int pad);
int dmc_conv_nhwc_stat_blocks(int N, int H, int W, int Cin, int Cout, int KH, int stride, int pad);
int dmc_conv_nhwc_fwd(const float* x, const float* w, void* wpack, const float* bias, const float* keep, float* y,
                      double* stat_partials, int stat_blocks, int N, int H, int W, int Cin, int Cout, int KH, int KW, int stride,
                      int pad, int act, dmc_stream_t stream);
int dmc_conv_nhwc_stats_final(const double* partials, int nblk, int C, long count, float* stats,
                              float* running_mean, float* running_var, float eps, float momentum,
                              dmc_stream_t stream);
size_t dmc_conv_nhwc_wt_bytes(int Cin, int Cout, int KH, int KW);
int dmc_conv_nhwc_presplit_supported(int Cin, int Cout);
int dmc_conv_nhwc_split(const float* w, void* wpack_f, void* wpack_t, int Cin, int Cout, int KH, int KW, dmc_stream_t stream);
int dmc_conv_nhwc_dgrad(const float* dy, const float* w, float* wt, float* dx, int N, int H, int W, int Cin,
                        int Cout, int KH, int KW, int stride, int pad, dmc_stream_t stream);
int dmc_conv_nhwc_dgrad_add(const float* dy, const float* w, float* wt, const float* addend, float* dx, int N, int H, int W,
                            int Cin, int Cout, int KH, int KW, int stride, int pad, dmc_stream_t stream);
size_t dmc_conv_nhwc_wgrad_bytes(int N, int H, int W, int Cin, int Cout, int KH, int KW, int stride, int pad);
int dmc_conv_nhwc_wgrad(const float* x, const float* dy, float* dw, float* workspace, int N, int H, int W,
                        int Cin, int Cout, int KH, int KW, int stride, int pad, dmc_stream_t stream);

size_t dmc_x3s_slices_bytes(long M, int C);
int dmc_x3s_split(const float* x, void* xs, long M, int C, dmc_stream_t stream);
int dmc_x3s_merge(const void* xs, float* x, long M, int C, dmc_stream_t stream);
size_t dmc_x3s_wpack_bytes(int Cin, int Cout);
int dmc_x3s_pack_weights(const float* w, void* wpack_f, void* wpack_t, int Cin, int Cout, dmc_stream_t stream);
int dmc_x3s_conv_supported(int N, int H, int W, int Cin, int Cout);
int dmc_x3s_conv_stat_blocks(int N, int H, int W, int Cout);
int dmc_x3s_conv_fwd(const void* xs, const void* wpack_f, float* y, double* stat_partials, int stat_blocks, int N, int H, int W,
                     int Cin, int Cout, dmc_stream_t stream);
int dmc_x3s_conv_dgrad(const void* dys, const void* wpack_t, const float* addend, float* dx, int N, int H, int W, int Cin,
                       int Cout, dmc_stream_t stream);
int dmc_x3s_conv_bn_eval(const void* xs, const void* wpack_f, const float* stats, const float* gamma, const float* beta,
                         const float* residual, float* y, void* ys, int s2d, int relu, int N, int H, int W, int Cin, int Cout,
                         dmc_stream_t stream);
int dmc_x3s_conv_wgrad_supported(int N, int H, int W, int Cin, int Cout);
size_t dmc_x3s_conv_wgrad_bytes(int N, int H, int W, int Cin, int Cout);
int dmc_x3s_conv_wgrad(const void* xs, const void* dys, float* dw, float* workspace, int N, int H, int W, int Cin, int Cout,
                       dmc_stream_t stream);
int dmc_x3s_conv_dgrad_s2_supported(int N, int OH, int OW, int Cin, int Cout);
int dmc_x3s_pack_weights_s2(const float* w, void* wpack_t2, int Cin, int Cout, dmc_stream_t stream);
int dmc_x3s_conv_dgrad_s2(const void* dys, const void* wpack_t2, float* dx, int N, int OH, int OW, int Cin, int Cout,
                          dmc_stream_t stream);


int dmc_bn_apply_act_x3s(const float* x, const float* residual, const float* gamma, const float* beta, const float* stats,
                         float* y, void* ys, unsigned char* relu_mask, int M, int C, int relu, dmc_stream_t stream);
int dmc_bn_act_bwd_x3s(const float* x, const float* residual, const float* gamma, const float* beta, const float* stats,
                       void* scratch, const float* dy, float* dx, void* dxs, float* dresidual, float* dgamma, float* dbeta,
                       const unsigned char* relu_mask, int M, int C, int relu, dmc_stream_t stream);
int dmc_bn_relu_pool_fwd_x3s(const float* x, const float* gamma, const float* beta, float* running_mean, float* running_var,
                             float* y_pool, void* ys, float* stats, void* scratch, int N, int H, int W, int C, int training,
                             float eps, float momentum, dmc_stream_t stream);
int dmc_bn_relu_pool_fwd_arg(const float* x, const float* gamma, const float* beta, float* running_mean, float* running_var,
                             float* y_pool, void* ys, void* codes, float* xmax, float* stats, void* scratch, int stat_split,
                             int N, int H, int W, int C, int training, float eps, float momentum, dmc_stream_t stream);
int dmc_bn_relu_pool_bwd_arg(const float* x, const float* gamma, const float* beta, const float* stats, void* scratch,
                             const float* d_pool, const void* codes, const float* xmax, float* dx, float* dgamma, float* dbeta,
                             int N, int H, int W, int C, dmc_stream_t stream);
size_t dmc_x3q_wpack_bytes(int Cin, int Cout);
int dmc_x3q_supported(int N, int OH, int OW, int Cin, int Cout);
int dmc_x3q_stat_blocks(int N, int OH, int OW, int Cout);
int dmc_x3q_split(const float* x, void* xq, int N, int H, int W, int C, dmc_stream_t stream);
int dmc_x3q_merge(const void* xq, float* x, int N, int H, int W, int C, dmc_stream_t stream);
int dmc_x3q_pack_weights(const float* w3, const float* w1, void* wpack_f, void* wpack_t, int Cin, int Cout, dmc_stream_t stream);
int dmc_x3q_conv_fwd(const void* xq, const void* wpack_f, float* y3, float* y1, double* stat_partials3, double* stat_partials1,
                     int stat_blocks, int N, int OH, int OW, int Cin, int Cout, dmc_stream_t stream);
int dmc_x3q_conv_dgrad(const void* dys3, const void* dys1, const void* wpack_t, float* dx, int N, int OH, int OW, int Cin, int Cout,
                       dmc_stream_t stream);
int dmc_x3q_conv_bn_eval(const void* xq, const void* wpack_f, const float* stats3, const float* gamma3, const float* beta3,
                         const float* stats1, const float* gamma1, const float* beta1, float* y3, void* ys3, float* y1, int N, int OH,
                         int OW, int Cin, int Cout, dmc_stream_t stream);
int dmc_bn_apply_act_x3q(const float* x, const float* residual, const float* gamma, const float* beta, const float* stats,
                         float* y, void* yq, unsigned char* relu_mask, int N, int H, int W, int C, int relu, dmc_stream_t stream);
int dmc_x3q_conv_wgrad_supported(int N, int OH, int OW, int Cin, int Cout);
size_t dmc_x3q_conv_wgrad_bytes(int N, int OH, int OW, int Cin, int Cout);
int dmc_x3q_conv_wgrad(const void* xq, const void* dys3, const void* dys1, float* dw3, float* dw1, float* workspace, int N, int OH,
                       int OW, int Cin, int Cout, dmc_stream_t stream);

int dmc_x3s_conv_dgrad_bnb(const void* dys, const void* wpack_t, const float* addend, float* dx, const float* bn_y,
                           const float* bn_stats, const float* bn_gamma, const float* bn_beta, const unsigned char* bn_relu_mask,
                           int bn_relu, double* partials, int stat_blocks, float* dgamma, float* dbeta, int N, int H, int W, int Cin,
                           int Cout, dmc_stream_t stream);
int dmc_bn_act_bwd_x3s_apply(const float* x, const float* residual, const float* gamma, const float* beta, const float* stats,
                             const float* dy, float* dx, void* dxs, float* dresidual, const float* dgamma, const float* dbeta,
                             const unsigned char* relu_mask, int M, int C, int relu, dmc_stream_t stream);




int dmc_disc_first_supported(int Cout);
int dmc_disc_first_fwd(const float* x, const float* w, const float* bias, const float* keep, float* z, int M,
                       int H, int W, int Cout, int act, dmc_stream_t stream);
int dmc_disc_first_dgrad(const float* g, const float* w, float* dx, int M, int H, int W, int Cout,
                         dmc_stream_t stream);
size_t dmc_disc_first_wgrad_bytes(int Cout);
int dmc_disc_first_wgrad(const float* x, const float* g, float* dw, float* db, void* workspace, int M, int H,
                         int W, int Cout, dmc_stream_t stream);

int dmc_stem_wgrad_supported(int H, int W);
size_t dmc_stem_wgrad_partials_bytes(int N, int H, int W);
int dmc_stem_wgrad(const float* x, const float* dy, float* dw, float* partials, int N, int H, int W,
                   dmc_stream_t stream);
int dmc_stem_fwd(const float* x, const float* w, long ws_co, long ws_ci, long ws_ky, long ws_kx, float* y, int N, int H, int W,
                 dmc_stream_t stream);
size_t dmc_stem_fwd_x3_workspace_bytes(int N, int H, int W);
int dmc_stem_fwd_x3(const float* x, const float* w, long ws_co, long ws_ci, long ws_ky, long ws_kx, void* workspace, float* y, int N,
                    int H, int W, dmc_stream_t stream);
int dmc_stem_fwd_x3_stat_blocks(int N, int H, int W);
int dmc_stem_fwd_x3_stats(const float* x, const float* w, long ws_co, long ws_ci, long ws_ky, long ws_kx, void* workspace, float* y,
                          void* stat_scratch, int N, int H, int W, dmc_stream_t stream);
size_t dmc_stem_dgrad_workspace_bytes(void);
int dmc_stem_dgrad_supported(int H, int W);
int dmc_stem_dgrad(const float* dy, const float* w, long ws_co, long ws_ci, long ws_ky, long ws_kx, void* workspace, float* dx, int N,
                   int H, int W, dmc_stream_t stream);

int dmc_conv3d_bf16_supported(int N, int D, int H, int W, int Cin, int Cout, int KD, int KH, int KW);
size_t dmc_conv3d_bf16_wpack_bytes(int Cin, int Cout, int KD, int KH, int KW);
int dmc_conv3d_bf16_pack(const float* w, long w_s_co, long w_s_ci, long w_s_tap, void* wpack_f, void* wpack_b, int Cin, int Cout,
                         int KD, int KH, int KW, dmc_stream_t stream);
int dmc_conv3d_bf16_stat_blocks(int N, int D, int H, int W, int Cout);
int dmc_conv3d_bf16_stat_blocks_k(int N, int D, int H, int W, int Cin, int Cout, int KD, int KH, int KW);
int dmc_conv3d_bf16_fwd(const void* x, const float* w, long w_s_co, long w_s_ci, long w_s_tap, void* wpack, void* y,
                        float* stat_partials, int N, int D, int H, int W, int Cin, int Cout, int KD, int KH, int KW,
                        dmc_stream_t stream);
int dmc_conv3d_bf16_dgrad(const void* dy, const float* w, long w_s_co, long w_s_ci, long w_s_tap, void* wpack, void* dx,
                          int N, int D, int H, int W, int Cin, int Cout, int KD, int KH, int KW, dmc_stream_t stream);
size_t dmc_conv3d_bf16_wgrad_bytes(int N, int D, int H, int W, int Cin, int Cout, int KD, int KH, int KW);
int dmc_conv3d_bf16_wgrad(const void* x, const void* dy, float* dw, float* workspace, int N, int D, int H, int W, int Cin,
                          int Cout, int KD, int KH, int KW, dmc_stream_t stream);

int dmc_maxpool3d_tf_out_shape(int D, int H, int W, int C, int kd, int kh, int kw, int sd, int sh, int sw, int* od, int* oh,
                               int* ow);
int dmc_maxpool3d_tf_bf16_fwd(const void* x, void* y, void* code, int N, int D, int H, int W, int C, int kd, int kh, int kw,
                              int sd, int sh, int sw, dmc_stream_t stream);
int dmc_maxpool3d_tf_bf16_bwd(const void* dy, const void* code, void* dx, int N, int D, int H, int W, int C, int kd, int kh,
                              int kw, int sd, int sh, int sw, dmc_stream_t stream);

int dmc_bn3d_bf16_supported(long M, int C);
size_t dmc_bn3d_bf16_scratch_bytes(int C);
int dmc_bn3d_bf16_fwd(const void* y, const float* partials, int nblk, const float* gamma, const float* beta, float* stats,
                      float* running_mean, float* running_var, void* out, long M, int C, int relu, float eps, float momentum,
                      dmc_stream_t stream);
int dmc_bn3d_bf16_fwd_ld(const void* y, const float* partials, int nblk, const float* gamma, const float* beta, float* stats,
                         float* running_mean, float* running_var, void* out, long out_ld, long M, int C, int relu, float eps,
                         float momentum, dmc_stream_t stream);
int dmc_add4_bf16(const void* a, const void* b, const void* c, const void* d, void* out, long n, dmc_stream_t stream);
int dmc_bn3d_bf16_bwd(const void* dout, long dout_ld, const void* y, const float* stats, const float* gamma, const float* beta,
                      float* scratch, void* dy, float* dgamma, float* dbeta, long M, int C, int relu, dmc_stream_t stream);

size_t dmc_unit3d_bf16_fwd_workspace_bytes(int N, int D, int H, int W, int Cin, int Cout, int KD, int KH, int KW);
size_t dmc_unit3d_bf16_bwd_workspace_bytes(int N, int D, int H, int W, int Cin, int Cout, int KD, int KH, int KW);
int dmc_unit3d_bf16_fwd(const void* x, const float* w, const float* gamma, const float* beta, float* running_mean,
                        float* running_var, void* workspace, void* y, void* out, int N, int D, int H, int W, int Cin, int Cout,
                        int KD, int KH, int KW, int relu, float eps, float momentum, dmc_stream_t stream);
int dmc_unit3d_bf16_fwd_into(const void* x, const float* w, const float* gamma, const float* beta, float* running_mean,
                             float* running_var, void* workspace, void* y, void* out, long out_ld, int N, int D, int H, int W, int Cin,
                             int Cout, int KD, int KH, int KW, int relu, float eps, float momentum, dmc_stream_t stream);
int dmc_unit3d_bf16_bwd(const void* dout, long dout_ld, const void* x, const void* y, const void* fwd_workspace, const float* gamma,
                        const float* beta, void* bwd_workspace, void* dy, void* dx, float* dw, float* dgamma, float* dbeta, int N,
                        int D, int H, int W, int Cin, int Cout, int KD, int KH, int KW, int relu, dmc_stream_t stream);
size_t dmc_unit3d_bf16_eval_workspace_bytes(int N, int D, int H, int W, int Cin, int Cout, int KD, int KH, int KW);
int dmc_unit3d_bf16_fwd_eval(const void* x, const float* w, const float* gamma, const float* beta, const float* running_mean,
                             const float* running_var, float eps, void* workspace, void* out, long out_ld, int N, int D, int H, int W,
                             int Cin, int Cout, int KD, int KH, int KW, int relu, dmc_stream_t stream);

size_t dmc_stem3d_bf16_workspace_bytes(int N, int T, int H, int W);
int dmc_stem3d_bf16_stat_blocks(int N, int T, int H, int W);
int dmc_stem3d_bf16_fwd(const float* x, const float* w, void* workspace, void* y, float* stat_partials, int N, int T, int H, int W,
                        dmc_stream_t stream);
size_t dmc_stem3d_bf16_eval_workspace_bytes(int N, int T, int H, int W);
int dmc_stem3d_bf16_fwd_eval(const float* x, const float* w, const float* gamma, const float* beta, const float* running_mean,
                             const float* running_var, float eps, void* workspace, void* y, int N, int T, int H, int W, int relu,
                             dmc_stream_t stream);
size_t dmc_stem3d_bf16_wgrad_workspace_bytes(int N, int T, int H, int W);
int dmc_stem3d_bf16_wgrad(const float* x, const void* dy, float* dw, void* workspace, int N, int T, int H, int W, dmc_stream_t stream);
size_t dmc_stem3d_bf16_dgrad_workspace_bytes(void);
int dmc_stem3d_bf16_dgrad(const void* dy, const float* w, float* dx, void* workspace, int N, int T, int H, int W, dmc_stream_t stream);

size_t dmc_mv_owner_bytes(int n_frames, int H, int W);
int dmc_mv_accu_init(int32_t* accu, int H, int W, dmc_stream_t stream);
int dmc_mv_rasterise(const void* mvs, int mv_stride, int n_mv, int32_t* owner_ws, int32_t* mv_out, int32_t* bad_source, int H,
                     int W, dmc_stream_t stream);
int dmc_mv_accumulate(const void* mvs, int mv_stride, int n_mv, int32_t* owner_ws, const int32_t* accu_old, int32_t* accu_new,
                      int32_t* bad_source, int H, int W, dmc_stream_t stream);
int dmc_mv_from_accu(const int32_t* accu, int32_t* mv_out, int H, int W, dmc_stream_t stream);
int dmc_residual(const uint8_t* bgr_ref, const uint8_t* bgr_cur, const int32_t* accu, const int32_t* mv, int32_t* res, int H, int W,
                 dmc_stream_t stream);
int dmc_mv_gop_batch(const void* mvs, int mv_stride, int n_mv, const int32_t* frame_off, int n_frames, const int32_t* chain_off,
                     int n_chains, const int32_t* emit, int32_t* owner_ws, const uint8_t* bgr_ref, const uint8_t* bgr_cur,
                     int32_t* accu_out, int32_t* mv_out, int32_t* res_out, int32_t* bad_source, int H, int W, dmc_stream_t stream);

#ifdef __cplusplus
}
#endif
#endif
```

Before: 3453.

## Remap conv workgroups to XCD-contiguous tile order for L2 locality

Flattens the 2D conv and weight-gradient grids to 1D and remaps each block index so that consecutive work items land on the same XCD (round-robin dispatch across 8 XCDs). For forward/dgrad convs the remapped order walks output-channel blocks fastest within a spatial tile, so blocks sharing input patches sit in the same L2. The goal is better L2 reuse and less cross-die traffic. It adds index arithmetic per block and a measurement-only XCC logging path, and the option is on for all four kernel families by default.

After: 3473 (median of 6 runs). Within noise of the previous version (+0.6%).

```diff
diff --git a/dmc-net_amd/_lib.py b/dmc-net_amd/_lib.py
--- a/dmc-net_amd/_lib.py
+++ b/dmc-net_amd/_lib.py
@@ -75,6 +75,7 @@
     "dmc_x3s_pack_weights": (_I, [_P, _P, _P, _I, _I, _P]),
     "dmc_x3s_conv_supported": (_I, [_I] * 5),
     "dmc_x3s_conv_stat_blocks": (_I, [_I] * 4),
+    "dmc_xcd_tile_order": (_I, [_I, _P]),
     "dmc_x3s_conv_fwd": (_I, [_P] * 4 + [_I] * 6 + [_P]),
     "dmc_x3s_conv_bn_eval": (_I, [_P] * 8 + [_I] * 7 + [_P]),
     "dmc_x3s_conv_dgrad": (_I, [_P] * 4 + [_I] * 5 + [_P]),
diff --git a/dmc-net_amd/csrc/conv_x3q.hip b/dmc-net_amd/csrc/conv_x3q.hip
--- a/dmc-net_amd/csrc/conv_x3q.hip
+++ b/dmc-net_amd/csrc/conv_x3q.hip
@@ -67,6 +67,9 @@
     int K, R, M;
     unsigned plane_bytes;
     int pps0, pps1;
+    int nx = 0, ny = 0;
+    int xcd = 0;
+    DMC_XCC_FIELD
 };
 
 struct X3qEvalArgs : X3qArgs {
@@ -99,7 +102,9 @@
     const unsigned lds0 = lds_addr_of(lds_q);
 
     const int HW = a.H * a.W, PW = a.W;
-    const int m0 = blockIdx.x * BM;
+    const XcdTile wt = xcd_conv_tile(a.xcd != 0, a.nx, a.ny);
+    DMC_XCC_LOG(a);
+    const int m0 = wt.tile * BM;
     const int mlast = (m0 + BM < a.M ? m0 + BM : a.M) - 1;
     const int r_first = m0 / PW, r_last = mlast / PW;
     const int f0 = (r_first - P::HALO_UP > 0 ? r_first - P::HALO_UP : 0) * PW;
@@ -117,7 +122,7 @@
     const int nchunk = a.K >> 4;
     const int total_units = nchunk * NUNIT, total_steps = nchunk * NSTEP;
     const u32x4 srd0 = make_srd(a.t0), srd1 = make_srd(a.t1 ? a.t1 : a.t0);
-    const u32x4 srd_w = make_srd(reinterpret_cast<const char*>(a.wp) + (size_t)blockIdx.y * nchunk * CHB);
+    const u32x4 srd_w = make_srd(reinterpret_cast<const char*>(a.wp) + (size_t)wt.cb * nchunk * CHB);
     const unsigned lane16 = (unsigned)lane * 16u;
 
     auto dma_patch = [&](int c, auto uc, int pbuf, int i) {
@@ -280,7 +285,7 @@
     constexpr int CW = 32 * TN, LPR = CW / 4, RPI = 64 / LPR;
     char* etile = lds_q + wave * QETILE;
     const int mw0 = m0 + wm * 32;
-    const int rbase = blockIdx.y * QBN + wn * CW;
+    const int rbase = wt.cb * QBN + wn * CW;
     const bool ok = mw0 + l31 <= mlast;
 #pragma unroll
     for (int A = 0; A < NACC; ++A) {
@@ -350,7 +355,7 @@
                     double e1 = 0.0, e2 = 0.0;
 #pragma unroll
                     for (int w = 0; w < WM; ++w) { e1 += red[(w * 64 + cc) * 2 + 0]; e2 += red[(w * 64 + cc) * 2 + 1]; }
-                    double* dst = part + ((size_t)blockIdx.x * a.R + blockIdx.y * QBN + cc) * 2;
+                    double* dst = part + ((size_t)wt.tile * a.R + wt.cb * QBN + cc) * 2;
                     dst[0] = e1; dst[1] = e2;
                 }
                 __syncthreads();
@@ -466,24 +471,36 @@
     return t1 < t2 ? 1 : 2;
 }
 
+void q_grid(X3qArgs& a, int BM) {
+    a.nx = (a.M + BM - 1) / BM;
+    a.ny = a.R / QBN;
+    a.xcd = option(OPT_CONV_XCD) & 4;
+}
+
 template <class P, int TN, class GEO>
-int launch_q(const X3qArgs& a, hipStream_t s) {
+int launch_q(const X3qArgs& args, hipStream_t s) {
+    X3qArgs a = args;
     static LdsLimit lim;
     const hipError_t attr = lim.raise(reinterpret_cast<const void*>(&x3q_conv_kernel<P, TN, GEO>), GEO::LDS);
     if (attr != hipSuccess) return fail(DMC_E_LAUNCH, "x3q_conv: cannot raise the dynamic LDS limit: %s", hipGetErrorString(attr));
     constexpr int BM = 32 * GEO::NW / (2 / TN);
-    dim3 grid((a.M + BM - 1) / BM, a.R / QBN);
+    q_grid(a, BM);
+    const dim3 grid(a.nx * a.ny);
+    DMC_XCC_SLOT(a, 3, a.nx * a.ny, a.xcd);
     x3q_conv_kernel<P, TN, GEO><<<grid, GEO::NW * 64, GEO::LDS, s>>>(a);
     return check_launch("x3q_conv");
 }
 
 template <int TN, class GEO>
-int launch_q_eval(const X3qEvalArgs& a, hipStream_t s) {
+int launch_q_eval(const X3qEvalArgs& args, hipStream_t s) {
+    X3qEvalArgs a = args;
     static LdsLimit lim;
     const hipError_t attr = lim.raise(reinterpret_cast<const void*>(&x3q_conv_kernel<ProgFwd, TN, GEO, true>), GEO::LDS);
     if (attr != hipSuccess) return fail(DMC_E_LAUNCH, "x3q_conv_bn_eval: cannot raise the dynamic LDS limit: %s", hipGetErrorString(attr));
     constexpr int BM = 32 * GEO::NW / (2 / TN);
-    dim3 grid((a.M + BM - 1) / BM, a.R / QBN);
+    q_grid(a, BM);
+    const dim3 grid(a.nx * a.ny);
+    DMC_XCC_SLOT(a, 3, a.nx * a.ny, a.xcd);
     x3q_conv_kernel<ProgFwd, TN, GEO, true><<<grid, GEO::NW * 64, GEO::LDS, s>>>(a);
     return check_launch("x3q_conv_bn_eval");
 }
@@ -508,6 +525,9 @@
     int N, OH, Cin, Cout;
     unsigned plane_bytes;
     int steps, per_group, tiles_ci;
+    int tiles;
+    int xcd;
+    DMC_XCC_FIELD
 };
 
 template <int OW_, int R, int HP_>
@@ -539,9 +559,12 @@
     const int l31 = lane & 31, khalf = lane >> 5, L = lane & 15, grp = (lane >> 4) & 1;
     const int quarter = wave & 3, trow = wave >> 2;
     const int wi = quarter & 1, wj = quarter >> 1;
-    const int tci = blockIdx.x % a.tiles_ci, tco = blockIdx.x / a.tiles_ci;
+    const int item = xcd_work_item(a.xcd != 0);
+    DMC_XCC_LOG(a);
+    const int group = item / a.tiles, blk = item - group * a.tiles;
+    const int tci = blk % a.tiles_ci, tco = blk / a.tiles_ci;
     const unsigned lds0 = lds_addr_of(lds_qw);
-    const int s_begin = blockIdx.y * a.per_group;
+    const int s_begin = group * a.per_group;
     const int s_end = s_begin + a.per_group < a.steps ? s_begin + a.per_group : a.steps;
     const u32x4 srd_x = make_srd(a.xq), srd_d = make_srd(a.dys);
     const int nch_in = a.Cin >> 4;
@@ -660,7 +683,7 @@
         asm volatile("s_waitcnt vmcnt(0) lgkmcnt(0)" ::: "memory");
         __builtin_amdgcn_s_barrier();
     }
-    float* out = a.part + (size_t)blockIdx.y * a.Cout * 9 * a.Cin;
+    float* out = a.part + (size_t)group * a.Cout * 9 * a.Cin;
     const int ci = tci * 64 + 32 * wj + l31;
 #pragma unroll
     for (int t = 0; t < 3; ++t)
@@ -674,6 +697,8 @@
 struct X3qWg1Args {
     const void* xq; const void* dys; float* part;
     int Cin, Cout; long Mq; unsigned plane_bytes; int steps, per_group, tiles_ci;
+    int tiles, xcd;
+    DMC_XCC_FIELD
 };
 constexpr int W1PX = 64, W1PL = 68;
 constexpr int W1TILE = 12 * W1PL * 32, W1LDS = 4 * W1TILE;
@@ -684,9 +709,12 @@
     const int wave = __builtin_amdgcn_readfirstlane(tid >> 6);
     const int l31 = lane & 31, khalf = lane >> 5, L = lane & 15, grp = (lane >> 4) & 1;
     const int wi = wave & 1, wj = wave >> 1;
-    const int tci = blockIdx.x % a.tiles_ci, tco = blockIdx.x / a.tiles_ci;
+    const int item = xcd_work_item(a.xcd != 0);
+    DMC_XCC_LOG(a);
+    const int group = item / a.tiles, blk = item - group * a.tiles;
+    const int tci = blk % a.tiles_ci, tco = blk / a.tiles_ci;
     const unsigned lds0 = lds_addr_of(lds_w1);
-    const int s_begin = blockIdx.y * a.per_group;
+    const int s_begin = group * a.per_group;
     const int s_end = s_begin + a.per_group < a.steps ? s_begin + a.per_group : a.steps;
     const u32x4 srd_x = make_srd(a.xq), srd_d = make_srd(a.dys);
     const int nch_in = a.Cin >> 4, nch_out = a.Cout >> 4;
@@ -739,7 +767,7 @@
         asm volatile("s_waitcnt vmcnt(0) lgkmcnt(0)" ::: "memory");
         __builtin_amdgcn_s_barrier();
     }
-    float* out = a.part + (size_t)blockIdx.y * a.Cout * a.Cin;
+    float* out = a.part + (size_t)group * a.Cout * a.Cin;
     const int ci = tci * 64 + 32 * wj + l31;
 #pragma unroll
     for (int e = 0; e < 16; ++e) {
@@ -796,13 +824,17 @@
 }
 
 template <int OW_, int R, int HP_>
-int launch_q_wgrad(const QWgPlan& p, const X3qWgArgs& a, hipStream_t s) {
+int launch_q_wgrad(const QWgPlan& p, const X3qWgArgs& args, hipStream_t s) {
+    X3qWgArgs a = args;
     using G = QWgGeom<OW_, R, HP_>;
     static_assert(G::LDS <= 160 * 1024, "weight-gradient tiles exceed the LDS");
     static LdsLimit lim;
     const hipError_t attr = lim.raise(reinterpret_cast<const void*>(&x3q_wgrad_kernel<OW_, R, HP_>), G::LDS);
     if (attr != hipSuccess) return fail(DMC_E_LAUNCH, "x3q_wgrad: cannot raise the dynamic LDS limit: %s", hipGetErrorString(attr));
-    x3q_wgrad_kernel<OW_, R, HP_><<<dim3(p.tiles, p.groups), 768, G::LDS, s>>>(a);
+    a.tiles = p.tiles;
+    a.xcd = option(OPT_CONV_XCD) & 8;
+    DMC_XCC_SLOT(a, 4, p.tiles * p.groups, a.xcd);
+    x3q_wgrad_kernel<OW_, R, HP_><<<dim3(p.tiles * p.groups), 768, G::LDS, s>>>(a);
     return check_launch("x3q_wgrad");
 }
 
@@ -936,7 +968,10 @@
     static LdsLimit lim1;
     const hipError_t attr = lim1.raise(reinterpret_cast<const void*>(&x3q_wgrad1_kernel), W1LDS);
     if (attr != hipSuccess) return fail(DMC_E_LAUNCH, "x3q_wgrad1: cannot raise the dynamic LDS limit: %s", hipGetErrorString(attr));
-    x3q_wgrad1_kernel<<<dim3(p.tiles, p.groups1), 256, W1LDS, s>>>(b);
+    b.tiles = p.tiles;
+    b.xcd = option(OPT_CONV_XCD) & 8;
+    DMC_XCC_SLOT(b, 5, p.tiles * p.groups1, b.xcd);
+    x3q_wgrad1_kernel<<<dim3(p.tiles * p.groups1), 256, W1LDS, s>>>(b);
     rc = check_launch("x3q_wgrad1");
     if (rc) return rc;
     blocks = (numel1 + 63) / 64;
diff --git a/dmc-net_amd/csrc/conv_x3s.hip b/dmc-net_amd/csrc/conv_x3s.hip
--- a/dmc-net_amd/csrc/conv_x3s.hip
+++ b/dmc-net_amd/csrc/conv_x3s.hip
@@ -78,6 +78,9 @@
     int bnb_relu = 0;
     double* bnb_part = nullptr;
     int part_blocks = -1;
+    int nx = 0, ny = 0;
+    int xcd = 0;
+    DMC_XCC_FIELD
     int ablate;
 };
 struct X3EvalArgs : X3Args {
@@ -114,7 +117,9 @@
 
     const int HW = a.H * a.W, PW = a.W;
     constexpr int ZROW = PPMAX - 1;
-    const int m0 = blockIdx.x * BM;
+    const XcdTile wt = xcd_conv_tile(a.xcd != 0, a.nx, a.ny);
+    DMC_XCC_LOG(a);
+    const int m0 = wt.tile * BM;
     const int mlast = (m0 + BM < a.M ? m0 + BM : a.M) - 1;
     const int r_first = m0 / PW, r_last = mlast / PW;
     const int f0 = (r_first > 0 ? r_first - 1 : 0) * PW;
@@ -146,7 +151,7 @@
 
     const u32x4 srd_x = make_srd(a.xs);
     const int nchunk = a.K >> 4, S = 3 * nchunk;
-    const u32x4 srd_w = make_srd(reinterpret_cast<const char*>(a.wp) + (size_t)blockIdx.y * S * WB);
+    const u32x4 srd_w = make_srd(reinterpret_cast<const char*>(a.wp) + (size_t)wt.cb * S * WB);
     const unsigned lane16 = (unsigned)lane * 16u;
 
     const bool grp_a = wave < NA, grp_b = !STAG || wave >= NA;
@@ -300,7 +305,7 @@
     constexpr int EP = 272, ETILE = 32 * TM * EP;
     char* etile = lds_x3 + wave * ETILE;
     const int mw0 = m0 + wm * TM * 32;
-    const int rbase = blockIdx.y * BN;
+    const int rbase = wt.cb * BN;
 #pragma unroll
     for (int cl = 0; cl < CLS; ++cl) {
 #pragma unroll
@@ -412,7 +417,7 @@
             double e1 = 0.0, e2 = 0.0;
 #pragma unroll
             for (int w = 0; w < WM; ++w) { e1 += red[(w * 64 + cc) * 2 + 0]; e2 += red[(w * 64 + cc) * 2 + 1]; }
-            double* dst = a.bnb_part + ((size_t)blockIdx.x * a.R + rbase + cc) * 2;
+            double* dst = a.bnb_part + ((size_t)wt.tile * a.R + rbase + cc) * 2;
             dst[0] = e1; dst[1] = e2;
         }
     }
@@ -432,7 +437,7 @@
             double e1 = 0.0, e2 = 0.0;
 #pragma unroll
             for (int w = 0; w < WM; ++w) { e1 += red[(w * 64 + c) * 2 + 0]; e2 += red[(w * 64 + c) * 2 + 1]; }
-            double* dst = a.stat_part + ((size_t)blockIdx.x * a.R + rbase + c) * 2;
+            double* dst = a.stat_part + ((size_t)wt.tile * a.R + rbase + c) * 2;
             dst[0] = e1; dst[1] = e2;
         }
     }
@@ -450,6 +455,12 @@
         if ((int)(f1 - f0) + 1 > worst) worst = (int)(f1 - f0) + 1;
     }
     return worst;
+}
+
+void x3s_grid(X3Args& a, int BM) {
+    a.nx = (a.M + BM - 1) / BM;
+    a.ny = a.R / 64;
+    a.xcd = option(OPT_CONV_XCD) & 1;
 }
 
 struct X3Cfg { int id, BM, PPMAX, threads; };
@@ -478,14 +489,17 @@
 }
 
 template <int WM, int TM, int PPMAX>
-int launch_x3s(const X3Args& a, hipStream_t s) {
+int launch_x3s(const X3Args& args, hipStream_t s) {
     constexpr int BM = 32 * TM * WM;
+    X3Args a = args;
     constexpr size_t op_bytes = 2 * 3 * PPMAX * 32 + 2 * 3 * 3 * 64 * 32, ep_bytes = 2 * (size_t)BM * 272 + 8192;
     constexpr size_t lds_bytes = op_bytes > ep_bytes ? op_bytes : ep_bytes;
-    dim3 grid((a.M + BM - 1) / BM, a.R / 64);
-    if ((a.stat_part || a.bnb_part) && a.part_blocks >= 0 && (unsigned)a.part_blocks != grid.x)
-        return fail(DMC_E_INVALID, "x3s_conv: statistics partials have %d rows but this launch writes %u (dmc_x3s_conv_stat_blocks was "
-                                   "called under another conv_cfg option?)", a.part_blocks, grid.x);
+    x3s_grid(a, BM);
+    const dim3 grid(a.nx * a.ny);
+    DMC_XCC_SLOT(a, 1, a.nx * a.ny, a.xcd);
+    if ((a.stat_part || a.bnb_part) && a.part_blocks >= 0 && a.part_blocks != a.nx)
+        return fail(DMC_E_INVALID, "x3s_conv: statistics partials have %d rows but this launch writes %d (dmc_x3s_conv_stat_blocks was "
+                                   "called under another conv_cfg option?)", a.part_blocks, a.nx);
     if constexpr (WM >= 4) {
         if (!(option(OPT_CONV_ABLATE) & 512)) {
             static LdsLimit lim_attr2;
@@ -532,11 +546,14 @@
 }
 
 template <int WM, int TM, int PPMAX>
-int launch_x3s_eval(const X3EvalArgs& a, hipStream_t s) {
+int launch_x3s_eval(const X3EvalArgs& args, hipStream_t s) {
     constexpr int BM = 32 * TM * WM;
+    X3EvalArgs a = args;
     constexpr size_t lds_bytes = 2 * 3 * PPMAX * 32 + 2 * 3 * 3 * 64 * 32;
     static_assert((size_t)BM * 272 <= lds_bytes, "the epilogue tiles live in the operand LDS");
-    dim3 grid((a.M + BM - 1) / BM, a.R / 64);
+    x3s_grid(a, BM);
+    const dim3 grid(a.nx * a.ny);
+    DMC_XCC_SLOT(a, 1, a.nx * a.ny, a.xcd);
     static LdsLimit lim_attr;
     const hipError_t attr = lim_attr.raise(reinterpret_cast<const void*>(&x3s_conv_kernel<WM, 1, TM, 2, PPMAX, (WM >= 4), 1, true>), (int)lds_bytes);
     if (attr != hipSuccess) return fail(DMC_E_LAUNCH, "x3s_conv_bn_eval: cannot raise the dynamic LDS limit: %s", hipGetErrorString(attr));
@@ -551,6 +568,9 @@
     int N, H, Cin, Cout;
     unsigned plane_bytes;
     int steps, per_group, tiles_ci;
+    int tiles;
+    int xcd;
+    DMC_XCC_FIELD
 };
 
 template <int W_, int R>
@@ -581,10 +601,13 @@
     const int l31 = lane & 31, khalf = lane >> 5, L = lane & 15, grp = (lane >> 4) & 1;
     const int quarter = wave & 3, trow = wave >> 2;
     const int wi = quarter & 1, wj = quarter >> 1;
-    const int tci = blockIdx.x % a.tiles_ci, tco = blockIdx.x / a.tiles_ci;
+    const int item = xcd_work_item(a.xcd != 0);
+    DMC_XCC_LOG(a);
+    const int group = item / a.tiles, blk = item - group * a.tiles;
+    const int tci = blk % a.tiles_ci, tco = blk / a.tiles_ci;
     const unsigned lds0 = lds_addr_of(lds_wg);
     const int HP = a.H + 2;
-    const int s_begin = blockIdx.y * a.per_group;
+    const int s_begin = group * a.per_group;
     const int s_end = s_begin + a.per_group < a.steps ? s_begin + a.per_group : a.steps;
     const u32x4 srd_x = make_srd(a.xs), srd_d = make_srd(a.dys);
     const unsigned soff_x = (unsigned)((wave >> 2) * (a.Cin >> 4) + tci * 4 + (wave & 3)) * a.plane_bytes;
@@ -689,7 +712,7 @@
         asm volatile("s_waitcnt vmcnt(0) lgkmcnt(0)" ::: "memory");
         __builtin_amdgcn_s_barrier();
     }
-    float* out = a.part + (size_t)blockIdx.y * a.Cout * 9 * a.Cin;
+    float* out = a.part + (size_t)group * a.Cout * 9 * a.Cin;
     const int ci = tci * 64 + 32 * wj + l31;
 #pragma unroll
     for (int t = 0; t < 3; ++t)
@@ -744,7 +767,10 @@
     static LdsLimit lim_attr;
     const hipError_t attr = lim_attr.raise(reinterpret_cast<const void*>(&x3s_wgrad_kernel<W_, R>), G::LDS);
     if (attr != hipSuccess) return fail(DMC_E_LAUNCH, "x3s_wgrad: cannot raise the dynamic LDS limit: %s", hipGetErrorString(attr));
-    x3s_wgrad_kernel<W_, R><<<dim3(p.tiles, p.groups), 768, G::LDS, s>>>(a);
+    a.tiles = p.tiles;
+    a.xcd = option(OPT_CONV_XCD) & 2;
+    DMC_XCC_SLOT(a, 2, p.tiles * p.groups, a.xcd);
+    x3s_wgrad_kernel<W_, R><<<dim3(p.tiles * p.groups), 768, G::LDS, s>>>(a);
     int rc = check_launch("x3s_wgrad");
     if (rc || p.groups == 1) return rc;
     const long numel = (long)a.Cout * 9 * a.Cin;
@@ -809,6 +835,12 @@
 int dmc_x3s_conv_supported(int N, int H, int W, int Cin, int Cout) {
     return Cin % 64 == 0 && Cout % 64 == 0 && x3s_shape_ok(N, H, W, Cin, Cout) && x3s_shape_ok(N, H, W, Cout, Cin) &&
            x3s_choose(N, H, W, Cout) >= 0 && x3s_choose(N, H, W, Cin) >= 0 ? 1 : 0;
+}
+
+int dmc_xcd_tile_order(int nwg, int* order) {
+    if (nwg < 1 || !order) return fail(DMC_E_INVALID, "dmc_xcd_tile_order: bad argument");
+    for (int b = 0; b < nwg; ++b) order[b] = xcd_item(b, nwg);
+    return DMC_OK;
 }
 
 int dmc_x3s_conv_stat_blocks(int N, int H, int W, int Cout) {
@@ -915,7 +947,9 @@
     static LdsLimit lim_attr;
     const hipError_t attr = lim_attr.raise(reinterpret_cast<const void*>(&x3s_conv_kernel<4, 1, 1, 2, 320, true, 4>), (int)lds_bytes);
     if (attr != hipSuccess) return fail(DMC_E_LAUNCH, "x3s_conv_dgrad_s2: cannot raise the dynamic LDS limit: %s", hipGetErrorString(attr));
-    dim3 grid((a.M + 127) / 128, Cin / 64);
+    x3s_grid(a, 128);
+    const dim3 grid(a.nx * a.ny);
+    DMC_XCC_SLOT(a, 1, a.nx * a.ny, a.xcd);
     x3s_conv_kernel<4, 1, 1, 2, 320, true, 4><<<grid, 256, lds_bytes, (hipStream_t)stream>>>(a);
     return check_launch("x3s_conv_dgrad_s2");
 }
diff --git a/dmc-net_amd/csrc/dmc_common.h b/dmc-net_amd/csrc/dmc_common.h
--- a/dmc-net_amd/csrc/dmc_common.h
+++ b/dmc-net_amd/csrc/dmc_common.h
@@ -40,7 +40,7 @@
 };
 
 enum Option { OPT_GEN_LAYER_PATH = 0, OPT_GEN_GATHER, OPT_GEN_FUSE45, OPT_GEN_WGRAD_PATH, OPT_GEN_FUSE_FWD,
-              OPT_GEN_FUSE_BWD, OPT_GEN_FRAMES, OPT_CONV_PATH, OPT_CONV_CFG, OPT_CONV_ABLATE, OPT_GEN_ABLATE, OPT_CONV_ARITH, OPT_CONV3D_WGRAD, OPT_GEN_X3, OPT_GEN_WINO, OPT_GEN_STAGGER, OPT_GEN_FUSED, OPT_GRID_RESERVE_CUS, OPT_COUNT };
+              OPT_GEN_FUSE_BWD, OPT_GEN_FRAMES, OPT_CONV_PATH, OPT_CONV_CFG, OPT_CONV_ABLATE, OPT_GEN_ABLATE, OPT_CONV_ARITH, OPT_CONV3D_WGRAD, OPT_GEN_X3, OPT_GEN_WINO, OPT_GEN_STAGGER, OPT_GEN_FUSED, OPT_GRID_RESERVE_CUS, OPT_CONV_XCD, OPT_COUNT };
 int option(Option o);
 inline int persistent_cus(int hw) {
     const int r = option(OPT_GRID_RESERVE_CUS);
diff --git a/dmc-net_amd/csrc/losses.hip b/dmc-net_amd/csrc/losses.hip
--- a/dmc-net_amd/csrc/losses.hip
+++ b/dmc-net_amd/csrc/losses.hip
@@ -232,8 +232,8 @@
 }
 
 const char* const OPTION_NAMES[OPT_COUNT] = {"gen_layer_path", "gen_gather", "gen_fuse45", "gen_wgrad_path",
-                                             "gen_fuse_fwd", "gen_fuse_bwd", "gen_frames", "conv_path", "conv_cfg", "conv_ablate", "gen_ablate", "conv_arith", "conv3d_wgrad", "gen_x3", "gen_wino", "gen_stagger", "gen_fused", "grid_reserve_cus"};
-std::atomic<int> g_options[OPT_COUNT] = {{1}, {1}, {1}, {5}, {1}, {1}, {0}, {1}, {0}, {0}, {0}, {1}, {2}, {2}, {768}, {0}, {1}, {0}};
+                                             "gen_fuse_fwd", "gen_fuse_bwd", "gen_frames", "conv_path", "conv_cfg", "conv_ablate", "gen_ablate", "conv_arith", "conv3d_wgrad", "gen_x3", "gen_wino", "gen_stagger", "gen_fused", "grid_reserve_cus", "conv_xcd"};
+std::atomic<int> g_options[OPT_COUNT] = {{1}, {1}, {1}, {5}, {1}, {1}, {0}, {1}, {0}, {0}, {0}, {1}, {2}, {2}, {768}, {0}, {1}, {0}, {15}};
 int option_index(const char* name) {
     if (!name) return -1;
     for (int i = 0; i < OPT_COUNT; ++i)
@@ -246,6 +246,44 @@
 namespace dmc {
 int option(Option o) { return !MEASURE_BUILD && measure_only(o) ? 0 : g_options[o].load(std::memory_order_relaxed); }
 }
+
+#ifdef DMC_MEASURE
+namespace {
+constexpr int XCC_MAX_REC = 8192;
+int* g_xcc_buf = nullptr;
+long g_xcc_cap = 0, g_xcc_used = 0;
+int g_xcc_rec[XCC_MAX_REC][4], g_xcc_nrec = 0;
+std::atomic_flag g_xcc_lock = ATOMIC_FLAG_INIT;
+}
+namespace dmc { namespace x3 {
+int* xcc_log_slot(int family, int nwg, int xcd_on) {
+    while (g_xcc_lock.test_and_set(std::memory_order_acquire)) {}
+    int* slot = nullptr;
+    if (g_xcc_buf && g_xcc_nrec < XCC_MAX_REC && g_xcc_used + nwg <= g_xcc_cap) {
+        int* r = g_xcc_rec[g_xcc_nrec++];
+        r[0] = family; r[1] = nwg; r[2] = xcd_on ? 1 : 0; r[3] = (int)g_xcc_used;
+        slot = g_xcc_buf + g_xcc_used;
+        g_xcc_used += nwg;
+    }
+    g_xcc_lock.clear(std::memory_order_release);
+    return slot;
+}
+} }
+extern "C" int dmc_measure_xcc_log(int* device_buf, long ints) {
+    while (g_xcc_lock.test_and_set(std::memory_order_acquire)) {}
+    g_xcc_buf = device_buf; g_xcc_cap = device_buf ? ints : 0; g_xcc_used = 0; g_xcc_nrec = 0;
+    g_xcc_lock.clear(std::memory_order_release);
+    return DMC_OK;
+}
+extern "C" int dmc_measure_xcc_records(int* out, int max_records) {
+    while (g_xcc_lock.test_and_set(std::memory_order_acquire)) {}
+    const int n = g_xcc_nrec < max_records ? g_xcc_nrec : max_records;
+    for (int i = 0; i < n && out; ++i)
+        for (int k = 0; k < 4; ++k) out[4 * i + k] = g_xcc_rec[i][k];
+    g_xcc_lock.clear(std::memory_order_release);
+    return n;
+}
+#endif
 
 __global__ void dmc_profile_mark_kernel() {}
 
@@ -337,6 +375,8 @@
         return fail(DMC_E_INVALID, "dmc_set_option: '%s' switches parts of a kernel off (results wrong) and exists only in the -DDMC_MEASURE build", name);
     if (i == OPT_GRID_RESERVE_CUS && (value < 0 || value > 128))
         return fail(DMC_E_INVALID, "dmc_set_option: grid_reserve_cus = %d (0 .. 128 CUs may be left to other streams)", value);
+    if (i == OPT_CONV_XCD && (value < 0 || value > 15))
+        return fail(DMC_E_INVALID, "dmc_set_option: conv_xcd = %d (a mask of bits 1, 2, 4, 8)", value);
     if (!MEASURE_BUILD && !product_value(i, value))
         return fail(DMC_E_INVALID, "dmc_set_option: %s = %d selects a kernel variant that lost its A/B measurement; it is compiled into the "
                     "-DDMC_MEASURE build only", name, value);
diff --git a/dmc-net_amd/csrc/x3s_common.h b/dmc-net_amd/csrc/x3s_common.h
--- a/dmc-net_amd/csrc/x3s_common.h
+++ b/dmc-net_amd/csrc/x3s_common.h
@@ -78,6 +78,37 @@
     return t < img_bytes ? t : OOB;
 }
 
+constexpr int NXCD = 8;
+__host__ __device__ __forceinline__ int xcd_item(int b, int nwg) {
+    const int x = b % NXCD, q = nwg / NXCD, r = nwg % NXCD;
+    return x * q + (x < r ? x : r) + b / NXCD;
+}
+__device__ __forceinline__ int xcd_work_item(bool on) {
+    const int b = (int)blockIdx.x;
+    return __builtin_amdgcn_readfirstlane(on ? xcd_item(b, (int)gridDim.x) : b);
+}
+struct XcdTile { int tile, cb; };
+__device__ __forceinline__ XcdTile xcd_conv_tile(bool on, int nx, int ny) {
+    const int w = xcd_work_item(on);
+    XcdTile t;
+    if (on) { t.tile = w / ny; t.cb = w - t.tile * ny; }
+    else { t.cb = w / nx; t.tile = w - t.cb * nx; }
+    return t;
+}
+#ifdef DMC_MEASURE
+int* xcc_log_slot(int family, int nwg, int xcd_on);
+__device__ __forceinline__ void xcc_log(int* dbg) {
+    if (dbg && threadIdx.x == 0) dbg[blockIdx.x] = (int)(__builtin_amdgcn_s_getreg(20 | (3 << 11)) & 15u);
+}
+#define DMC_XCC_FIELD int* xcc_dbg = nullptr;
+#define DMC_XCC_LOG(a) xcc_log((a).xcc_dbg)
+#define DMC_XCC_SLOT(a, family, nwg, on) (a).xcc_dbg = xcc_log_slot(family, nwg, on)
+#else
+#define DMC_XCC_FIELD
+#define DMC_XCC_LOG(a) ((void)0)
+#define DMC_XCC_SLOT(a, family, nwg, on) ((void)0)
+#endif
+
 typedef float f32x4 __attribute__((ext_vector_type(4)));
 __device__ __forceinline__ f32x4 mfma16(const u32x4& a, const u32x4& b, const f32x4& c) {
     return __builtin_amdgcn_mfma_f32_16x16x32_bf16(__builtin_bit_cast(bf16x8, a), __builtin_bit_cast(bf16x8, b), c, 0, 0, 0);
diff --git a/include/dmcnet_hip.h b/include/dmcnet_hip.h
--- a/include/dmcnet_hip.h
+++ b/include/dmcnet_hip.h
@@ -150,6 +150,7 @@
 int dmc_x3s_pack_weights(const float* w, void* wpack_f, void* wpack_t, int Cin, int Cout, dmc_stream_t stream);
 int dmc_x3s_conv_supported(int N, int H, int W, int Cin, int Cout);
 int dmc_x3s_conv_stat_blocks(int N, int H, int W, int Cout);
+int dmc_xcd_tile_order(int nwg, int* order);
 int dmc_x3s_conv_fwd(const void* xs, const void* wpack_f, float* y, double* stat_partials, int stat_blocks, int N, int H, int W,
                      int Cin, int Cout, dmc_stream_t stream);
 int dmc_x3s_conv_dgrad(const void* dys, const void* wpack_t, const float* addend, float* dx, int N, int H, int W, int Cin,
```
